# hpcaitech/Open-Sora

Measured on AMD Instinct MI355X. Metric: latent_frames_per_sec (30-step rectified-flow sampling; denoise-step ms in ms_per_step), higher is better.
Workload: dtype bf16; 1 GPU; MMDiT-XL (hidden 1152, 16x72, 9+19 blocks) denoise step, latent 16x64x64 (16x512x512 px), L=16896 tokens, CFG batch 3, 30-step Euler sampling; cfg_batch=3, parallelism=single GPU

## Files before the change

### include/osk.h

```cpp
#ifndef OSK_H
#define OSK_H
#include <stdint.h>
#ifdef __cplusplus
extern "C" {
#endif

#define OSK_ABI_VERSION 2
int osk_abi_version(void);
const char* osk_arch(void);

int osk_ln_modulate_bf16(const void* x, int64_t x_batch_stride, int64_t x_row_stride,
                         void* out, int64_t out_batch_stride, int64_t out_row_stride,
                         const float* shift, const float* scale, int64_t mod_batch_stride,
                         int B, int L, int D, float eps, void* stream);

int osk_gemm_bf16(const void* A, int64_t a_batch_stride, int64_t a_row_stride, int a_rows_per_batch,
                  const void* W, int64_t w_row_stride, const float* bias,
                  void* C, int64_t c_batch_stride, int64_t c_row_stride, int c_rows_per_batch,
                  const void* res, const float* gate, int64_t gate_batch_stride,
                  int M, int N, int K, int gelu_from, int out_f32, void* stream);

int osk_gemm_tile_choice(int M, int N, int K);
int osk_gemm_tile_override(int tile_kind);
int osk_gemm_tile_choice_strided(int M, int N, int K, int64_t a_batch_stride, int64_t a_row_stride, int a_rows_per_batch,
                                 int64_t w_row_stride);

typedef struct OskGemmOperands {
  const void* A; int64_t a_batch_stride, a_row_stride; int a_rows_per_batch;
  const void* W; int64_t w_row_stride; const float* bias;
  void* C; int64_t c_batch_stride, c_row_stride; int c_rows_per_batch;
  const void* res; const float* gate; int64_t gate_batch_stride;
  int M;
} OskGemmOperands;
int osk_gemm_bf16_pair(const OskGemmOperands* first, const OskGemmOperands* second, int N, int K, int gelu_from, void* stream);

typedef struct OskGemmTask {
  OskGemmOperands op;
  int N, gelu_from;
  int skip_from, skip_len;
  int vt_head_dim;
} OskGemmTask;
int osk_gemm_group_bf16(const OskGemmTask* tasks, int n_tasks, int K, void* stream);

int osk_gemm_geglu_bf16(const void* A, int64_t a_batch_stride, int64_t a_row_stride, int a_rows_per_batch,
                        const void* W_packed, int64_t w_row_stride, const float* bias_packed, void* C,
                        int64_t c_batch_stride, int64_t c_row_stride, int c_rows_per_batch, int M, int N_out, int K,
                        void* workspace, int64_t workspace_bytes, void* stream);

int osk_ln_modulate_fp8(const void* x, int64_t x_batch_stride, int64_t x_row_stride, void* out8, float* scales,
                        const float* shift, const float* scale, int64_t mod_batch_stride,
                        int B, int L, int D, float eps, void* stream);
int osk_quantize_rows_fp8(const void* x, int64_t x_batch_stride, int64_t x_row_stride, int rows_per_batch,
                          void* out8, float* scales, int M, int K, void* stream);
int osk_gemm_fp8(const void* A8, int64_t a_batch_stride, int64_t a_row_stride, int a_rows_per_batch,
                 const float* a_scale, const void* W8, int64_t w_row_stride, const float* w_scale,
                 const float* bias, void* C, int64_t c_batch_stride, int64_t c_row_stride, int c_rows_per_batch,
                 const void* res, const float* gate, int64_t gate_batch_stride,
                 int M, int N, int K, int gelu_from, int out_f32, void* stream);

int osk_gemv_tasks_bf16(const float* x, int64_t x_batch_stride, int Bv, int K,
                        const uint64_t* w_ptrs, const uint64_t* b_ptrs, const int32_t* out_cols,
                        const int32_t* n_rows, int n_tasks,
                        float* out, int64_t out_batch_stride, int act_in, int accumulate, void* stream);

int osk_timestep_embedding(const float* t, int B, int dim, float max_period, float time_factor,
                           float* out, void* stream);

int osk_rope_table(const float* ids, int64_t n_rows, int n_axes, const int32_t* axes_dim_host,
                   double theta, int f32_angles, float* cos_out, float* sin_out, void* stream);

int osk_qknorm_rope_bf16(void* q, void* k, int64_t batch_stride, int64_t row_stride,
                         const void* q_scale0, const void* k_scale0,
                         const void* q_scale1, const void* k_scale1, int l_split,
                         const float* cos_t, const float* sin_t, int64_t cs_batch_stride,
                         int B, int L, int H, int hd, int rope_mode, float eps, float q_mult, void* stream);

int osk_v_transpose_bf16(const void* v, int64_t batch_stride, int64_t row_stride,
                         void* vt, int B, int L, int H, int hd, void* stream);

int osk_kv_join_bf16(const void* k_seg, const void* v_seg,
                     int64_t seg_stride, int64_t batch_stride, int64_t row_stride,
                     void* k_out, int64_t ko_batch_stride, int64_t ko_row_stride,
                     void* vt_out,
                     int B, int H, int hd, int n_seg, int seg_len, int L, void* stream);

#define OSK_KV_JOIN_K_BF16 0
#define OSK_KV_JOIN_K_E4M3 1
int osk_kv_quant_rows_fp8(const void* x, int64_t batch_stride, int64_t row_stride, const float* scales,
                          void* out, int64_t o_batch_stride, int64_t o_row_stride,
                          int B, int L, int H, int hd, void* stream);
int osk_kv_join_fp8(const void* k_seg, int64_t k_seg_stride, int64_t k_batch_stride, int64_t k_row_stride, int k_kind,
                    const void* v_seg, int64_t v_seg_stride, int64_t v_batch_stride, int64_t v_row_stride,
                    void* k_out, int64_t ko_batch_stride, int64_t ko_row_stride,
                    void* vt8_out,
                    int B, int H, int hd, int n_seg, int seg_len, int L, void* stream);

int osk_attention_fwd_bf16(const void* q, int64_t q_batch_stride, int64_t q_row_stride,
                           const void* k, int64_t k_seg_stride, int64_t k_batch_stride, int64_t k_row_stride,
                           const void* vt, int64_t vt_seg_stride,
                           void* out, int64_t o_batch_stride, int64_t o_row_stride,
                           float* lse, int B, int H, int Lq, int n_seg, int seg_len, int hd,
                           float scale, int q_prescaled, int kv_batches, void* stream);

int64_t osk_attention_workspace_bytes(void);
int osk_attention_tail_split_factor(int B, int H, int Lq, int n_seg, int seg_len, int hd, int64_t workspace_bytes);
int osk_attention_launch_shape(int B, int H, int Lq, int n_seg, int seg_len, int hd, float score_bound,
                               int64_t workspace_bytes, int* rows_per_unit);
int osk_attention_rows_override(int rows_per_unit);
int osk_attention_fwd_ws_bf16(const void* q, int64_t q_batch_stride, int64_t q_row_stride,
                           const void* k, int64_t k_seg_stride, int64_t k_batch_stride, int64_t k_row_stride,
                           const void* vt, int64_t vt_seg_stride,
                           void* out, int64_t o_batch_stride, int64_t o_row_stride,
                           float* lse, int B, int H, int Lq, int n_seg, int seg_len, int hd,
                           float scale, int q_prescaled, int kv_batches, void* workspace, int64_t workspace_bytes, void* stream);

int osk_attention_fwd_bounded_bf16(const void* q, int64_t q_batch_stride, int64_t q_row_stride,
                           const void* k, int64_t k_seg_stride, int64_t k_batch_stride, int64_t k_row_stride,
                           const void* vt, int64_t vt_seg_stride,
                           void* out, int64_t o_batch_stride, int64_t o_row_stride,
                           float* lse, int B, int H, int Lq, int n_seg, int seg_len, int hd,
                           float scale, int q_prescaled, int kv_batches, float score_bound,
                           void* workspace, int64_t workspace_bytes, void* stream);

int osk_rownorm2_max_bf16(const void* x, int64_t batch_stride, int64_t row_stride, int B, int L, int H, int hd,
                          float* out, int accumulate, void* stream);
int osk_attention_fwd_auto_bf16(const void* q, int64_t q_batch_stride, int64_t q_row_stride,
                           const void* k, int64_t k_seg_stride, int64_t k_batch_stride, int64_t k_row_stride,
                           const void* vt, int64_t vt_seg_stride,
                           void* out, int64_t o_batch_stride, int64_t o_row_stride,
                           float* lse, int B, int H, int Lq, int n_seg, int seg_len, int hd,
                           float scale, int q_prescaled, int kv_batches, const float* q_norm2_max, const float* k_norm2_max,
                           void* workspace, int64_t workspace_bytes, void* stream);

int osk_attention_merge_bf16(const void* parts, int64_t part_stride, int64_t p_batch_stride, int64_t p_row_stride,
                             const float* lse, void* out, int64_t o_batch_stride, int64_t o_row_stride, float* lse_out,
                             int S, int B, int H, int L, int hd, void* stream);

int osk_v_scale_fp8(const void* v, int64_t v_batch_stride, int64_t v_row_stride, float* scales, int B, int L, int H,
                    int hd, void* stream);
int osk_kv_scale_fp8(const void* k, int64_t k_batch_stride, int64_t k_row_stride,
                     const void* v, int64_t v_batch_stride, int64_t v_row_stride, float* scales,
                     int B, int L, int H, int hd, void* stream);
int osk_v_transpose_fp8(const void* v, int64_t v_batch_stride, int64_t v_row_stride, const float* scales, void* vt8,
                        int B, int L, int H, int hd, void* stream);
int osk_attention_fwd_pv8_bf16(const void* q, int64_t q_batch_stride, int64_t q_row_stride,
                               const void* k, int64_t k_seg_stride, int64_t k_batch_stride, int64_t k_row_stride,
                               const void* vt8, int64_t vt8_seg_stride, const float* v_scale,
                               void* out, int64_t o_batch_stride, int64_t o_row_stride,
                               float* lse, int B, int H, int Lq, int n_seg, int seg_len, int hd,
                               float scale, int q_prescaled, int kv_batches, void* workspace, int64_t workspace_bytes,
                               void* stream);

int osk_k_pack_fp8(const void* k, int64_t k_batch_stride, int64_t k_row_stride, const float* scales, void* k8,
                   int B, int L, int H, int hd, void* stream);
int osk_attention_fwd_qk8_bf16(const void* q, int64_t q_batch_stride, int64_t q_row_stride,
                               const void* k8, int64_t k8_seg_stride, int64_t k8_batch_stride, int64_t k8_row_stride,
                               const float* k_scale, const void* vt8, int64_t vt8_seg_stride, const float* v_scale,
                               void* out, int64_t o_batch_stride, int64_t o_row_stride,
                               float* lse, int B, int H, int Lq, int n_seg, int seg_len, int hd,
                               float scale, int q_prescaled, int kv_batches, void* workspace, int64_t workspace_bytes,
                               void* stream);

#define OSK_ATTN_BF16 0
#define OSK_ATTN_PV8 1
#define OSK_ATTN_QK8 2
int64_t osk_attention_ragged_workspace_bytes(int B, int H, int Lq, int hd);
int osk_attention_fwd_ragged_bf16(const void* q, int64_t q_batch_stride, int64_t q_row_stride,
                                  const void* k, int64_t k_seg_stride, int64_t k_batch_stride, int64_t k_row_stride,
                                  const float* k_scale, const void* vt, int64_t vt_seg_stride, const float* v_scale,
                                  void* out, int64_t o_batch_stride, int64_t o_row_stride, float* lse,
                                  int B, int H, int Lq, int n_seg, int seg_len, int last_seg_len, int hd,
                                  float scale, int q_prescaled, int kv_batches, float score_bound, int mode,
                                  void* workspace, int64_t workspace_bytes, void* stream);
int osk_attention_merge_into_bf16(void* out, int64_t o_batch_stride, int64_t o_row_stride, float* lse, const float* o_b,
                                  const float* lse_b, int B, int H, int Lq, int hd, void* stream);
int osk_attention_merge_into2_bf16(void* out, int64_t o_batch_stride, int64_t o_row_stride, float* lse, const float* o_b,
                                   const float* lse_b, const float* o_c, const float* lse_c, int B, int H, int Lq, int hd,
                                   void* stream);

int64_t osk_attention_window_workspace_bytes(int B, int H, int Lq, int hd);
int osk_attention_fwd_window_bf16(const void* q, int64_t q_batch_stride, int64_t q_row_stride,
                                  const void* k, int64_t k_batch_stride, int64_t k_row_stride, const void* vt,
                                  void* out, int64_t o_batch_stride, int64_t o_row_stride, float* lse,
                                  int B, int H, int Lq, int Lk, int n_prefix, int hd, float scale, int q_prescaled,
                                  int kv_batches, float score_bound, const int32_t* windows, int n_windows,
                                  void* workspace, int64_t workspace_bytes, void* stream);
int osk_attention_fwd_window_fp8_bf16(const void* q, int64_t q_batch_stride, int64_t q_row_stride,
                                      const void* k, int64_t k_batch_stride, int64_t k_row_stride, const float* k_scale,
                                      const void* vt, const float* v_scale, void* out, int64_t o_batch_stride,
                                      int64_t o_row_stride, float* lse, int B, int H, int Lq, int Lk, int n_prefix, int hd,
                                      float scale, int q_prescaled, int kv_batches, int mode, const int32_t* windows,
                                      int n_windows, void* workspace, int64_t workspace_bytes, void* stream);
int64_t osk_attention_window_anchor_workspace_bytes(int B, int H, int Lq, int hd);
int osk_attention_fwd_window_anchor_bf16(const void* q, int64_t q_batch_stride, int64_t q_row_stride,
                                         const void* k, int64_t k_batch_stride, int64_t k_row_stride, const float* k_scale,
                                         const void* vt, const float* v_scale, void* out, int64_t o_batch_stride,
                                         int64_t o_row_stride, float* lse, int B, int H, int Lq, int Lk, int n_prefix,
                                         int n_suffix, int hd, float scale, int q_prescaled, int kv_batches, float score_bound,
                                         int mode, const int32_t* windows, int n_windows, void* workspace,
                                         int64_t workspace_bytes, void* stream);

int osk_attention_short_bf16(const void* q, int64_t q_batch_stride, int64_t q_row_stride, const void* k, int64_t k_batch_stride,
                             int64_t k_row_stride, const void* v, int64_t v_batch_stride, int64_t v_row_stride, void* out,
                             int64_t o_batch_stride, int64_t o_row_stride, const float* alibi_slopes, int B, int H, int Lq, int Lk,
                             int hd, float scale, void* stream);

int osk_attention_relbias_bf16(const void* q, int64_t q_batch_stride, int64_t q_row_stride, const void* k, int64_t k_batch_stride,
                               int64_t k_row_stride, const void* v, int64_t v_batch_stride, int64_t v_row_stride, void* out,
                               int64_t o_batch_stride, int64_t o_row_stride, const float* bias, int64_t bias_row_stride, int B,
                               int H, int L, int hd, float scale, void* stream);

const char* osk_attention_kernel_name(int hd, int seg_len);
const char* osk_attention_body_name(int hd, int n_seg, int seg_len, float score_bound);

int osk_cfg_euler_bf16(const void* pred, int64_t n, const void* x, void* x_out,
                       float g_txt, float g_img, const float* g_img_vec, float dt, void* stream);

int osk_cfg_euler_nb_bf16(const void* pred, int nb, int64_t n, const void* x, void* x_out,
                          float g_txt, float g_img, const float* g_img_vec, float dt, void* stream);

int osk_copy_rows_bf16(const void* src, int64_t src_chunk_stride, int64_t src_batch_stride, int64_t src_row_stride, void* dst,
                       int64_t dst_chunk_stride, int64_t dst_batch_stride, int64_t dst_row_stride, int n_chunks, int B, int L, int C,
                       void* stream);

int64_t osk_step_delta_workspace_bytes(int B, int L, int C);
int osk_step_delta_bf16(const void* cur, int64_t cur_batch_stride, int64_t cur_row_stride, void* prev, float* sums, int B, int L, int C,
                        void* workspace, int64_t workspace_bytes, void* stream);

int osk_step_sums_combine_f32(const float* pairs, int P, float* sums, void* stream);

int osk_residual_sub_bf16(const void* a, int64_t a_batch_stride, int64_t a_row_stride, const void* b, int64_t b_batch_stride,
                          int64_t b_row_stride, void* out, int64_t out_batch_stride, int64_t out_row_stride, int B, int L, int C,
                          void* stream);
int osk_residual_add_bf16(const void* a, int64_t a_batch_stride, int64_t a_row_stride, const void* b, int64_t b_batch_stride,
                          int64_t b_row_stride, void* out, int64_t out_batch_stride, int64_t out_row_stride, int B, int L, int C,
                          void* stream);

int osk_attn_cache_copy_bf16(const void* src, int64_t src_batch_stride, int64_t src_row_stride, void* dst, int64_t dst_batch_stride,
                             int64_t dst_row_stride, const int32_t* row_map, int cache_rows, int to_cache, int B, int L, int C,
                             void* stream);


int osk_causal_conv3d_ndhwc_bf16(const void* x, int B, int T, int H, int W, int Cin,
                                 const void* w, int64_t w_row_stride, const float* bias, int Cout, int ksize,
                                 int stride_t, int stride_h, int stride_w, int up_t, int up_hw,
                                 const void* res, void* out, int To, int Ho, int Wo, void* stream);

int osk_causal_conv3d_gn_ndhwc_bf16(const void* x, int B, int T, int H, int W, int Cin,
                                    const void* w, int64_t w_row_stride, const float* bias, int Cout, int ksize,
                                    int stride_t, int stride_h, int stride_w, int up_t, int up_hw,
                                    const void* res, void* out, int To, int Ho, int Wo,
                                    double* gn_sums, int gn_groups, void* stream);


int osk_conv2d_nhwc_bf16(const void* x, int B, int H, int W, int Cin, const void* w, int64_t w_row_stride,
                         const float* bias, int Cout, int ksize, int stride, int pad, int up, const void* res,
                         void* out, int Ho, int Wo, double* gn_sums, int gn_groups, void* stream);

int osk_groupnorm_stats_ndhwc_bf16(const void* x, int B, int64_t S, int C, int G, double* sums, void* stream);

int osk_groupnorm_apply_ndhwc_bf16(const void* x, const double* sums, const float* gamma, const float* beta,
                                   void* out, int B, int64_t S, int C, int G, float eps, int silu, void* stream);

int osk_groupnorm_table_f32(const double* sums, const float* gamma, const float* beta, float* table, int B, int64_t S,
                            int C, int G, float eps, void* stream);
int osk_causal_conv3d_gnin_ndhwc_bf16(const void* x, const float* gn_in_table, int B, int T, int H, int W, int Cin,
                                      const void* w, int64_t w_row_stride, const float* bias, int Cout, int ksize,
                                      int stride_t, int stride_h, int stride_w, const void* res, void* out, int To, int Ho,
                                      int Wo, double* gn_sums, int gn_groups, void* stream);

int osk_masked_softmax_f32_bf16(const float* scores, int64_t ld_scores, void* probs, int64_t ld_probs,
                                int Sq, int Sk, int keys_per_frame, float scale, void* stream);

int osk_attention_hd512_fwd_bf16(const void* q, int64_t q_batch_stride, int64_t q_row_stride, const void* k,
                                 int64_t k_batch_stride, int64_t k_row_stride, const void* vt, int64_t vt_batch_stride,
                                 int64_t vt_row_stride, const float* bias_v, void* out, int64_t out_batch_stride,
                                 int64_t out_row_stride, int B, int S, int keys_per_frame, float scale, void* stream);
int osk_attention_hd512_fwd_ws_bf16(const void* q, int64_t q_batch_stride, int64_t q_row_stride, const void* k,
                                    int64_t k_batch_stride, int64_t k_row_stride, const void* vt, int64_t vt_batch_stride,
                                    int64_t vt_row_stride, const float* bias_v, void* out, int64_t out_batch_stride,
                                    int64_t out_row_stride, int B, int S, int keys_per_frame, float scale, void* workspace,
                                    int64_t workspace_bytes, void* stream);
int64_t osk_attention_hd512_workspace_bytes(int B, int S);

int osk_blend_bf16(const void* a, void* b, int64_t outer, int Da, int Db, int extent, int64_t inner, void* stream);


int osk_conv3d_zp_ndhwc_bf16(const void* x, int B, int T, int H, int W, int Cin, const void* w, int64_t w_row_stride,
                             const float* bias, int Cout, int ksize, int up_t, int up_hw, int act, const void* res,
                             void* out, void* stream);

int osk_conv3d_zp_strided_ndhwc_bf16(const void* x, int B, int T, int H, int W, int Cin, const void* w, int64_t w_row_stride,
                                     const float* bias, int Cout, int stride_t, int stride_hw, const void* res, void* out,
                                     void* stream);

int osk_unshuffle_avg_ndhwc_bf16(const void* x, int B, int T, int H, int W, int Cin, void* out, int Cout, int ft, int fhw,
                                 void* stream);

int osk_dup_shuffle_ndhwc_bf16(const void* x, int B, int T, int H, int W, int Cin, void* out, int Cout, int ft, int fhw,
                               void* stream);

int osk_dwconv3d_ndhwc_bf16(const void* x, int B, int T, int H, int W, int C, const void* w, const float* bias, int ksize,
                            int glu, void* out, void* stream);

int osk_gconv32_bf16(const void* x, int64_t M, int C, const void* w, void* out, void* stream);

int osk_relu_linear_attn_bf16(const void* qkv, int B, int N, int G, void* out, int64_t out_row_stride, float* workspace,
                              int64_t workspace_bytes, int nsplit, float eps, void* stream);

int osk_rmsnorm_affine_bf16(const void* x, int64_t M, int C, const float* weight, const float* bias, float eps,
                            const void* res, int relu, void* out, void* stream);


int osk_layernorm_affine_bf16(const void* x, int64_t x_row_stride, void* out, int64_t out_row_stride, const float* weight,
                              const float* bias, int64_t M, int C, float eps, void* stream);

int osk_attention_causal_bf16(const void* q, int64_t q_batch_stride, int64_t q_row_stride, const void* k, int64_t k_batch_stride,
                              int64_t k_row_stride, const void* v, int64_t v_batch_stride, int64_t v_row_stride, void* out,
                              int64_t o_batch_stride, int64_t o_row_stride, int B, int H, int L, int hd, float scale, void* stream);

int osk_gemm_quickgelu_bf16(const void* A, int64_t a_batch_stride, int64_t a_row_stride, int a_rows_per_batch, const void* W,
                            int64_t w_row_stride, const float* bias, void* C, int64_t c_batch_stride, int64_t c_row_stride,
                            int c_rows_per_batch, int M, int N, int K, void* stream);

typedef struct OskLoraAdapter {
  const void* a; int64_t a_row_stride;
  const void* b; int64_t b_row_stride;
  int r; float scale;
} OskLoraAdapter;
int osk_lora_merge_bf16(const void* w, int64_t w_row_stride, void* out, int64_t out_row_stride, int N, int K,
                        const OskLoraAdapter* adapters, int n_adapters, void* stream);

#ifdef __cplusplus
}
#endif
#endif
```

### open_sora_amd/_C.py

```python
from __future__ import annotations

import ctypes as C
import os

import torch

from .build import LIB_PATH

_i64, _i32, _f32, _f64, _vp = C.c_int64, C.c_int32, C.c_float, C.c_double, C.c_void_p

SIGNATURES = {
    "osk_abi_version": [],
    "osk_arch": [],
    "osk_gemm_geglu_bf16": [_vp, _i64, _i64, _i32, _vp, _i64, _vp, _vp, _i64, _i64, _i32, _i32, _i32, _i32, _vp, _i64, _vp],
    "osk_attention_short_bf16": [_vp, _i64, _i64, _vp, _i64, _i64, _vp, _i64, _i64, _vp, _i64, _i64, _vp, _i32, _i32, _i32, _i32, _i32,
                                 _f32, _vp],
    "osk_attention_relbias_bf16": [_vp, _i64, _i64, _vp, _i64, _i64, _vp, _i64, _i64, _vp, _i64, _i64, _vp, _i64, _i32, _i32, _i32, _i32,
                                   _f32, _vp],
    "osk_attention_kernel_name": [_i32, _i32],
    "osk_attention_body_name": [_i32, _i32, _i32, _f32],
    "osk_ln_modulate_bf16": [_vp, _i64, _i64, _vp, _i64, _i64, _vp, _vp, _i64, _i32, _i32, _i32, _f32, _vp],
    "osk_gemm_bf16": [_vp, _i64, _i64, _i32, _vp, _i64, _vp, _vp, _i64, _i64, _i32, _vp, _vp, _i64,
                      _i32, _i32, _i32, _i32, _i32, _vp],
    "osk_gemm_bf16_pair": [_vp, _vp, _i32, _i32, _i32, _vp],
    "osk_gemm_group_bf16": [_vp, _i32, _i32, _vp],
    "osk_gemm_tile_choice": [_i32, _i32, _i32],
    "osk_gemm_tile_choice_strided": [_i32, _i32, _i32, _i64, _i64, _i32, _i64],
    "osk_gemm_tile_override": [_i32],
    "osk_ln_modulate_fp8": [_vp, _i64, _i64, _vp, _vp, _vp, _vp, _i64, _i32, _i32, _i32, _f32, _vp],
    "osk_quantize_rows_fp8": [_vp, _i64, _i64, _i32, _vp, _vp, _i32, _i32, _vp],
    "osk_gemm_fp8": [_vp, _i64, _i64, _i32, _vp, _vp, _i64, _vp, _vp, _vp, _i64, _i64, _i32, _vp, _vp, _i64,
                     _i32, _i32, _i32, _i32, _i32, _vp],
    "osk_gemv_tasks_bf16": [_vp, _i64, _i32, _i32, _vp, _vp, _vp, _vp, _i32, _vp, _i64, _i32, _i32, _vp],
    "osk_timestep_embedding": [_vp, _i32, _i32, _f32, _f32, _vp, _vp],
    "osk_rope_table": [_vp, _i64, _i32, C.POINTER(_i32), _f64, _i32, _vp, _vp, _vp],
    "osk_qknorm_rope_bf16": [_vp, _vp, _i64, _i64, _vp, _vp, _vp, _vp, _i32, _vp, _vp, _i64,
                             _i32, _i32, _i32, _i32, _i32, _f32, _f32, _vp],
    "osk_v_transpose_bf16": [_vp, _i64, _i64, _vp, _i32, _i32, _i32, _i32, _vp],
    "osk_kv_join_bf16": [_vp, _vp, _i64, _i64, _i64, _vp, _i64, _i64, _vp, _i32, _i32, _i32, _i32, _i32, _i32, _vp],
    "osk_kv_quant_rows_fp8": [_vp, _i64, _i64, _vp, _vp, _i64, _i64, _i32, _i32, _i32, _i32, _vp],
    "osk_kv_join_fp8": [_vp, _i64, _i64, _i64, _i32, _vp, _i64, _i64, _i64, _vp, _i64, _i64, _vp, _i32, _i32, _i32, _i32, _i32, _i32, _vp],
    "osk_attention_fwd_bf16": [_vp, _i64, _i64, _vp, _i64, _i64, _i64, _vp, _i64, _vp, _i64, _i64, _vp,
                               _i32, _i32, _i32, _i32, _i32, _i32, _f32, _i32, _i32, _vp],
    "osk_attention_fwd_ws_bf16": [_vp, _i64, _i64, _vp, _i64, _i64, _i64, _vp, _i64, _vp, _i64, _i64, _vp,
                                  _i32, _i32, _i32, _i32, _i32, _i32, _f32, _i32, _i32, _vp, _i64, _vp],
    "osk_attention_fwd_bounded_bf16": [_vp, _i64, _i64, _vp, _i64, _i64, _i64, _vp, _i64, _vp, _i64, _i64, _vp,
                                       _i32, _i32, _i32, _i32, _i32, _i32, _f32, _i32, _i32, _f32, _vp, _i64, _vp],
    "osk_attention_fwd_auto_bf16": [_vp, _i64, _i64, _vp, _i64, _i64, _i64, _vp, _i64, _vp, _i64, _i64, _vp,
                                    _i32, _i32, _i32, _i32, _i32, _i32, _f32, _i32, _i32, _vp, _vp, _vp, _i64, _vp],
    "osk_attention_merge_bf16": [_vp, _i64, _i64, _i64, _vp, _vp, _i64, _i64, _vp, _i32, _i32, _i32, _i32, _i32, _vp],
    "osk_attention_ragged_workspace_bytes": [_i32, _i32, _i32, _i32],
    "osk_attention_fwd_ragged_bf16": [_vp, _i64, _i64, _vp, _i64, _i64, _i64, _vp, _vp, _i64, _vp, _vp, _i64, _i64, _vp,
                                      _i32, _i32, _i32, _i32, _i32, _i32, _i32, _f32, _i32, _i32, _f32, _i32, _vp, _i64, _vp],
    "osk_attention_merge_into_bf16": [_vp, _i64, _i64, _vp, _vp, _vp, _i32, _i32, _i32, _i32, _vp],
    "osk_attention_window_workspace_bytes": [_i32, _i32, _i32, _i32],
    "osk_attention_fwd_window_bf16": [_vp, _i64, _i64, _vp, _i64, _i64, _vp, _vp, _i64, _i64, _vp, _i32, _i32, _i32, _i32, _i32, _i32,
                                      _f32, _i32, _i32, _f32, _vp, _i32, _vp, _i64, _vp],
    "osk_attention_fwd_window_fp8_bf16": [_vp, _i64, _i64, _vp, _i64, _i64, _vp, _vp, _vp, _vp, _i64, _i64, _vp, _i32, _i32, _i32, _i32,
                                          _i32, _i32, _f32, _i32, _i32, _i32, _vp, _i32, _vp, _i64, _vp],
    "osk_attention_merge_into2_bf16": [_vp, _i64, _i64, _vp, _vp, _vp, _vp, _vp, _i32, _i32, _i32, _i32, _vp],
    "osk_attention_window_anchor_workspace_bytes": [_i32, _i32, _i32, _i32],
    "osk_attention_fwd_window_anchor_bf16": [_vp, _i64, _i64, _vp, _i64, _i64, _vp, _vp, _vp, _vp, _i64, _i64, _vp, _i32, _i32, _i32, _i32,
                                             _i32, _i32, _i32, _f32, _i32, _i32, _f32, _i32, _vp, _i32, _vp, _i64, _vp],
    "osk_rownorm2_max_bf16": [_vp, _i64, _i64, _i32, _i32, _i32, _i32, _vp, _i32, _vp],
    "osk_attention_workspace_bytes": [],
    "osk_v_scale_fp8": [_vp, _i64, _i64, _vp, _i32, _i32, _i32, _i32, _vp],
    "osk_kv_scale_fp8": [_vp, _i64, _i64, _vp, _i64, _i64, _vp, _i32, _i32, _i32, _i32, _vp],
    "osk_v_transpose_fp8": [_vp, _i64, _i64, _vp, _vp, _i32, _i32, _i32, _i32, _vp],
    "osk_attention_fwd_pv8_bf16": [_vp, _i64, _i64, _vp, _i64, _i64, _i64, _vp, _i64, _vp, _vp, _i64, _i64, _vp,
                                   _i32, _i32, _i32, _i32, _i32, _i32, _f32, _i32, _i32, _vp, _i64, _vp],
    "osk_k_pack_fp8": [_vp, _i64, _i64, _vp, _vp, _i32, _i32, _i32, _i32, _vp],
    "osk_attention_fwd_qk8_bf16": [_vp, _i64, _i64, _vp, _i64, _i64, _i64, _vp, _vp, _i64, _vp, _vp, _i64, _i64, _vp,
                                   _i32, _i32, _i32, _i32, _i32, _i32, _f32, _i32, _i32, _vp, _i64, _vp],
    "osk_attention_tail_split_factor": [_i32, _i32, _i32, _i32, _i32, _i32, _i64],
    "osk_attention_launch_shape": [_i32, _i32, _i32, _i32, _i32, _i32, _f32, _i64, C.POINTER(_i32)],
    "osk_attention_rows_override": [_i32],
    "osk_cfg_euler_bf16": [_vp, _i64, _vp, _vp, _f32, _f32, _vp, _f32, _vp],
    "osk_cfg_euler_nb_bf16": [_vp, _i32, _i64, _vp, _vp, _f32, _f32, _vp, _f32, _vp],
    "osk_copy_rows_bf16": [_vp, _i64, _i64, _i64, _vp, _i64, _i64, _i64, _i32, _i32, _i32, _i32, _vp],
    "osk_step_delta_workspace_bytes": [_i32, _i32, _i32],
    "osk_step_delta_bf16": [_vp, _i64, _i64, _vp, _vp, _i32, _i32, _i32, _vp, _i64, _vp],
    "osk_step_sums_combine_f32": [_vp, _i32, _vp, _vp],
    "osk_residual_sub_bf16": [_vp, _i64, _i64, _vp, _i64, _i64, _vp, _i64, _i64, _i32, _i32, _i32, _vp],
    "osk_residual_add_bf16": [_vp, _i64, _i64, _vp, _i64, _i64, _vp, _i64, _i64, _i32, _i32, _i32, _vp],
    "osk_attn_cache_copy_bf16": [_vp, _i64, _i64, _vp, _i64, _i64, _vp, _i32, _i32, _i32, _i32, _i32, _vp],
    "osk_causal_conv3d_ndhwc_bf16": [_vp, _i32, _i32, _i32, _i32, _i32, _vp, _i64, _vp, _i32, _i32, _i32, _i32, _i32,
                                     _i32, _i32, _vp, _vp, _i32, _i32, _i32, _vp],
    "osk_causal_conv3d_gn_ndhwc_bf16": [_vp, _i32, _i32, _i32, _i32, _i32, _vp, _i64, _vp, _i32, _i32, _i32, _i32, _i32,
                                        _i32, _i32, _vp, _vp, _i32, _i32, _i32, _vp, _i32, _vp],
    "osk_causal_conv3d_gnin_ndhwc_bf16": [_vp, _vp, _i32, _i32, _i32, _i32, _i32, _vp, _i64, _vp, _i32, _i32, _i32, _i32,
                                          _i32, _vp, _vp, _i32, _i32, _i32, _vp, _i32, _vp],
    "osk_conv2d_nhwc_bf16": [_vp, _i32, _i32, _i32, _i32, _vp, _i64, _vp, _i32, _i32, _i32, _i32, _i32, _vp, _vp, _i32, _i32,
                             _vp, _i32, _vp],
    "osk_groupnorm_table_f32": [_vp, _vp, _vp, _vp, _i32, _i64, _i32, _i32, _f32, _vp],
    "osk_groupnorm_stats_ndhwc_bf16": [_vp, _i32, _i64, _i32, _i32, _vp, _vp],
    "osk_groupnorm_apply_ndhwc_bf16": [_vp, _vp, _vp, _vp, _vp, _i32, _i64, _i32, _i32, _f32, _i32, _vp],
    "osk_masked_softmax_f32_bf16": [_vp, _i64, _vp, _i64, _i32, _i32, _i32, _f32, _vp],
    "osk_blend_bf16": [_vp, _vp, _i64, _i32, _i32, _i32, _i64, _vp],
    "osk_attention_hd512_fwd_ws_bf16": [_vp, _i64, _i64, _vp, _i64, _i64, _vp, _i64, _i64, _vp, _vp, _i64, _i64, _i32, _i32,
                                        _i32, _f32, _vp, _i64, _vp],
    "osk_attention_hd512_workspace_bytes": [_i32, _i32],
    "osk_attention_hd512_fwd_bf16": [_vp, _i64, _i64, _vp, _i64, _i64, _vp, _i64, _i64, _vp, _vp, _i64, _i64, _i32, _i32,
                                     _i32, _f32, _vp],
    "osk_conv3d_zp_ndhwc_bf16": [_vp, _i32, _i32, _i32, _i32, _i32, _vp, _i64, _vp, _i32, _i32, _i32, _i32, _i32, _vp, _vp, _vp],
    "osk_conv3d_zp_strided_ndhwc_bf16": [_vp, _i32, _i32, _i32, _i32, _i32, _vp, _i64, _vp, _i32, _i32, _i32, _vp, _vp, _vp],
    "osk_dup_shuffle_ndhwc_bf16": [_vp, _i32, _i32, _i32, _i32, _i32, _vp, _i32, _i32, _i32, _vp],
    "osk_unshuffle_avg_ndhwc_bf16": [_vp, _i32, _i32, _i32, _i32, _i32, _vp, _i32, _i32, _i32, _vp],
    "osk_dwconv3d_ndhwc_bf16": [_vp, _i32, _i32, _i32, _i32, _i32, _vp, _vp, _i32, _i32, _vp, _vp],
    "osk_gconv32_bf16": [_vp, _i64, _i32, _vp, _vp, _vp],
    "osk_relu_linear_attn_bf16": [_vp, _i32, _i32, _i32, _vp, _i64, _vp, _i64, _i32, _f32, _vp],
    "osk_rmsnorm_affine_bf16": [_vp, _i64, _i32, _vp, _vp, _f32, _vp, _i32, _vp, _vp],
    "osk_layernorm_affine_bf16": [_vp, _i64, _vp, _i64, _vp, _vp, _i64, _i32, _f32, _vp],
    "osk_attention_causal_bf16": [_vp, _i64, _i64, _vp, _i64, _i64, _vp, _i64, _i64, _vp, _i64, _i64, _i32, _i32, _i32, _i32, _f32, _vp],
    "osk_gemm_quickgelu_bf16": [_vp, _i64, _i64, _i32, _vp, _i64, _vp, _vp, _i64, _i64, _i32, _i32, _i32, _i32, _vp],
    "osk_lora_merge_bf16": [_vp, _i64, _vp, _i64, _i32, _i32, _vp, _i32, _vp],
}


def _load() -> C.CDLL:
    if not os.path.isfile(LIB_PATH):
        raise ImportError(
            f"{LIB_PATH} is missing: build it with `python -m open_sora_amd.build` (hipcc, gfx950). "
            "open_sora_amd has no CPU or eager fallback."
        )
    lib = C.CDLL(LIB_PATH)
    for name, argtypes in SIGNATURES.items():
        fn = getattr(lib, name)
        fn.argtypes = argtypes
        fn.restype = (C.c_char_p if name in ("osk_arch", "osk_attention_kernel_name", "osk_attention_body_name") else
                      _i64 if name in ("osk_attention_workspace_bytes", "osk_attention_hd512_workspace_bytes",
                                       "osk_attention_ragged_workspace_bytes", "osk_attention_window_workspace_bytes",
                                       "osk_attention_window_anchor_workspace_bytes",
                                       "osk_step_delta_workspace_bytes") else _i32)
    if lib.osk_abi_version() != 2:
        raise ImportError("libosk_hip.so ABI version mismatch")
    return lib


class _TracingLib:

    def __init__(self, inner):
        self._inner = inner
        self._ids: dict = {}

    def _norm(self, kind, v):
        if kind is _vp:
            if v is None:
                return "NULL"
            v = int(v)
            k = self._ids.setdefault(v, len(self._ids))
            return f"p{k}@{v & 0xFF:02x}"
        if isinstance(v, C.Array):
            return tuple(int(x) for x in v)
        return round(float(v), 9) if kind in (_f32, _f64) else int(v)

    def __getattr__(self, name):
        fn = getattr(self._inner, name)
        sig = SIGNATURES.get(name)
        if sig is None:
            return fn

        def traced(*args):
            TRACE_LOG.append((name,) + tuple(self._norm(k, a) for k, a in zip(sig, args)))
            return fn(*args)

        return traced


TRACE_LOG: list = []
lib = _load()
if os.environ.get("OSK_TRACE"):
    lib = _TracingLib(lib)


OSK_EUNSUPPORTED = -2


def _check(status: int, what: str) -> None:
    if status != 0:
        kind = "invalid argument / unsupported shape" if status < 0 else "HIP error"
        raise RuntimeError(f"{what} failed: status {status} ({kind})")


def _stream() -> int:
    return torch.cuda.current_stream().cuda_stream


def _p(t) -> int | None:
    return None if t is None else t.data_ptr()


def ln_modulate(x: torch.Tensor, shift: torch.Tensor, scale: torch.Tensor, out: torch.Tensor,
                mod_batch_stride: int, eps: float = 1e-6) -> torch.Tensor:
    B, L, D = x.shape
    assert x.dtype == torch.bfloat16 and out.dtype == torch.bfloat16 and shift.dtype == torch.float32, (x.dtype, out.dtype)
    _check(lib.osk_ln_modulate_bf16(x.data_ptr(), x.stride(0), x.stride(1), out.data_ptr(), out.stride(0),
                                    out.stride(1), shift.data_ptr(), scale.data_ptr(), mod_batch_stride,
                                    B, L, D, eps, _stream()), "osk_ln_modulate_bf16")
    return out


PROFILE_GEMM = None
PROFILE_ATTENTION = None


class _prof:

    def __init__(self, sink, *extra):
        self.sink, self.extra = sink, extra

    def __enter__(self):
        if self.sink is not None:
            self.e0, self.e1 = torch.cuda.Event(enable_timing=True), torch.cuda.Event(enable_timing=True)
            self.e0.record()

    def __exit__(self, *exc):
        if self.sink is not None:
            self.e1.record()
            self.sink.append((self.e0, self.e1, *self.extra))
        return False


def _gemm_prof(flops: float) -> _prof:
    return _prof(PROFILE_GEMM, flops)


def _attn_prof() -> _prof:
    return _prof(PROFILE_ATTENTION)


def gemm(a: torch.Tensor, w: torch.Tensor, bias, out: torch.Tensor, *, res=None, gate=None,
         gate_batch_stride: int = 0, gelu_from: int | None = None) -> torch.Tensor:
    B, L, K = a.shape
    N = w.shape[0]
    assert out.shape[0] == B and out.shape[1] == L and out.shape[2] == N
    assert a.dtype == torch.bfloat16 and w.dtype == torch.bfloat16 and out.dtype in (torch.bfloat16, torch.float32), \
        (a.dtype, w.dtype, out.dtype)
    if res is not None:
        assert res.stride() == out.stride() and res.dtype == torch.bfloat16
    with _gemm_prof(2.0 * B * L * N * K):
        _check(lib.osk_gemm_bf16(a.data_ptr(), a.stride(0), a.stride(1), L, w.data_ptr(), w.stride(0), _p(bias),
                                 out.data_ptr(), out.stride(0), out.stride(1), L, _p(res), _p(gate),
                                 gate_batch_stride, B * L, N, K, N if gelu_from is None else gelu_from,
                                 1 if out.dtype == torch.float32 else 0, _stream()), "osk_gemm_bf16")
    return out


def gemm_tile_kind(a: torch.Tensor, w: torch.Tensor) -> int:
    B, L, K = a.shape
    kind = lib.osk_gemm_tile_choice_strided(B * L, w.shape[0], K, a.stride(0), a.stride(1), L, w.stride(0))
    if kind < 0:
        _check(kind, "osk_gemm_tile_choice_strided")
    return kind


def geglu_pack(w_value: torch.Tensor, w_gate: torch.Tensor, b_value=None, b_gate=None):
    n, k = w_value.shape
    assert w_gate.shape == (n, k) and n % 16 == 0
    w = torch.stack((w_value.reshape(n // 16, 16, k), w_gate.reshape(n // 16, 16, k)), 1).reshape(2 * n, k).contiguous()
    b = None
    if b_value is not None:
        b = torch.stack((b_value.float().reshape(n // 16, 16), b_gate.float().reshape(n // 16, 16)), 1).reshape(2 * n).contiguous()
    return w, b


def gemm_geglu(a: torch.Tensor, w_packed: torch.Tensor, bias_packed, out: torch.Tensor, workspace: torch.Tensor | None = None):
    B, L, K = a.shape
    n_out = w_packed.shape[0] // 2
    assert out.shape == (B, L, n_out) and a.dtype == out.dtype == w_packed.dtype == torch.bfloat16
    _check(lib.osk_gemm_geglu_bf16(a.data_ptr(), a.stride(0), a.stride(1), L, w_packed.data_ptr(), w_packed.stride(0), _p(bias_packed),
                                   out.data_ptr(), out.stride(0), out.stride(1), L, B * L, n_out, K, _p(workspace),
                                   0 if workspace is None else workspace.numel() * workspace.element_size(), _stream()),
           "osk_gemm_geglu_bf16")
    return out


class OskGemmOperands(C.Structure):
    _fields_ = [("A", _vp), ("a_batch_stride", _i64), ("a_row_stride", _i64), ("a_rows_per_batch", _i32),
                ("W", _vp), ("w_row_stride", _i64), ("bias", _vp),
                ("C", _vp), ("c_batch_stride", _i64), ("c_row_stride", _i64), ("c_rows_per_batch", _i32),
                ("res", _vp), ("gate", _vp), ("gate_batch_stride", _i64), ("M", _i32)]


def _gemm_operands(a, w, bias, out, res, gate, gate_batch_stride, *, wide_out: bool = False) -> OskGemmOperands:
    B, L, K = a.shape
    assert out.shape[0] == B and out.shape[1] == L and (out.shape[2] >= 1 if wide_out else out.shape[2] == w.shape[0]) and w.shape[1] == K
    assert a.dtype == torch.bfloat16 and w.dtype == torch.bfloat16 and out.dtype == torch.bfloat16
    if res is not None:
        assert res.stride() == out.stride() and res.dtype == torch.bfloat16
    return OskGemmOperands(a.data_ptr(), a.stride(0), a.stride(1), L, w.data_ptr(), w.stride(0), _p(bias), out.data_ptr(),
                           out.stride(0), out.stride(1), L, _p(res), _p(gate), gate_batch_stride, B * L)


def gemm_pair(first: dict, second: dict, *, gelu_from: int | None = None) -> None:
    ops = [_gemm_operands(d["a"], d["w"], d["bias"], d["out"], d.get("res"), d.get("gate"), d.get("gate_batch_stride", 0))
           for d in (first, second)]
    N, K = first["w"].shape
    assert tuple(second["w"].shape) == (N, K)
    with _gemm_prof(2.0 * (ops[0].M + ops[1].M) * N * K):
        _check(lib.osk_gemm_bf16_pair(C.addressof(ops[0]), C.addressof(ops[1]), N, K, N if gelu_from is None else gelu_from,
                                      _stream()), "osk_gemm_bf16_pair")


class OskGemmTask(C.Structure):
    _fields_ = [("op", OskGemmOperands), ("N", _i32), ("gelu_from", _i32), ("skip_from", _i32), ("skip_len", _i32), ("vt_head_dim", _i32)]


def gemm_group(tasks: list) -> bool:
    arr = (OskGemmTask * len(tasks))()
    K = None
    flops = 0.0
    for t, d in zip(arr, tasks):
        if "vt" in d:
            x, w, vt = d["x"], d["w"], d["vt"]
            B, L, k_ = x.shape
            assert x.dtype == w.dtype == vt.dtype == torch.bfloat16 and vt.is_contiguous() and vt.dim() == 4 and d["vt_pos"] % 64 == 0
            assert vt.shape[0] == B and vt.shape[1] * vt.shape[2] == w.shape[0] and d["vt_pos"] + (L + 63) // 64 * 64 <= vt.shape[3]
            t.op = OskGemmOperands(x.data_ptr(), x.stride(0), x.stride(1), L, w.data_ptr(), w.stride(0), _p(d.get("bias")),
                                   vt.data_ptr() + 2 * d["vt_pos"], vt.stride(0), vt.stride(2), L, None, None, 0, B * L)
            t.N, t.gelu_from, t.skip_from, t.skip_len, t.vt_head_dim = w.shape[0], w.shape[0], 0, 0, d["hd"]
            flops += 2.0 * B * L * w.shape[0] * k_
        else:
            a, w, out = d["a"], d["w"], d["out"]
            k_ = a.shape[2]
            t.op = _gemm_operands(a, w, d.get("bias"), out, d.get("res"), d.get("gate"), d.get("gate_batch_stride", 0), wide_out=True)
            sf, sl = d.get("skip", (0, 0))
            t.N, t.gelu_from, t.skip_from, t.skip_len, t.vt_head_dim = w.shape[0], d.get("gelu_from", w.shape[0]) if d.get("gelu_from") is not None else w.shape[0], sf, sl, 0
            flops += 2.0 * a.shape[0] * a.shape[1] * (w.shape[0] - sl) * k_
        assert K in (None, k_), "the tasks of a group share K"
        K = k_
    with _gemm_prof(flops):
        rc = lib.osk_gemm_group_bf16(C.addressof(arr), len(tasks), K, _stream())
    if rc == OSK_EUNSUPPORTED:
        return False
    _check(rc, "osk_gemm_group_bf16")
    return True


def ln_modulate_fp8(x: torch.Tensor, shift: torch.Tensor, scale: torch.Tensor, mod_batch_stride: int, eps: float = 1e-6):
    B, L, D = x.shape
    out8 = torch.empty(B * L, D, dtype=torch.uint8, device=x.device)
    scales = torch.empty(B * L, dtype=torch.float32, device=x.device)
    _check(lib.osk_ln_modulate_fp8(x.data_ptr(), x.stride(0), x.stride(1), out8.data_ptr(), scales.data_ptr(),
                                   shift.data_ptr(), scale.data_ptr(), mod_batch_stride, B, L, D, eps, _stream()),
           "osk_ln_modulate_fp8")
    return out8, scales


def quantize_rows_fp8(x: torch.Tensor, out8: torch.Tensor | None = None, scales: torch.Tensor | None = None):
    if x.dim() == 2:
        x = x.unsqueeze(0)
    B, L, K = x.shape
    M = B * L
    if out8 is None:
        out8 = torch.empty(M, K, dtype=torch.uint8, device=x.device)
    if scales is None:
        scales = torch.empty(M, dtype=torch.float32, device=x.device)
    assert out8.is_contiguous() and out8.numel() == M * K and scales.numel() >= M
    _check(lib.osk_quantize_rows_fp8(x.data_ptr(), x.stride(0), x.stride(1), L, out8.data_ptr(), scales.data_ptr(),
                                     M, K, _stream()), "osk_quantize_rows_fp8")
    return out8, scales


def gemm_fp8_supported(M: int, N: int, K: int) -> bool:
    return M >= 256 and N >= 128 and K % 128 == 0 and 256 * K <= 0xFFFFFFFF


def gemm_fp8(a8: torch.Tensor, a_scale: torch.Tensor, w8: torch.Tensor, w_scale: torch.Tensor, bias,
             out: torch.Tensor, *, res=None, gate=None, gate_batch_stride: int = 0,
             gelu_from: int | None = None) -> torch.Tensor:
    M, K = a8.shape
    N = w8.shape[0]
    B, L = out.shape[0], out.shape[1]
    assert B * L == M and out.shape[2] == N and w8.shape[1] == K
    if res is not None:
        assert res.stride() == out.stride()
    with _gemm_prof(2.0 * M * N * K):
        _check(lib.osk_gemm_fp8(a8.data_ptr(), 0, a8.stride(0), M, a_scale.data_ptr(), w8.data_ptr(), w8.stride(0),
                                w_scale.data_ptr(), _p(bias), out.data_ptr(), out.stride(0), out.stride(1), L, _p(res),
                                _p(gate), gate_batch_stride, M, N, K, N if gelu_from is None else gelu_from,
                                1 if out.dtype == torch.float32 else 0, _stream()), "osk_gemm_fp8")
    return out


def gemv_tasks(x: torch.Tensor, tasks, out: torch.Tensor, act_in: int = 0, accumulate: bool = False):
    Bv, K = x.shape
    _check(lib.osk_gemv_tasks_bf16(x.data_ptr(), x.stride(0), Bv, K, tasks.w_ptrs.data_ptr(),
                                   tasks.b_ptrs.data_ptr(), tasks.out_cols.data_ptr(),
                                   tasks.n_rows.data_ptr(), tasks.n_tasks, out.data_ptr(), out.stride(0),
                                   act_in, 1 if accumulate else 0, _stream()), "osk_gemv_tasks_bf16")
    return out


class GemvTasks:

    ROWS = 64

    def __init__(self, layers, device):
        wp, bp, oc, nr = [], [], [], []
        self._keep = []
        for w, b, col in layers:
            assert w.dtype == torch.bfloat16 and w.is_contiguous()
            self._keep.append((w, b))
            N, K = w.shape
            for r0 in range(0, N, self.ROWS):
                n = min(self.ROWS, N - r0)
                wp.append(w.data_ptr() + r0 * K * 2)
                bp.append(0 if b is None else b.data_ptr() + r0 * 2)
                oc.append(col + r0)
                nr.append(n)
        self.n_tasks = len(wp)
        to_i64 = lambda v: v - (1 << 64) if v >= (1 << 63) else v
        self.w_ptrs = torch.tensor([to_i64(v) for v in wp], dtype=torch.int64, device=device)
        self.b_ptrs = torch.tensor([to_i64(v) for v in bp], dtype=torch.int64, device=device)
        self.out_cols = torch.tensor(oc, dtype=torch.int32, device=device)
        self.n_rows = torch.tensor(nr, dtype=torch.int32, device=device)


def timestep_embedding(t: torch.Tensor, out: torch.Tensor, max_period: float = 10000.0,
                       time_factor: float = 1000.0) -> torch.Tensor:
    B, dim = out.shape
    _check(lib.osk_timestep_embedding(t.data_ptr(), B, dim, max_period, time_factor, out.data_ptr(), _stream()),
           "osk_timestep_embedding")
    return out


def rope_table(ids: torch.Tensor, axes_dim, theta: float, f32_angles: bool, cos: torch.Tensor, sin: torch.Tensor):
    n_rows, n_axes = ids.shape
    arr = (_i32 * n_axes)(*[int(a) for a in axes_dim])
    _check(lib.osk_rope_table(ids.data_ptr(), n_rows, n_axes, arr, float(theta), 1 if f32_angles else 0,
                              cos.data_ptr(), sin.data_ptr(), _stream()), "osk_rope_table")


def qknorm_rope(q: torch.Tensor, k: torch.Tensor, qs0, ks0, qs1, ks1, l_split: int, cos, sin,
                cs_batch_stride: int, H: int, hd: int, rope_mode: int, eps: float = 1e-6, q_mult: float = 1.0):
    t = q if q is not None else k
    B, L, _ = t.shape
    assert q is None or k is None or q.stride() == k.stride()
    _check(lib.osk_qknorm_rope_bf16(_p(q), _p(k), t.stride(0), t.stride(1), qs0.data_ptr(),
                                    ks0.data_ptr(), qs1.data_ptr(), ks1.data_ptr(), l_split, cos.data_ptr(),
                                    sin.data_ptr(), cs_batch_stride, B, L, H, hd, rope_mode, eps, q_mult, _stream()),
           "osk_qknorm_rope_bf16")


def v_transpose(v: torch.Tensor, vt: torch.Tensor, H: int, hd: int):
    B, L, _ = v.shape
    _check(lib.osk_v_transpose_bf16(v.data_ptr(), v.stride(0), v.stride(1), vt.data_ptr(), B, L, H, hd, _stream()),
           "osk_v_transpose_bf16")


def kv_join(k_seg: torch.Tensor, v_seg: torch.Tensor, k_out: torch.Tensor, vt_out: torch.Tensor, H: int, hd: int, L: int):
    n_seg, B, seg_len, D = k_seg.shape
    assert k_seg.dtype == v_seg.dtype == k_out.dtype == vt_out.dtype == torch.bfloat16 and D == H * hd, (k_seg.dtype, v_seg.dtype, D, H, hd)
    assert v_seg.shape == k_seg.shape and v_seg.stride() == k_seg.stride() and k_seg.stride(3) == 1, (v_seg.shape, v_seg.stride(), k_seg.stride())
    assert tuple(k_out.shape) == (B, L, D) and k_out.stride(2) == 1, (k_out.shape, k_out.stride())
    assert tuple(vt_out.shape) == (B, H, hd, (L + 63) // 64 * 64) and vt_out.is_contiguous(), (vt_out.shape, vt_out.stride())
    _check(lib.osk_kv_join_bf16(k_seg.data_ptr(), v_seg.data_ptr(), k_seg.stride(0), k_seg.stride(1), k_seg.stride(2), k_out.data_ptr(),
                                k_out.stride(0), k_out.stride(1), vt_out.data_ptr(), B, H, hd, n_seg, seg_len, L, _stream()),
           "osk_kv_join_bf16")


_ATTN_WS: dict = {}


def attention_workspace(device) -> torch.Tensor:
    dev = torch.device(device)
    key = (str(dev), torch.cuda.current_stream(dev).cuda_stream if dev.type == "cuda" else 0)
    ws = _ATTN_WS.get(key)
    if ws is None:
        ws = _ATTN_WS[key] = torch.empty(lib.osk_attention_workspace_bytes(), dtype=torch.uint8, device=dev)
    return ws


def _attn_call(name: str, q, k, vt, out, H, hd, scale, lse, n_seg, seg_len, k_seg_stride, vt_seg_stride, q_prescaled, kv_batches,
               workspace, own=(), after_vt=()):
    B, Lq, _ = q.shape
    with _attn_prof():
        _check(getattr(lib, name)(q.data_ptr(), q.stride(0), q.stride(1), k.data_ptr(), k_seg_stride, k.stride(0), k.stride(1),
                                  vt.data_ptr(), vt_seg_stride, *after_vt, out.data_ptr(), out.stride(0), out.stride(1), _p(lse),
                                  B, H, Lq, n_seg, k.shape[1] if seg_len is None else seg_len, hd, scale, int(q_prescaled),
                                  kv_batches, *own, _p(workspace), 0 if workspace is None else workspace.numel(), _stream()), name)
    return out


def attention_fwd(q: torch.Tensor, k: torch.Tensor, vt: torch.Tensor, out: torch.Tensor, H: int, hd: int,
                  scale: float, *, lse=None, n_seg: int = 1, seg_len: int | None = None,
                  k_seg_stride: int = 0, vt_seg_stride: int = 0, q_prescaled: bool = False, kv_batches: int = 0,
                  workspace: torch.Tensor | None = None, score_bound: float = 0.0):
    if CHECK_SCORE_BOUND and score_bound > 0 and not torch.cuda.is_current_stream_capturing():
        _assert_score_bound(q, k, H, hd, scale, n_seg, k.shape[1] if seg_len is None else seg_len, k_seg_stride, q_prescaled, kv_batches,
                            score_bound)
    return _attn_call("osk_attention_fwd_bounded_bf16", q, k, vt, out, H, hd, scale, lse, n_seg, seg_len, k_seg_stride, vt_seg_stride,
                      q_prescaled, kv_batches, workspace, own=(float(score_bound),))


def rownorm2_max(x: torch.Tensor, out: torch.Tensor, H: int, hd: int, accumulate: bool = False) -> torch.Tensor:
    B, L, _ = x.shape
    assert x.dtype == torch.bfloat16 and out.dtype == torch.float32 and out.is_contiguous() and out.numel() == B * H
    _check(lib.osk_rownorm2_max_bf16(x.data_ptr(), x.stride(0), x.stride(1), B, L, H, hd, out.data_ptr(), 1 if accumulate else 0, _stream()),
           "osk_rownorm2_max_bf16")
    return out


def attention_fwd_auto(q: torch.Tensor, k: torch.Tensor, vt: torch.Tensor, out: torch.Tensor, H: int, hd: int, scale: float,
                       qn2: torch.Tensor, kn2: torch.Tensor, *, lse=None, n_seg: int = 1, seg_len: int | None = None,
                       k_seg_stride: int = 0, vt_seg_stride: int = 0, q_prescaled: bool = True, kv_batches: int = 0,
                       workspace: torch.Tensor | None = None):
    B = q.shape[0]
    assert qn2.dtype == kn2.dtype == torch.float32 and qn2.numel() == B * H and kn2.numel() == (kv_batches or B) * H
    return _attn_call("osk_attention_fwd_auto_bf16", q, k, vt, out, H, hd, scale, lse, n_seg, seg_len, k_seg_stride, vt_seg_stride,
                      q_prescaled, kv_batches, workspace, own=(qn2.data_ptr(), kn2.data_ptr()))


def attention_merge(parts: torch.Tensor, lse: torch.Tensor, out: torch.Tensor, H: int, hd: int,
                    lse_out: torch.Tensor | None = None) -> torch.Tensor:
    assert parts.dim() == 4 and lse.dim() == 4 and out.dim() == 3, (parts.shape, lse.shape, out.shape)
    S, B, L, D = parts.shape
    assert 1 <= S <= 8 and D == H * hd and hd % 8 == 0, (parts.shape, H, hd)
    assert parts.dtype == torch.bfloat16 and out.dtype == torch.bfloat16 and tuple(out.shape) == (B, L, D), (parts.dtype, out.dtype, out.shape)
    assert lse.dtype == torch.float32 and lse.is_contiguous() and tuple(lse.shape) == (S, B, H, L), (lse.dtype, lse.shape, lse.stride())
    for t in (parts, out):
        assert t.stride(-1) == 1 and all(st % 8 == 0 for st in t.stride()[:-1]) and t.data_ptr() % 16 == 0, (t.stride(), t.data_ptr() % 16)
    if lse_out is not None:
        assert lse_out.dtype == torch.float32 and lse_out.is_contiguous() and tuple(lse_out.shape) == (B, H, L), (lse_out.dtype, lse_out.shape)
    _check(lib.osk_attention_merge_bf16(parts.data_ptr(), parts.stride(0), parts.stride(1), parts.stride(2), lse.data_ptr(),
                                        out.data_ptr(), out.stride(0), out.stride(1), _p(lse_out), S, B, H, L, hd, _stream()),
           "osk_attention_merge_bf16")
    return out


def _grown_workspace(kind: str, need: int, device) -> torch.Tensor:
    dev = torch.device(device)
    key = (kind, str(dev), torch.cuda.current_stream(dev).cuda_stream if dev.type == "cuda" else 0)
    ws = _ATTN_WS.get(key)
    if ws is None or ws.numel() < need:
        ws = _ATTN_WS[key] = torch.empty(need, dtype=torch.uint8, device=dev)
    return ws


def attention_ragged_workspace(B: int, H: int, Lq: int, hd: int, device) -> torch.Tensor:
    return _grown_workspace("ragged", lib.osk_attention_ragged_workspace_bytes(B, H, Lq, hd), device)


def _attn_operands(mode: int, q, k, k_scale, vt, v_scale, out, lse, H: int, hd: int, kv_batches: int, Lk: int, k_seg_stride: int = 0,
                   vt_seg_stride: int = 0, vt_keys: int | None = None):
    assert mode != 2 or hd == 128, f"the fp8 QK^T kernel exists for head_dim 128 only, not {hd}"
    assert q.dim() == 3 and q.shape[2] == H * hd, (q.shape, H, hd)
    assert q.dtype == torch.bfloat16 and out.dtype == torch.bfloat16 and q.stride(2) == 1 and out.stride(2) == 1, (q.dtype, out.dtype, q.stride(), out.stride())
    assert q.stride(0) % 8 == 0 and q.stride(1) % 8 == 0 and q.data_ptr() % 16 == 0, (q.stride(), q.data_ptr() % 16)
    B, Lq, _ = q.shape
    Bkv = kv_batches or B
    for s_ in ((), (v_scale,), (k_scale, v_scale))[mode]:
        assert s_ is not None and s_.dtype == torch.float32 and s_.is_contiguous() and s_.numel() == Bkv * H, "scales: f32 [Bkv, H]"
    if mode == 2:
        assert k.dtype == torch.uint8 and k.dim() == 4 and k.stride(3) == 1 and k.stride(2) == 128, (k.dtype, k.shape, k.stride())
        assert tuple(k.shape) == k8_shape(Bkv, H, Lk, hd) and k.stride(1) == k.shape[2] * 128, (k.shape, k.stride(), Lk)
        assert k.data_ptr() % 16 == 0 and k.stride(0) % 16 == 0 and k_seg_stride % 16 == 0, (k.stride(), k_seg_stride)
    else:
        assert k.dtype == torch.bfloat16 and k.dim() == 3 and k.stride(2) == 1 and k.shape[2] == H * hd, (k.dtype, k.shape, k.stride())
        assert k.stride(0) % 8 == 0 and k.stride(1) % 8 == 0 and k_seg_stride % 8 == 0 and k.data_ptr() % 16 == 0, (k.stride(), k_seg_stride)
    assert vt.dtype == (torch.bfloat16 if mode == 0 else torch.uint8) and vt.data_ptr() % 16 == 0, (vt.dtype, vt.data_ptr() % 16)
    assert vt_seg_stride % (8 if mode == 0 else 16) == 0, vt_seg_stride
    if vt_keys is not None:
        assert vt.shape[-2] == (hd if mode == 0 else vt8_rows(hd)) and vt.shape[-1] == vt_keys, (vt.shape, hd, vt_keys)
    if lse is not None:
        assert lse.dtype == torch.float32 and lse.is_contiguous() and tuple(lse.shape) == (B, H, Lq), (lse.dtype, lse.shape)
    return k.stride(0), 128 if mode == 2 else k.stride(1)


def attention_fwd_ragged(q: torch.Tensor, k: torch.Tensor, vt: torch.Tensor, out: torch.Tensor, H: int, hd: int, scale: float, *,
                         n_seg: int, seg_len: int, last_seg_len: int, k_seg_stride: int, vt_seg_stride: int, workspace: torch.Tensor,
                         lse=None, q_prescaled: bool = False, kv_batches: int = 0, score_bound: float = 0.0,
                         k_scale: torch.Tensor | None = None, v_scale: torch.Tensor | None = None):
    assert out.dim() == 3 and q.shape == out.shape, (q.shape, out.shape)
    assert n_seg >= 2 and 1 <= last_seg_len <= seg_len, (n_seg, seg_len, last_seg_len)
    assert out.stride(0) % 8 == 0 and out.stride(1) % 8 == 0 and out.data_ptr() % 16 == 0, (out.stride(), out.data_ptr() % 16)
    assert k_scale is None or v_scale is not None, "qk8 operands come with both scale vectors"
    mode = 0 if v_scale is None else (1 if k_scale is None else 2)
    kbs, krs = _attn_operands(mode, q, k, k_scale, vt, v_scale, out, lse, H, hd, kv_batches, seg_len, k_seg_stride, vt_seg_stride)
    B, Lq, _ = q.shape
    Bkv = kv_batches or B
    assert workspace is not None and workspace.dtype == torch.uint8 and workspace.data_ptr() % 16 == 0
    if CHECK_SCORE_BOUND and mode == 0 and score_bound > 0 and not torch.cuda.is_current_stream_capturing():
        _assert_score_bound(q, k, H, hd, scale, n_seg - 1, seg_len, k_seg_stride, q_prescaled, kv_batches, score_bound)
        k_last = torch.as_strided(k, (Bkv, last_seg_len, H * hd), k.stride(), k.storage_offset() + (n_seg - 1) * k_seg_stride)
        _assert_score_bound(q, k_last, H, hd, scale, 1, last_seg_len, 0, q_prescaled, kv_batches, score_bound)
    with _attn_prof():
        _check(lib.osk_attention_fwd_ragged_bf16(q.data_ptr(), q.stride(0), q.stride(1), k.data_ptr(), k_seg_stride, kbs, krs, _p(k_scale),
                                                 vt.data_ptr(), vt_seg_stride, _p(v_scale), out.data_ptr(), out.stride(0), out.stride(1),
                                                 _p(lse), B, H, Lq, n_seg, seg_len, last_seg_len, hd, scale, int(q_prescaled), kv_batches,
                                                 float(score_bound), mode, workspace.data_ptr(), workspace.numel(), _stream()),
               "osk_attention_fwd_ragged_bf16")
    return out


def attention_window_workspace_bytes(B: int, H: int, Lq: int, hd: int) -> int:
    return int(lib.osk_attention_window_workspace_bytes(B, H, Lq, hd))


def attention_window_workspace(B: int, H: int, Lq: int, hd: int, device) -> torch.Tensor:
    return _grown_workspace("window", lib.osk_attention_window_workspace_bytes(B, H, Lq, hd), device)


def check_window_table(windows: torch.Tensor, Lq: int, Lk: int, n_prefix: int, n_suffix: int = 0) -> None:
    if not (isinstance(windows, torch.Tensor) and windows.device.type == "cpu" and windows.dtype == torch.int32):
        raise ValueError("windows: a host (CPU) int32 tensor is expected")
    if n_prefix < 0 or n_prefix % 64 or n_prefix >= Lk:
        raise ValueError(f"n_prefix = {n_prefix}: a multiple of 64 in [0, Lk = {Lk}) is expected")
    if n_suffix < 0 or (n_suffix > 0 and ((Lk - n_suffix) % 64 or Lk - n_suffix <= n_prefix)):
        raise ValueError(f"n_suffix = {n_suffix}: 0, or Lk - n_suffix a multiple of 64 greater than n_prefix = {n_prefix} is expected (Lk = {Lk})")
    nqb, tiles = (Lq + 255) // 256, (Lk - n_suffix - n_prefix + 63) // 64
    if windows.dim() != 2 or tuple(windows.shape) != (nqb, 2):
        raise ValueError(f"windows: shape {tuple(windows.shape)}, expected ({nqb}, 2) = one row per 256 query rows")
    first, n = windows[:, 0], windows[:, 1]
    if bool((first < 0).any()):
        raise ValueError("windows: a negative first tile")
    if bool((n < 1).any()):
        raise ValueError("windows: an empty range (tile count < 1)")
    if bool((first.long() + n.long() > tiles).any()):
        raise ValueError(f"windows: a range ends past the body's {tiles} tiles")


_WINDOW_DEV: dict = {}


def _window_on_device(windows: torch.Tensor, device) -> torch.Tensor:
    c = windows.contiguous()
    key = (str(torch.device(device)), tuple(c.shape), c.numpy().tobytes())
    dev = _WINDOW_DEV.get(key)
    if dev is None:
# ... 771 lines not shown
```

### open_sora_amd/csrc/gemm256x.hip

```cpp
#include "acc_quads.h"
#include "gemm_epilogue16.h"
#include "tile256.h"
#include "gemm256x_regs.inc"

namespace osk_gemm {
namespace {

struct GeoX {
  static constexpr int NB = OSKX_NB;
  template <int T>
  OSK_DEV void read(const osk_v4f* aq, float* v4) {
#pragma unroll
    for (int i = 0; i < 4; ++i) asm volatile("v_accvgpr_read_b32 %0, %1" : "=v"(v4[i]) : "a"(aq[T][i]));
  }
};

template <int NP>
struct GemmPack {
  GemmParams p[NP];
};

#ifdef OSK_GEMM_TILE_TIMING
__device__ unsigned long long osk_gemm_tile_ticks[4];
#define OSK_TT(i, t0) if (threadIdx.x == 0) atomicAdd(&osk_gemm_tile_ticks[i], __builtin_amdgcn_s_memtime() - (t0))
#else
#define OSK_TT(i, t0)
#endif


template <bool OUT_F32>
struct LinearWalk {
  template <int NP>
  OSK_DEV int col_tiles(const GemmPack<NP>& pk, int) { return (pk.p[0].N - pk.p[0].skip_len + 255) / 256; }
  template <int NP>
  OSK_DEV int phys_n0(const GemmPack<NP>& pk, int n0) { return n0 + (n0 >= pk.p[0].skip_from ? pk.p[0].skip_len : 0); }
  OSK_DEV int64_t a_row(const GemmParams& p, int m) { return osk_tile256::a_row_offset(p, m); }
  OSK_DEV int64_t w_row(const GemmParams& p, int n, bool) { return osk_tile256::w_row_offset(p, n); }
  OSK_DEV bool affine(const GemmParams& p, int m0, int n0) {
    return m0 + 256 <= p.M && n0 + 256 <= p.N && m0 / p.arpb == (m0 + 255) / p.arpb;
  }
  OSK_DEV int64_t a_origin(const GemmParams& p, int m0) { return osk_tile256::tile_window(m0, p.M, p.arpb, 0x7fffffff, p.abs_, p.ars).lo; }
  OSK_DEV int64_t w_origin(const GemmParams& p, int n0) { return osk_tile256::tile_window(n0, p.N, 0x7fffffff, 0x7fffffff, 0, p.wrs).lo; }
  OSK_DEV bool folded(const GemmParams& p, int n0w) { return p.bias != nullptr && n0w + OSKX_NB * 16 <= p.N; }
  OSK_DEV void epilogue(const osk_v4f* aq, const GemmParams& p, int m0w, int n0w, int l15, int q4, bool folded) {
    constexpr int WT = OSKX_NB * 16;
    const int b_first = m0w / p.crpb, b_last = (m0w + WT - 1) / p.crpb;
    const bool interior = m0w + WT <= p.M && n0w + WT <= p.N && b_first == b_last;
    epi16::epilogue_all<GeoX, OUT_F32>(aq, p, m0w, n0w, l15, q4, interior, folded);
  }
};

struct VtWalk {
  template <int NP>
  OSK_DEV int col_tiles(const GemmPack<NP>& pk, int i) { return (pk.p[i].N + 255) / 256; }
  template <int NP>
  OSK_DEV int phys_n0(const GemmPack<NP>&, int n0) { return n0; }
  OSK_DEV int64_t a_row(const GemmParams& p, int m) {
    m = m < p.M ? m : p.M - 1;
    return (int64_t)m * p.ars;
  }
  OSK_DEV int64_t w_row(const GemmParams& p, int n, bool permute) {
    n = n < p.N ? n : p.N - 1;
    const int wb = n / p.wrpb;
    int pos = n - wb * p.wrpb;
    if (permute) pos = vt_perm64(pos, p.vt);
    pos = pos < p.wvalid ? pos : p.wvalid - 1;
    return wb * p.wbs + (int64_t)pos * p.wrs;
  }
  OSK_DEV bool affine(const GemmParams& p, int m0, int n0) {
    const int wb = n0 / p.wrpb, pos0 = n0 - wb * p.wrpb;
    return m0 + 256 <= p.M && n0 + 256 <= p.N && pos0 + 256 <= p.wrpb && pos0 + 256 <= p.wvalid;
  }
  OSK_DEV int64_t a_origin(const GemmParams& p, int m0) { return osk_tile256::tile_window(m0, p.M, 0x7fffffff, 0x7fffffff, 0, p.ars).lo; }
  OSK_DEV int64_t w_origin(const GemmParams& p, int n0) { return osk_tile256::tile_window(n0, p.N, p.wrpb, p.wvalid, p.wbs, p.wrs).lo; }
  OSK_DEV bool folded(const GemmParams&, int) { return false; }
  OSK_DEV void epilogue(const osk_v4f* aq, const GemmParams& p, int m0w, int n0w, int l15, int q4, bool) {
    epi16::vt_all<GeoX>(aq, p, m0w, n0w, l15, q4);
  }
};

#define OSKW_OPERANDS                                                                                               \
  ::"v"(faA0), "v"(faW0), "v"(aoff[0]), "v"(aoff[1]), "v"(aoff[2]), "v"(aoff[3]), "v"(aoff[4]), "v"(aoff[5]),          \
      "v"(aoff[6]), "v"(aoff[7]), "v"(woff[0]), "v"(woff[1]), "v"(woff[2]), "v"(woff[3]), "v"(woff[4]), "v"(woff[5]),  \
      "v"(woff[6]), "v"(woff[7]), "v"(boff), "s"(abase), "s"(wbase), "s"(bbase), "s"(nk), "s"(adst), "s"(wdst),        \
      "s"(flags), "s"(abasen), "s"(wbasen), "v"(aoffp), "v"(woffp)

template <class Walk, int NP>
OSK_DEV void tile_walk(const GemmPack<NP>& pk) {
  constexpr int WT = OSKX_NB * 16;
  extern __shared__ __attribute__((aligned(16))) unsigned char smem[];
  const int tid = threadIdx.x;
  const int lane = tid & 63;
  const int wave = __builtin_amdgcn_readfirstlane(tid >> 6);
  const int wm = wave >> 1, wn = wave & 1;
  const int q4 = lane >> 4, l15 = lane & 15;

  const int nbn0 = Walk::col_tiles(pk, 0), nbn1 = Walk::col_tiles(pk, NP - 1);
  const int nt0 = ((pk.p[0].M + 255) / 256) * nbn0;
  const int ntiles = NP == 1 ? nt0 : nt0 + ((pk.p[NP - 1].M + 255) / 256) * nbn1;
  const int grp = pk.p[0].group > 0 ? pk.p[0].group : 1;
  auto tile_of = [&](int it, int& sel, int& m0, int& n0) {
    int tile = xcd_remap(it, ntiles);
    sel = (NP > 1 && tile >= nt0) ? 1 : 0;
    tile -= sel ? nt0 : 0;
    const osk_tile256::TileBlock t = osk_tile256::grouped_tile(tile, (pk.p[sel].M + 255) / 256, sel ? nbn1 : nbn0, grp);
    m0 = t.bm * 256;
    n0 = Walk::phys_n0(pk, t.bn * 256);
  };
  const unsigned lds_base = (unsigned)(uintptr_t)(__attribute__((address_space(3))) unsigned char*)smem;
  const unsigned sz0 = (unsigned)((q4 ^ ((l15 >> 1) & 7)) << 4);
  const unsigned faA0 = lds_base + (wm * WT + l15) * 128 + sz0;
  const unsigned faW0 = lds_base + OSKX_W_BASE + (wn * WT + l15) * 128 + sz0;
  const unsigned nk = rfl((unsigned)(pk.p[0].K / 64));
  const unsigned adst = rfl(lds_base + wave * 1024), wdst = rfl(lds_base + OSKX_W_BASE + wave * 1024);

  unsigned prefetched = 0;
  for (int it = blockIdx.x; it < ntiles; it += (int)gridDim.x) {
    const int itn = it + (int)gridDim.x;
#ifdef OSK_GEMM_TILE_TIMING
    const unsigned long long tt0 = __builtin_amdgcn_s_memtime();
#endif
    int sel, m0, n0, seln = 0, m0n = 0, n0n = 0;
    tile_of(it, sel, m0, n0);
    const GemmParams& p = pk.p[NP == 1 ? 0 : sel];
    bool has_next = itn < ntiles;
    const int64_t alo = Walk::a_origin(p, m0), wlo = Walk::w_origin(p, n0);
    int64_t alon = alo, wlon = wlo;
    if (has_next) {
      tile_of(itn, seln, m0n, n0n);
      has_next = seln == sel && Walk::affine(p, m0, n0) && Walk::affine(p, m0n, n0n);
      alon = Walk::a_origin(p, m0n);
      wlon = Walk::w_origin(p, n0n);
    }
    const uint64_t abase = rfl64((uint64_t)(uintptr_t)p.A + (uint64_t)(alo * 2)), wbase = rfl64((uint64_t)(uintptr_t)p.W + (uint64_t)(wlo * 2));
    const uint64_t abasen = rfl64((uint64_t)(uintptr_t)p.A + (uint64_t)(alon * 2)), wbasen = rfl64((uint64_t)(uintptr_t)p.W + (uint64_t)(wlon * 2));
    const uint64_t bbase = rfl64((uint64_t)(uintptr_t)p.bias);
    unsigned aoff[8], woff[8];
#pragma unroll
    for (int i = 0; i < 8; ++i) {
      const int r = osk_tile256::dma_row<4>(wave, lane, i);
      const int c = osk_tile256::dma_chunk(lane, r);
      aoff[i] = (unsigned)((Walk::a_row(p, m0 + r) - alo) * 2 + c * 16);
      woff[i] = (unsigned)((Walk::w_row(p, n0 + r, true) - wlo) * 2 + c * 16);
    }
    const int m0w = m0 + wm * WT, n0w = n0 + wn * WT;
    const bool folded = Walk::folded(p, n0w);
    const unsigned boff = (unsigned)((n0w + q4 * 4) * 4);
    const unsigned flags = rfl(prefetched | (has_next ? 2u : 0u) | (folded ? 4u : 0u));
    const unsigned aoffp = (unsigned)((Walk::a_row(p, m0 + wave * 64 + lane) - alo) * 2);
    const unsigned woffp = (unsigned)((Walk::w_row(p, n0 + wave * 64 + lane, false) - wlo) * 2);
    OSK_TT(0, tt0);
#ifdef OSK_GEMM_TILE_TIMING
    const unsigned long long tt1 = __builtin_amdgcn_s_memtime();
#endif
    asm volatile(
#include "gemm256x_body.inc"
        OSKW_OPERANDS : OSKX_CLOBBERS);
    static_assert(OSKX_ACC_QUADS == 64, "the generated loop's accumulator map: quad T = tile T, a0 .. a255");
    osk_v4f aq[64];
    asm volatile("" : OSK_AQ_OUT_0_64(aq));
    OSK_TT(1, tt1);
#ifdef OSK_GEMM_TILE_TIMING
    const unsigned long long tt2 = __builtin_amdgcn_s_memtime();
#endif
    Walk::epilogue(aq, p, m0w, n0w, l15, q4, folded);
    OSK_TT(2, tt2);
#ifdef OSK_GEMM_TILE_TIMING
    if (threadIdx.x == 0) atomicAdd(&osk_gemm_tile_ticks[3], 1ull);
#endif
    prefetched = has_next ? 1u : 0u;
  }
}

#undef OSKW_OPERANDS

template <bool OUT_F32, int NP>
__global__ void __launch_bounds__(256, 1) gemm256x_kernel(const GemmPack<NP> pk) {
  tile_walk<LinearWalk<OUT_F32>>(pk);
}

template <int NP>
__global__ void __launch_bounds__(256, 1) gemm256x_vt_kernel(const GemmPack<NP> pk) {
  static_assert(NP <= 2, "a run-time index into a wider pack makes hipcc copy the pack to scratch");
  tile_walk<VtWalk>(pk);
}

int tiles_of(const GemmParams& p) { return ((p.M + 255) / 256) * ((p.N - p.skip_len + 255) / 256); }

template <bool OUT_F32>
int launch_one(const GemmParams& p, hipStream_t st) {
  auto kernel = gemm256x_kernel<OUT_F32, 1>;
  OSK_ENSURE_MAX_SMEM(kernel, OSKX_SMEM);
  GemmPack<1> pk;
  pk.p[0] = p;
  hipLaunchKernelGGL(kernel, dim3(osk_tile256::persistent_grid(tiles_of(p))), dim3(256), OSKX_SMEM, st, pk);
  return (int)hipGetLastError();
}

}

#ifdef OSK_GEMM_TILE_TIMING
extern "C" int osk_gemm_tile_timing_read(unsigned long long* out4) {
  unsigned long long zero[4] = {0, 0, 0, 0};
  if (hipMemcpyFromSymbol(out4, HIP_SYMBOL(osk_gemm_tile_ticks), sizeof(zero)) != hipSuccess) return -1;
  return hipMemcpyToSymbol(HIP_SYMBOL(osk_gemm_tile_ticks), zero, sizeof(zero)) == hipSuccess ? 0 : -1;
}
#endif

int launch_gemm256x(const GemmParams& p, int out_f32, hipStream_t st) {
  return out_f32 ? launch_one<true>(p, st) : launch_one<false>(p, st);
}

int launch_gemm256x_pair(const GemmParams& p0, const GemmParams& p1, hipStream_t st) {
  auto kernel = gemm256x_kernel<false, 2>;
  OSK_ENSURE_MAX_SMEM(kernel, OSKX_SMEM);
  GemmPack<2> pk;
  pk.p[0] = p0;
  pk.p[1] = p1;
  hipLaunchKernelGGL(kernel, dim3(osk_tile256::persistent_grid(tiles_of(p0) + tiles_of(p1))), dim3(256), OSKX_SMEM, st, pk);
  return (int)hipGetLastError();
}

int launch_gemm256x_vt(const GemmParams* ps, int n, hipStream_t st) {
  if (n < 1 || n > 2) return OSK_EINVAL;
  auto kernel = gemm256x_vt_kernel<2>;
  OSK_ENSURE_MAX_SMEM(kernel, OSKX_SMEM);
  GemmPack<2> pk;
  int ntiles = 0;
  for (int i = 0; i < 2; ++i) {
    pk.p[i] = ps[i < n ? i : 0];
    if (i >= n) pk.p[i].M = 0;
    ntiles += tiles_of(pk.p[i]);
  }
  hipLaunchKernelGGL(kernel, dim3(osk_tile256::persistent_grid(ntiles)), dim3(256), OSKX_SMEM, st, pk);
  return (int)hipGetLastError();
}

}
```

### open_sora_amd/csrc/gemm_bf16.hip

```cpp
#include <atomic>
#include "gemm_params.h"
#include "tile128.h"
#include "../../include/osk.h"

namespace {

using namespace osk_tile128;
using osk_gemm::GemmParams;

struct GemmASrc {
  const unsigned short* ga[4];
  __device__ __forceinline__ const unsigned short* operator()(const Lane&, int i, int kt) const { return ga[i] + kt * BK; }
};

constexpr int ACT_GELU_FROM = 0, ACT_QUICK_GELU = 1;

template <bool OUT_F32, int ACT = ACT_GELU_FROM>
__global__ void __launch_bounds__(256, 2) gemm_bf16_kernel(const GemmParams p) {
  extern __shared__ __attribute__((aligned(16))) unsigned char smem[];
  const Lane g = make_lane(p.M, p.N, p.W, p.wrs);
  const int m0 = g.bm * BM;

  GemmASrc a_src;
#pragma unroll
  for (int i = 0; i < 4; ++i) {
    int m = m0 + g.row[i];
    m = m < p.M ? m : p.M - 1;
    const int b = m / p.arpb, l = m - b * p.arpb;
    a_src.ga[i] = p.A + b * p.abs_ + (int64_t)l * p.ars + g.cch[i] * 8;
  }

  f32x16_t acc[2][2];
  mainloop(g, smem, p.K / BK, a_src, acc);

#pragma unroll
  for (int tm = 0; tm < 2; ++tm) {
    const int m = m0 + acc_row(g, tm);
    if (m >= p.M) continue;
    const int b = m / p.crpb, l = m - b * p.crpb;
    const int64_t roff = b * p.cbs + (int64_t)l * p.crs;
    const float* grow = p.gate ? p.gate + b * p.gbs : nullptr;
#pragma unroll
    for (int tn = 0; tn < 2; ++tn) {
#pragma unroll
      for (int qd = 0; qd < 4; ++qd) {
        const int n = acc_col(g, tn, qd);
        if (n >= p.N) continue;
        float v[4];
#pragma unroll
        for (int j = 0; j < 4; ++j) v[j] = acc[tn][tm][qd * 4 + j];
        if (n + 3 < p.N) {
          if (p.bias) {
            const float4 bv = *reinterpret_cast<const float4*>(p.bias + n);
            v[0] += bv.x; v[1] += bv.y; v[2] += bv.z; v[3] += bv.w;
          }
#pragma unroll
          for (int j = 0; j < 4; ++j) {
            if constexpr (ACT == ACT_QUICK_GELU) v[j] = quick_gelu(v[j]);
            else if (n + j >= p.gelu_from) v[j] = gelu_tanh(v[j]);
          }
          if (grow) {
            const float4 gv = *reinterpret_cast<const float4*>(grow + n);
            const uint2 rv = *reinterpret_cast<const uint2*>(p.res + roff + n);
            v[0] = bf16_lo(rv.x) + gv.x * v[0];
            v[1] = bf16_hi(rv.x) + gv.y * v[1];
            v[2] = bf16_lo(rv.y) + gv.z * v[2];
            v[3] = bf16_hi(rv.y) + gv.w * v[3];
          }
          if constexpr (OUT_F32) {
            *reinterpret_cast<float4*>(reinterpret_cast<float*>(p.C) + roff + n) = make_float4(v[0], v[1], v[2], v[3]);
          } else {
            uint2 o;
            o.x = pack_bf16x2(v[0], v[1]);
            o.y = pack_bf16x2(v[2], v[3]);
            *reinterpret_cast<uint2*>(reinterpret_cast<unsigned short*>(p.C) + roff + n) = o;
          }
        } else {
          for (int j = 0; j < 4 && n + j < p.N; ++j) {
            float t = v[j] + (p.bias ? p.bias[n + j] : 0.f);
            if constexpr (ACT == ACT_QUICK_GELU) t = quick_gelu(t);
            else if (n + j >= p.gelu_from) t = gelu_tanh(t);
            if (grow) t = bf16_bits_to_f32(p.res[roff + n + j]) + grow[n + j] * t;
            if constexpr (OUT_F32) reinterpret_cast<float*>(p.C)[roff + n + j] = t;
            else reinterpret_cast<unsigned short*>(p.C)[roff + n + j] = f32_to_bf16_bits(t);
          }
        }
      }
    }
  }
}

}

static int fill_params(GemmParams& p, const void* A, int64_t a_batch_stride, int64_t a_row_stride, int a_rows_per_batch,
                       const void* W, int64_t w_row_stride, const float* bias, void* C, int64_t c_batch_stride,
                       int64_t c_row_stride, int c_rows_per_batch, const void* res, const float* gate,
                       int64_t gate_batch_stride, int M, int N, int K, int gelu_from, int out_f32) {
  if (!A || !W || !C || M <= 0 || N <= 0 || K <= 0) return OSK_EINVAL;
  if (K % BK) return OSK_EINVAL;
  if (a_rows_per_batch <= 0 || c_rows_per_batch <= 0) return OSK_EINVAL;
  if ((a_batch_stride & 7) || (a_row_stride & 7) || (w_row_stride & 7)) return OSK_EINVAL;
  if ((c_batch_stride & 3) || (c_row_stride & 3)) return OSK_EINVAL;
  if (((uintptr_t)A & 15) || ((uintptr_t)W & 15) || ((uintptr_t)C & 7) || ((uintptr_t)bias & 15)) return OSK_EINVAL;
  if (gate && (!res || ((uintptr_t)gate & 15) || (gate_batch_stride & 3) || ((uintptr_t)res & 7))) return OSK_EINVAL;
  if (out_f32 && ((uintptr_t)C & 15)) return OSK_EINVAL;
  p.A = (const unsigned short*)A; p.abs_ = a_batch_stride; p.ars = a_row_stride; p.arpb = a_rows_per_batch;
  p.W = (const unsigned short*)W; p.wrs = w_row_stride; p.bias = bias;
  p.C = C; p.cbs = c_batch_stride; p.crs = c_row_stride; p.crpb = c_rows_per_batch;
  p.res = (const unsigned short*)res; p.gate = gate; p.gbs = gate_batch_stride;
  p.M = M; p.N = N; p.K = K; p.gelu_from = gelu_from;
  p.group = (N + 255) / 256 <= 6 ? 4 : 8;
  return OSK_OK;
}

static std::atomic<int> g_tile_override{-1};
static int tile_choice(int M, int N, int K, double* cost = nullptr) {
  auto rounds = [](int64_t tiles, int64_t slots) { return (double)((tiles + slots - 1) / slots); };
  const int forced = g_tile_override.load(std::memory_order_relaxed);
  if (forced >= 0 && !cost) return forced;
  const int64_t m256 = (M + 255) / 256, m128 = (M + 127) / 128;
  const double r128 = K >= 2304 ? 0.60 : 0.74;
  const double c256 = rounds(m256 * ((N + 255) / 256), 256) * 4.0 / 1.00;
  const double c128 = rounds(m256 * ((N + 127) / 128), 256) * 2.0 / r128;
  const double cold = rounds(m128 * ((N + 127) / 128), 512) * 1.0 / (0.5 * 0.55);
  const bool wide = N >= 256 && c256 <= c128;
  const double best = wide ? c256 : c128;
  if (cost) *cost = cold < best ? cold : best;
  if (cold < best) return 0;
  return wide ? 2 : 1;
}

static bool large_tiles_ok(const GemmParams& p) { return osk_gemm::gemm256_supported(p); }

static int dispatch_kind(const GemmParams& p) { return large_tiles_ok(p) ? tile_choice(p.M, p.N, p.K) : 0; }

namespace {
__global__ void __launch_bounds__(256) geglu_rows_kernel(const unsigned short* __restrict__ t, unsigned short* __restrict__ c,
                                                         int64_t cbs, int64_t crs, int crpb, int M, int n_out) {
  const int per_row = n_out / 4;
  const int64_t total = (int64_t)M * per_row;
  for (int64_t i = (int64_t)blockIdx.x * 256 + threadIdx.x; i < total; i += (int64_t)gridDim.x * 256) {
    const int m = (int)(i / per_row), c4 = (int)(i - (int64_t)m * per_row) * 4;
    const int j2 = c4 >> 4, r = c4 & 15;
    const unsigned short* row = t + (int64_t)m * 2 * n_out + j2 * 32 + r;
    const uint2 v = *reinterpret_cast<const uint2*>(row), g = *reinterpret_cast<const uint2*>(row + 16);
    uint2 o;
    o.x = pack_bf16x2(bf16_lo(v.x) * gelu_tanh(bf16_lo(g.x)), bf16_hi(v.x) * gelu_tanh(bf16_hi(g.x)));
    o.y = pack_bf16x2(bf16_lo(v.y) * gelu_tanh(bf16_lo(g.y)), bf16_hi(v.y) * gelu_tanh(bf16_hi(g.y)));
    const int b = m / crpb, l = m - b * crpb;
    *reinterpret_cast<uint2*>(c + b * cbs + (int64_t)l * crs + c4) = o;
  }
}
}

extern "C" int osk_gemm_geglu_bf16(const void* A, int64_t a_batch_stride, int64_t a_row_stride, int a_rows_per_batch,
                                   const void* W_packed, int64_t w_row_stride, const float* bias_packed, void* C,
                                   int64_t c_batch_stride, int64_t c_row_stride, int c_rows_per_batch, int M, int N_out, int K,
                                   void* workspace, int64_t workspace_bytes, void* stream) {
  if (N_out <= 0 || (N_out & 15)) return OSK_EINVAL;
  GemmParams p;
  const int N = 2 * N_out;
  const int rc = fill_params(p, A, a_batch_stride, a_row_stride, a_rows_per_batch, W_packed, w_row_stride, bias_packed, C,
                             c_batch_stride, c_row_stride, c_rows_per_batch, nullptr, nullptr, 0, M, N, K, N, 0);
  if (rc != OSK_OK) return rc;
  hipStream_t st = (hipStream_t)stream;
  p.geglu = 1;
  if (large_tiles_ok(p) && tile_choice(M, N, K) == 2) return osk_gemm::launch_gemm256x(p, 0, st);
  if (!workspace || ((uintptr_t)workspace & 15) || workspace_bytes < (int64_t)M * N * 2) return OSK_EUNSUPPORTED;
  const int rc2 = osk_gemm_bf16(A, a_batch_stride, a_row_stride, a_rows_per_batch, W_packed, w_row_stride, bias_packed, workspace,
                                (int64_t)M * N, N, M, nullptr, nullptr, 0, M, N, K, N, 0, stream);
  if (rc2 != OSK_OK) return rc2;
  const int64_t total = (int64_t)M * (N_out / 4);
  const int blocks = (int)((total + 255) / 256 < 4096 ? (total + 255) / 256 : 4096);
  hipLaunchKernelGGL(geglu_rows_kernel, dim3(blocks), dim3(256), 0, st, (const unsigned short*)workspace, (unsigned short*)C,
                     c_batch_stride, c_row_stride, c_rows_per_batch, M, N_out);
  return (int)hipGetLastError();
}

extern "C" int osk_gemm_tile_choice(int M, int N, int K) { return tile_choice(M, N, K); }
extern "C" int osk_gemm_tile_choice_strided(int M, int N, int K, int64_t a_batch_stride, int64_t a_row_stride, int a_rows_per_batch,
                                            int64_t w_row_stride) {
  if (M <= 0 || N <= 0 || K <= 0 || (K % BK) || a_rows_per_batch <= 0) return OSK_EINVAL;
  if ((a_batch_stride & 7) || (a_row_stride & 7) || (w_row_stride & 7)) return OSK_EINVAL;
  GemmParams p{};
  p.abs_ = a_batch_stride; p.ars = a_row_stride; p.arpb = a_rows_per_batch; p.wrs = w_row_stride;
  p.M = M; p.N = N; p.K = K;
  return dispatch_kind(p);
}
extern "C" int osk_gemm_tile_override(int tile_kind) {
  if (tile_kind < -1 || tile_kind > 2) return OSK_EINVAL;
  g_tile_override.store(tile_kind, std::memory_order_relaxed);
  return OSK_OK;
}

extern "C" int osk_gemm_bf16_pair(const OskGemmOperands* a, const OskGemmOperands* b, int N, int K, int gelu_from, void* stream) {
  if (!a || !b) return OSK_EINVAL;
  GemmParams p[2];
  const OskGemmOperands* o[2] = {a, b};
  for (int i = 0; i < 2; ++i) {
    const int rc = fill_params(p[i], o[i]->A, o[i]->a_batch_stride, o[i]->a_row_stride, o[i]->a_rows_per_batch, o[i]->W,
                               o[i]->w_row_stride, o[i]->bias, o[i]->C, o[i]->c_batch_stride, o[i]->c_row_stride,
                               o[i]->c_rows_per_batch, o[i]->res, o[i]->gate, o[i]->gate_batch_stride, o[i]->M, N, K, gelu_from, 0);
    if (rc != OSK_OK) return rc;
  }
  const int big = p[0].M >= p[1].M ? 0 : 1;
  double c_big = 0.0, c_small = 0.0;
  if (large_tiles_ok(p[0]) && large_tiles_ok(p[1]) && tile_choice(p[big].M, N, K, &c_big) == 2) {
    tile_choice(p[big ^ 1].M, N, K, &c_small);
    const int64_t nbn = (N + 255) / 256, tiles = ((p[0].M + 255) / 256 + (p[1].M + 255) / 256) * nbn;
    const double c_pair = (double)((tiles + 255) / 256) * 4.0;
    if (c_pair < c_big + c_small) return osk_gemm::launch_gemm256x_pair(p[big], p[big ^ 1], (hipStream_t)stream);
  }
  (void)big;
  for (int i = 0; i < 2; ++i) {
    const int rc = osk_gemm_bf16(o[i]->A, o[i]->a_batch_stride, o[i]->a_row_stride, o[i]->a_rows_per_batch, o[i]->W, o[i]->w_row_stride,
                                 o[i]->bias, o[i]->C, o[i]->c_batch_stride, o[i]->c_row_stride, o[i]->c_rows_per_batch, o[i]->res,
                                 o[i]->gate, o[i]->gate_batch_stride, o[i]->M, N, K, gelu_from, 0, stream);
    if (rc != OSK_OK) return rc;
  }
  return OSK_OK;
}

extern "C" int osk_gemm_bf16(const void* A, int64_t a_batch_stride, int64_t a_row_stride,
                             int a_rows_per_batch, const void* W, int64_t w_row_stride,
                             const float* bias, void* C, int64_t c_batch_stride, int64_t c_row_stride,
                             int c_rows_per_batch, const void* res, const float* gate,
                             int64_t gate_batch_stride, int M, int N, int K, int gelu_from,
                             int out_f32, void* stream) {
  GemmParams p;
  const int rc = fill_params(p, A, a_batch_stride, a_row_stride, a_rows_per_batch, W, w_row_stride, bias, C, c_batch_stride,
                             c_row_stride, c_rows_per_batch, res, gate, gate_batch_stride, M, N, K, gelu_from, out_f32);
  if (rc != OSK_OK) return rc;
  hipStream_t st = (hipStream_t)stream;
  const int kind = dispatch_kind(p);
  if (kind == 2) return osk_gemm::launch_gemm256x(p, out_f32, st);
  if (kind == 1) return osk_gemm::launch_gemm256p(p, out_f32, st);
  const int nblk = ((M + BM - 1) / BM) * ((N + BN - 1) / BN);
  dim3 grid(nblk), block(256);
  if (out_f32) hipLaunchKernelGGL((gemm_bf16_kernel<true>), grid, block, SMEM_BYTES, st, p);
  else hipLaunchKernelGGL((gemm_bf16_kernel<false>), grid, block, SMEM_BYTES, st, p);
  return (int)hipGetLastError();
}

extern "C" int osk_gemm_quickgelu_bf16(const void* A, int64_t a_batch_stride, int64_t a_row_stride, int a_rows_per_batch, const void* W,
                                       int64_t w_row_stride, const float* bias, void* C, int64_t c_batch_stride, int64_t c_row_stride,
                                       int c_rows_per_batch, int M, int N, int K, void* stream) {
  GemmParams p;
  const int rc = fill_params(p, A, a_batch_stride, a_row_stride, a_rows_per_batch, W, w_row_stride, bias, C, c_batch_stride,
                             c_row_stride, c_rows_per_batch, nullptr, nullptr, 0, M, N, K, N, 0);
  if (rc != OSK_OK) return rc;
  const int64_t nblk = (int64_t)((M + BM - 1) / BM) * ((N + BN - 1) / BN);
  if (nblk > 0x7FFFFFFF) return OSK_EUNSUPPORTED;
  hipLaunchKernelGGL((gemm_bf16_kernel<false, ACT_QUICK_GELU>), dim3((unsigned)nblk), dim3(256), SMEM_BYTES, (hipStream_t)stream, p);
  return (int)hipGetLastError();
}

extern "C" int osk_gemm_group_bf16(const OskGemmTask* tasks, int n_tasks, int K, void* stream) {
  if (!tasks || n_tasks < 1 || n_tasks > 4 || K <= 0 || (K % BK)) return OSK_EINVAL;
  GemmParams plain[4], vts[4];
  int n_plain = 0, n_vt = 0;
  for (int i = 0; i < n_tasks; ++i) {
    const OskGemmTask& t = tasks[i];
    const OskGemmOperands& o = t.op;
    if (t.vt_head_dim == 0) {
      GemmParams& p = plain[n_plain++];
      const int rc = fill_params(p, o.A, o.a_batch_stride, o.a_row_stride, o.a_rows_per_batch, o.W, o.w_row_stride, o.bias, o.C,
                                 o.c_batch_stride, o.c_row_stride, o.c_rows_per_batch, o.res, o.gate, o.gate_batch_stride, o.M, t.N, K,
                                 t.gelu_from, 0);
      if (rc != OSK_OK) return rc;
      if (t.skip_len < 0 || t.skip_from < 0) return OSK_EINVAL;
      if (t.skip_len > 0) {
        if (o.gate || (t.skip_from % 256) || (t.skip_len % 8) || t.skip_from + t.skip_len > t.N) return OSK_EINVAL;
        p.skip_from = t.skip_from;
        p.skip_len = t.skip_len;
      }
      if (!large_tiles_ok(p) || t.N - t.skip_len < 128) return OSK_EUNSUPPORTED;
      continue;
    }
    GemmParams& p = vts[n_vt++];
    const int hd = t.vt_head_dim, L = o.a_rows_per_batch;
    if (hd != 64 && hd != 72 && hd != 128) return OSK_EUNSUPPORTED;
    if (!o.A || !o.W || !o.C || o.res || o.gate || L <= 0 || o.M <= 0 || (o.M % L) || t.N <= 0 || (t.N % hd)) return OSK_EINVAL;
    if ((o.a_batch_stride & 7) || (o.a_row_stride & 7) || (o.w_row_stride & 7) || ((uintptr_t)o.A & 15) || ((uintptr_t)o.W & 15) ||
        ((uintptr_t)o.C & 1) || ((uintptr_t)o.bias & 3))
      return OSK_EINVAL;
    const int B = o.M / L, Lp = (L + 63) / 64 * 64;
    if ((int64_t)B * Lp > 0x7fffff00) return OSK_EUNSUPPORTED;
    p = GemmParams{};
    p.A = (const unsigned short*)o.W; p.abs_ = 0; p.ars = o.w_row_stride; p.arpb = 0x7fffffff;
    p.W = (const unsigned short*)o.A; p.wrs = o.a_row_stride; p.wbs = o.a_batch_stride; p.wrpb = Lp; p.wvalid = L;
    p.bias = nullptr; p.rowbias = o.bias;
    p.C = o.C; p.cbs = 0; p.crs = o.c_row_stride; p.crpb = t.N; p.ccbs = o.c_batch_stride;
    p.res = nullptr; p.gate = nullptr; p.gbs = 0;
    p.M = t.N; p.N = B * Lp; p.K = K; p.gelu_from = p.N;
    p.group = 8;
    p.vt = hd == 128 ? 2 : 1;
    if (!osk_gemm::gemm256_supported(p)) return OSK_EUNSUPPORTED;
  }
  if (n_vt > 2 || n_plain > 2) return OSK_EUNSUPPORTED;
  hipStream_t st = (hipStream_t)stream;
  if (n_plain == 2 && plain[0].N == plain[1].N && plain[0].gelu_from == plain[1].gelu_from && !plain[0].skip_len && !plain[1].skip_len) {
    const int big = plain[0].M >= plain[1].M ? 0 : 1;
    plain[big ^ 1].group = plain[big].group;
    const int rc = osk_gemm::launch_gemm256x_pair(plain[big], plain[big ^ 1], st);
    if (rc != OSK_OK) return rc;
  } else {
    for (int i = 0; i < n_plain; ++i) {
      const int rc = osk_gemm::launch_gemm256x(plain[i], 0, st);
      if (rc != OSK_OK) return rc;
    }
  }
  if (n_vt) {
    if (n_vt == 2 && vts[1].M * (int64_t)vts[1].N > vts[0].M * (int64_t)vts[0].N) { const GemmParams t_ = vts[0]; vts[0] = vts[1]; vts[1] = t_; }
    return osk_gemm::launch_gemm256x_vt(vts, n_vt, st);
  }
  return OSK_OK;
}
```

### open_sora_amd/csrc/gemm_epilogue16.h

```cpp
#pragma once
#include "gemm_epilogue.h"

namespace osk_gemm {
namespace epi16 {

using epi::GELU_ALL;
using epi::GELU_MIXED;
using epi::GELU_NONE;

template <class Geo, int T, bool GATE, int GELU>
OSK_DEV void tile_values_rv(const osk_v4f* aq, const GemmParams& p, int n, const float4& gq, const uint2& rv, float* acc) {
  Geo::template read<T>(aq, acc);
  if constexpr (GELU == GELU_ALL) {
#pragma unroll
    for (int i = 0; i < 4; ++i) acc[i] = gelu_tanh(acc[i]);
  } else if constexpr (GELU == GELU_MIXED) {
#pragma unroll
    for (int i = 0; i < 4; ++i) {
      const float g = gelu_tanh(acc[i]);
      acc[i] = n + i >= p.gelu_from ? g : acc[i];
    }
  }
  if constexpr (GATE) {
    acc[0] = bf16_lo(rv.x) + gq.x * acc[0];
// ... 25 lines not shown
    *reinterpret_cast<uint4*>(reinterpret_cast<unsigned short*>(p.C) + storeoff[I / 2] + n0w + J * 16) = make_uint4(sx[0], sy[0], sx[1], sy[1]);
  }
}


template <class Geo, bool GATE, int GELU, int J, int I>
OSK_DEV uint4 chunk_interior(const osk_v4f* aq, const GemmParams& p, const int64_t* rowoff, int n0w, int q4, const float4& gq) {
  constexpr int NB = Geo::NB;
  const int n = n0w + J * 16 + q4 * 4;
  float a0[4], a1[4];
  tile_values<Geo, J * NB + I, GATE, GELU>(aq, p, rowoff[I], n, gq, a0);
  tile_values<Geo, J * NB + I + 1, GATE, GELU>(aq, p, rowoff[I + 1], n, gq, a1);
  auto sx = __builtin_amdgcn_permlane16_swap(pack_bf16x2(a0[0], a0[1]), pack_bf16x2(a1[0], a1[1]), false, false);
  auto sy = __builtin_amdgcn_permlane16_swap(pack_bf16x2(a0[2], a0[3]), pack_bf16x2(a1[2], a1[3]), false, false);
  return make_uint4(sx[0], sy[0], sx[1], sy[1]);
}

template <class Geo, int GELU, int J, int I>
OSK_DEV uint4 chunk_interior_res(const osk_v4f* aq, const GemmParams& p, int n0w, int q4, const float4& gq, const uint4& rc) {
  constexpr int NB = Geo::NB;
  const int n = n0w + J * 16 + q4 * 4;
  auto ux = __builtin_amdgcn_permlane16_swap(rc.x, rc.z, false, false);
  auto uy = __builtin_amdgcn_permlane16_swap(rc.y, rc.w, false, false);
  float a0[4], a1[4];
  tile_values_rv<Geo, J * NB + I, true, GELU>(aq, p, n, gq, make_uint2(ux[0], uy[0]), a0);
  tile_values_rv<Geo, J * NB + I + 1, true, GELU>(aq, p, n, gq, make_uint2(ux[1], uy[1]), a1);
  auto sx = __builtin_amdgcn_permlane16_swap(pack_bf16x2(a0[0], a0[1]), pack_bf16x2(a1[0], a1[1]), false, false);
  auto sy = __builtin_amdgcn_permlane16_swap(pack_bf16x2(a0[2], a0[3]), pack_bf16x2(a1[2], a1[3]), false, false);
  return make_uint4(sx[0], sy[0], sx[1], sy[1]);
}

template <class Geo, bool GATE, int GELU, bool RESW, int I, int... Js>
OSK_DEV void row_pair_wide(const osk_v4f* aq, const GemmParams& p, const int64_t* rowoff, int64_t own, int n0w, int q4, int lane, const float4* gq,
                           std::integer_sequence<int, Js...>) {
  constexpr int NB = Geo::NB;
  static_assert(NB % 4 == 0, "column blocks are transposed in groups of four");
  uint4 d[NB];
  const int j = lane & 3;
  const bool odd = lane & 1, hi = lane & 2;
  const int64_t base_off = own + n0w + 16 * j - (int64_t)j * p.crs;
  if constexpr (GATE && RESW) {
    uint4 rw[NB];
    const unsigned short* rbase = p.res + base_off;
#pragma unroll
    for (int b = 0; b < NB / 4; ++b)
#pragma unroll
      for (int r = 0; r < 4; ++r) rw[4 * b + r] = *reinterpret_cast<const uint4*>(rbase + (int64_t)r * p.crs + 64 * b);
#pragma unroll
    for (int b = 0; b < NB / 4; ++b) {
      quad_transpose(rw[4 * b].x, rw[4 * b + 1].x, rw[4 * b + 2].x, rw[4 * b + 3].x, odd, hi);
      quad_transpose(rw[4 * b].y, rw[4 * b + 1].y, rw[4 * b + 2].y, rw[4 * b + 3].y, odd, hi);
      quad_transpose(rw[4 * b].z, rw[4 * b + 1].z, rw[4 * b + 2].z, rw[4 * b + 3].z, odd, hi);
      quad_transpose(rw[4 * b].w, rw[4 * b + 1].w, rw[4 * b + 2].w, rw[4 * b + 3].w, odd, hi);
    }
    ((d[Js] = chunk_interior_res<Geo, GELU, Js, I>(aq, p, n0w, q4, gq[Js], rw[Js])), ...);
  } else {
    ((d[Js] = chunk_interior<Geo, GATE, GELU, Js, I>(aq, p, rowoff, n0w, q4, gq[Js])), ...);
  }
#pragma unroll
  for (int b = 0; b < NB / 4; ++b) {
    quad_transpose(d[4 * b].x, d[4 * b + 1].x, d[4 * b + 2].x, d[4 * b + 3].x, odd, hi);
    quad_transpose(d[4 * b].y, d[4 * b + 1].y, d[4 * b + 2].y, d[4 * b + 3].y, odd, hi);
    quad_transpose(d[4 * b].z, d[4 * b + 1].z, d[4 * b + 2].z, d[4 * b + 3].z, odd, hi);
    quad_transpose(d[4 * b].w, d[4 * b + 1].w, d[4 * b + 2].w, d[4 * b + 3].w, odd, hi);
  }
  unsigned short* base = reinterpret_cast<unsigned short*>(p.C) + base_off;
#pragma unroll
  for (int b = 0; b < NB / 4; ++b)
#pragma unroll
    for (int r = 0; r < 4; ++r)
      *reinterpret_cast<uint4*>(base + (int64_t)r * p.crs + 64 * b) = d[4 * b + r];
}

template <class Geo, bool GATE, int GELU, int... Is>
OSK_DEV void tile_interior_wide(const osk_v4f* aq, const GemmParams& p, const int64_t* rowoff, const int64_t* storeoff, int n0w, int q4, int lane,
                                const float4* gq, std::integer_sequence<int, Is...>) {
  if constexpr (GATE) {
#ifndef OSK_GEMM_NARROW_RES
    if ((((uintptr_t)p.res) & 15) == 0) {
      (row_pair_wide<Geo, GATE, GELU, true, 2 * Is>(aq, p, rowoff, storeoff[Is], n0w, q4, lane, gq, std::make_integer_sequence<int, Geo::NB>{}), ...);
      return;
    }
#endif
  }
  (row_pair_wide<Geo, GATE, GELU, false, 2 * Is>(aq, p, rowoff, storeoff[Is], n0w, q4, lane, gq, std::make_integer_sequence<int, Geo::NB>{}), ...);
}

template <class Geo, bool OUT_F32, int T>
OSK_DEV void tile_edge(const osk_v4f* aq, const GemmParams& p, int m0w, int n0w, int l15, int q4, bool folded) {
  constexpr int NB = Geo::NB;
  constexpr int J = T / NB, I = T % NB;
  float acc[4];
  Geo::template read<T>(aq, acc);
  const int m = m0w + I * 16 + l15;
  if (m >= p.M) return;
  const int b = m / p.crpb, l = m - b * p.crpb;
  const int64_t roff = b * p.cbs + (int64_t)l * p.crs;
  const float* grow = p.gate ? p.gate + b * p.gbs : nullptr;
  const int n = n0w + J * 16 + q4 * 4;
  for (int j = 0; j < 4 && n + j < p.N; ++j) {
    float t = acc[j];
    if (!folded && p.bias) t += p.bias[n + j];
    if (n + j >= p.gelu_from) t = gelu_tanh(t);
    if (grow) t = bf16_bits_to_f32(p.res[roff + n + j]) + grow[n + j] * t;
    if constexpr (OUT_F32) reinterpret_cast<float*>(p.C)[roff + n + j] = t;
    else reinterpret_cast<unsigned short*>(p.C)[roff + n + j] = f32_to_bf16_bits(t);
  }
}

template <class Geo, bool OUT_F32, bool GATE, int GELU, int I, int... Js>
OSK_DEV void row_pair(const osk_v4f* aq, const GemmParams& p, const int64_t* rowoff, const int64_t* storeoff, int n0w, int q4, const float4* gq,
                      std::integer_sequence<int, Js...>) {
  (pair_interior<Geo, OUT_F32, GATE, GELU, Js, I>(aq, p, rowoff, storeoff, n0w, q4, gq[Js]), ...);
}

template <class Geo, bool OUT_F32, bool GATE, int GELU, int... Is>
OSK_DEV void tile_interior(const osk_v4f* aq, const GemmParams& p, const int64_t* rowoff, const int64_t* storeoff, int n0w, int q4, const float4* gq,
                           std::integer_sequence<int, Is...>) {
  (row_pair<Geo, OUT_F32, GATE, GELU, 2 * Is>(aq, p, rowoff, storeoff, n0w, q4, gq, std::make_integer_sequence<int, Geo::NB>{}), ...);
}

template <class Geo, bool OUT_F32, bool GATE>
OSK_DEV void cols_interior(const osk_v4f* aq, const GemmParams& p, const int64_t* rowoff, const int64_t* storeoff, int m0w, int n0w, int q4) {
  constexpr int NB = Geo::NB;
  constexpr auto seq = std::make_integer_sequence<int, NB / 2>{};
  float4 gq[NB];
#pragma unroll
  for (int j = 0; j < NB; ++j) {
    gq[j] = make_float4(0.f, 0.f, 0.f, 0.f);
    if constexpr (GATE) gq[j] = *reinterpret_cast<const float4*>(p.gate + (m0w / p.crpb) * p.gbs + n0w + j * 16 + q4 * 4);
  }
  if constexpr (!OUT_F32) {
#ifndef OSK_GEMM_NARROW_STORES
    const int lane = q4 * 16 + (int)(threadIdx.x & 15);
    if (n0w + NB * 16 <= p.gelu_from) tile_interior_wide<Geo, GATE, GELU_NONE>(aq, p, rowoff, storeoff, n0w, q4, lane, gq, seq);
    else if (n0w >= p.gelu_from) tile_interior_wide<Geo, GATE, GELU_ALL>(aq, p, rowoff, storeoff, n0w, q4, lane, gq, seq);
    else tile_interior_wide<Geo, GATE, GELU_MIXED>(aq, p, rowoff, storeoff, n0w, q4, lane, gq, seq);
    return;
#endif
  }
  if (n0w + NB * 16 <= p.gelu_from) tile_interior<Geo, OUT_F32, GATE, GELU_NONE>(aq, p, rowoff, storeoff, n0w, q4, gq, seq);
  else if (n0w >= p.gelu_from) tile_interior<Geo, OUT_F32, GATE, GELU_ALL>(aq, p, rowoff, storeoff, n0w, q4, gq, seq);
  else tile_interior<Geo, OUT_F32, GATE, GELU_MIXED>(aq, p, rowoff, storeoff, n0w, q4, gq, seq);
}

template <class Geo, bool OUT_F32, int... Ts>
OSK_DEV void tiles_edge(const osk_v4f* aq, const GemmParams& p, int m0w, int n0w, int l15, int q4, bool folded, std::integer_sequence<int, Ts...>) {
  (tile_edge<Geo, OUT_F32, Ts>(aq, p, m0w, n0w, l15, q4, folded), ...);
}

template <class Geo, int J2, int I>
OSK_DEV void geglu_pair_interior(const osk_v4f* aq, const GemmParams& p, const int64_t* storeoff, int n0o) {
  constexpr int NB = Geo::NB;
  float v0[4], g0[4], v1[4], g1[4];
  Geo::template read<(2 * J2) * NB + I>(aq, v0);
  Geo::template read<(2 * J2 + 1) * NB + I>(aq, g0);
  Geo::template read<(2 * J2) * NB + I + 1>(aq, v1);
  Geo::template read<(2 * J2 + 1) * NB + I + 1>(aq, g1);
#pragma unroll
  for (int i = 0; i < 4; ++i) {
    v0[i] *= gelu_tanh(g0[i]);
    v1[i] *= gelu_tanh(g1[i]);
  }
  auto sx = __builtin_amdgcn_permlane16_swap(pack_bf16x2(v0[0], v0[1]), pack_bf16x2(v1[0], v1[1]), false, false);
  auto sy = __builtin_amdgcn_permlane16_swap(pack_bf16x2(v0[2], v0[3]), pack_bf16x2(v1[2], v1[3]), false, false);
  *reinterpret_cast<uint4*>(reinterpret_cast<unsigned short*>(p.C) + storeoff[I / 2] + n0o + J2 * 16) = make_uint4(sx[0], sy[0], sx[1], sy[1]);
}

template <class Geo, int I, int... J2s>
OSK_DEV void geglu_row_pair(const osk_v4f* aq, const GemmParams& p, const int64_t* storeoff, int n0o, std::integer_sequence<int, J2s...>) {
  (geglu_pair_interior<Geo, J2s, I>(aq, p, storeoff, n0o), ...);
}

template <class Geo, int... Is>
OSK_DEV void geglu_interior(const osk_v4f* aq, const GemmParams& p, const int64_t* storeoff, int n0o, std::integer_sequence<int, Is...>) {
  (geglu_row_pair<Geo, 2 * Is>(aq, p, storeoff, n0o, std::make_integer_sequence<int, Geo::NB / 2>{}), ...);
}

template <class Geo, int T2>
OSK_DEV void geglu_tile_edge(const osk_v4f* aq, const GemmParams& p, int m0w, int n0w, int l15, int q4, bool folded) {
  constexpr int NB = Geo::NB;
  constexpr int J2 = T2 / NB, I = T2 % NB;
  float v[4], g[4];
  Geo::template read<(2 * J2) * NB + I>(aq, v);
  Geo::template read<(2 * J2 + 1) * NB + I>(aq, g);
  const int m = m0w + I * 16 + l15;
  if (m >= p.M) return;
  const int b = m / p.crpb, l = m - b * p.crpb;
  const int64_t roff = b * p.cbs + (int64_t)l * p.crs;
  const int nv = n0w + (2 * J2) * 16 + q4 * 4;
  const int no = n0w / 2 + J2 * 16 + q4 * 4;
  for (int j = 0; j < 4 && no + j < p.N / 2; ++j) {
    float tv = v[j], tg = g[j];
    if (!folded && p.bias) { tv += p.bias[nv + j]; tg += p.bias[nv + 16 + j]; }
    reinterpret_cast<unsigned short*>(p.C)[roff + no + j] = f32_to_bf16_bits(tv * gelu_tanh(tg));
  }
}

template <class Geo, int... Ts>
OSK_DEV void geglu_tiles_edge(const osk_v4f* aq, const GemmParams& p, int m0w, int n0w, int l15, int q4, bool folded, std::integer_sequence<int, Ts...>) {
  (geglu_tile_edge<Geo, Ts>(aq, p, m0w, n0w, l15, q4, folded), ...);
}

template <class Geo>
OSK_DEV void geglu_all(const osk_v4f* aq, const GemmParams& p, int m0w, int n0w, int l15, int q4, bool interior, bool folded) {
  constexpr int NB = Geo::NB;
  if (m0w >= p.M || n0w >= p.N) return;
  const bool wide = ((((uintptr_t)p.C) & 15) == 0) && ((p.crs & 7) == 0) && ((p.cbs & 7) == 0);
  if (!interior || !wide || (p.bias && !folded)) {
    geglu_tiles_edge<Geo>(aq, p, m0w, n0w, l15, q4, folded, std::make_integer_sequence<int, (NB / 2) * NB>{});
    return;
  }
  int64_t storeoff[NB / 2];
  const int b = m0w / p.crpb, l0 = m0w - b * p.crpb + l15;
#pragma unroll
  for (int i = 0; i < NB / 2; ++i) storeoff[i] = b * p.cbs + (int64_t)(l0 + 16 * (2 * i + (q4 & 1))) * p.crs + (q4 >> 1) * 8;
  geglu_interior<Geo>(aq, p, storeoff, n0w / 2, std::make_integer_sequence<int, NB / 2>{});
}

template <class Geo, int J, int I>
OSK_DEV uint4 vt_chunk(const osk_v4f* aq, float rb0, float rb1) {
  constexpr int NB = Geo::NB;
  float a0[4], a1[4];
  Geo::template read<J * NB + I>(aq, a0);
  Geo::template read<J * NB + I + 1>(aq, a1);
#pragma unroll
  for (int i = 0; i < 4; ++i) { a0[i] += rb0; a1[i] += rb1; }
  auto sx = __builtin_amdgcn_permlane16_swap(pack_bf16x2(a0[0], a0[1]), pack_bf16x2(a1[0], a1[1]), false, false);
  auto sy = __builtin_amdgcn_permlane16_swap(pack_bf16x2(a0[2], a0[3]), pack_bf16x2(a1[2], a1[3]), false, false);
  return make_uint4(sx[0], sy[0], sx[1], sy[1]);
}

template <class Geo, int I, int... Js>
OSK_DEV void vt_row_pair(const osk_v4f* aq, const GemmParams& p, int64_t own, const float* rb, int lane, std::integer_sequence<int, Js...>) {
  constexpr int NB = Geo::NB;
  uint4 d[NB];
  const int j = lane & 3;
  const bool odd = lane & 1, hi = lane & 2;
  ((d[Js] = vt_chunk<Geo, Js, I>(aq, rb[I], rb[I + 1])), ...);
#pragma unroll
  for (int b = 0; b < NB / 4; ++b) {
    quad_transpose(d[4 * b].x, d[4 * b + 1].x, d[4 * b + 2].x, d[4 * b + 3].x, odd, hi);
    quad_transpose(d[4 * b].y, d[4 * b + 1].y, d[4 * b + 2].y, d[4 * b + 3].y, odd, hi);
    quad_transpose(d[4 * b].z, d[4 * b + 1].z, d[4 * b + 2].z, d[4 * b + 3].z, odd, hi);
    quad_transpose(d[4 * b].w, d[4 * b + 1].w, d[4 * b + 2].w, d[4 * b + 3].w, odd, hi);
  }
  unsigned short* base = reinterpret_cast<unsigned short*>(p.C) + own + 16 * j - (int64_t)j * p.crs;
#pragma unroll
  for (int b = 0; b < NB / 4; ++b)
#pragma unroll
    for (int r = 0; r < 4; ++r)
      *reinterpret_cast<uint4*>(base + (int64_t)r * p.crs + 64 * b) = d[4 * b + r];
}

template <class Geo, int... Is>
OSK_DEV void vt_interior(const osk_v4f* aq, const GemmParams& p, const int64_t* storeoff, const float* rb, int lane, std::integer_sequence<int, Is...>) {
  (vt_row_pair<Geo, 2 * Is>(aq, p, storeoff[Is], rb, lane, std::make_integer_sequence<int, Geo::NB>{}), ...);
}

template <class Geo, int T>
OSK_DEV void vt_tile_edge(const osk_v4f* aq, const GemmParams& p, int m0w, int n0w, int l15, int q4) {
  constexpr int NB = Geo::NB;
  constexpr int J = T / NB, I = T % NB;
  float acc[4];
  Geo::template read<T>(aq, acc);
  const int m = m0w + I * 16 + l15;
  if (m >= p.M) return;
  const float rb = p.rowbias ? p.rowbias[m] : 0.f;
  const int n = n0w + J * 16 + q4 * 4;
  for (int j = 0; j < 4 && n + j < p.N; ++j) {
    const int b = (n + j) / p.wrpb, pos = (n + j) - b * p.wrpb;
    const float t = vt_perm64(pos, p.vt) < p.wvalid ? acc[j] + rb : 0.f;
    reinterpret_cast<unsigned short*>(p.C)[b * p.ccbs + (int64_t)m * p.crs + pos] = f32_to_bf16_bits(t);
  }
}

template <class Geo, int... Ts>
OSK_DEV void vt_tiles_edge(const osk_v4f* aq, const GemmParams& p, int m0w, int n0w, int l15, int q4, std::integer_sequence<int, Ts...>) {
  (vt_tile_edge<Geo, Ts>(aq, p, m0w, n0w, l15, q4), ...);
}

template <class Geo>
OSK_DEV void vt_all(const osk_v4f* aq, const GemmParams& p, int m0w, int n0w, int l15, int q4) {
  constexpr int NB = Geo::NB, WT = NB * 16;
  if (m0w >= p.M || n0w >= p.N) return;
  const int bcol = n0w / p.wrpb, pos0 = n0w - bcol * p.wrpb;
  const bool interior = m0w + WT <= p.M && n0w + WT <= p.N && pos0 + WT <= p.wrpb && pos0 + WT <= p.wvalid &&
                        ((((uintptr_t)p.C) & 15) == 0) && ((p.crs & 7) == 0) && ((p.ccbs & 7) == 0);
  if (!interior) {
    vt_tiles_edge<Geo>(aq, p, m0w, n0w, l15, q4, std::make_integer_sequence<int, NB * NB>{});
    return;
  }
  float rb[NB];
#pragma unroll
  for (int i = 0; i < NB; ++i) rb[i] = p.rowbias ? p.rowbias[m0w + 16 * i + l15] : 0.f;
  int64_t storeoff[NB / 2];
  const int64_t col0 = bcol * p.ccbs + pos0 + (q4 >> 1) * 8;
#pragma unroll
  for (int i = 0; i < NB / 2; ++i) storeoff[i] = (int64_t)(m0w + l15 + 16 * (2 * i + (q4 & 1))) * p.crs + col0;
  const int lane = q4 * 16 + l15;
  vt_interior<Geo>(aq, p, storeoff, rb, lane, std::make_integer_sequence<int, NB / 2>{});
}

template <class Geo, bool OUT_F32>
OSK_DEV void epilogue_all(const osk_v4f* aq, const GemmParams& p, int m0w, int n0w, int l15, int q4, bool interior, bool folded) {
  constexpr int NB = Geo::NB;
  if constexpr (!OUT_F32) {
    if (p.geglu) {
      geglu_all<Geo>(aq, p, m0w, n0w, l15, q4, interior, folded);
      return;
    }
  }
  if (m0w >= p.M || n0w >= p.N) return;
  const bool wide = OUT_F32 || (((((uintptr_t)p.C) & 15) == 0) && ((p.crs & 7) == 0) && ((p.cbs & 7) == 0));
  if (!interior || !wide || (p.bias && !folded)) {
    tiles_edge<Geo, OUT_F32>(aq, p, m0w, n0w, l15, q4, folded, std::make_integer_sequence<int, NB * NB>{});
    return;
  }
  int64_t rowoff[NB], storeoff[NB / 2];
  const int b = m0w / p.crpb, l0 = m0w - b * p.crpb + l15;
#pragma unroll
  for (int i = 0; i < NB; ++i) rowoff[i] = b * p.cbs + (int64_t)(l0 + 16 * i) * p.crs;
#pragma unroll
  for (int i = 0; i < NB / 2; ++i) storeoff[i] = ((q4 & 1) ? rowoff[2 * i + 1] : rowoff[2 * i]) + (q4 >> 1) * 8;
  if (p.gate) cols_interior<Geo, OUT_F32, true>(aq, p, rowoff, storeoff, m0w, n0w, q4);
  else cols_interior<Geo, OUT_F32, false>(aq, p, rowoff, storeoff, m0w, n0w, q4);
}

}
}
```

### open_sora_amd/csrc/gemm_params.h

```cpp
#pragma once
#include "osk_common.h"
#include <utility>

namespace osk_gemm {

struct GemmParams {
  const unsigned short* A;
  int64_t abs_, ars;
  int arpb;
  const unsigned short* W;
  int64_t wrs;
  const float* bias;
  void* C;
  int64_t cbs, crs;
  int crpb;
  const unsigned short* res;
  const float* gate;
  int64_t gbs;
  int M, N, K, gelu_from;
  int group;
  int geglu = 0;
  const float* sa = nullptr;
  const float* sw = nullptr;
  int skip_from = 0x7fffffff, skip_len = 0;
  int vt = 0;
  int wrpb = 0x7fffffff, wvalid = 0x7fffffff;
  int64_t wbs = 0, ccbs = 0;
  const float* rowbias = nullptr;
};

static __host__ __device__ __forceinline__ int vt_perm64(int pos, int kind) {
  const int g = pos & ~63, p = pos & 63;
  if (kind == 1) {
    const int pc = p >> 3, j = p & 7, r = pc & 3;
    return g + 32 * (pc >> 2) + ((r & 1) << 4) + ((r >> 1) << 2) + ((j >> 2) << 3) + (j & 3);
  }
  const int p16 = p & 15, grp = p & ~15;
  return g + grp + ((p16 < 4 || p16 >= 12) ? p16 : (p16 < 8 ? p16 + 4 : p16 - 4));
}

bool gemm256_supported(const GemmParams& p);
int launch_gemm256p(const GemmParams& p, int out_f32, hipStream_t st);
int launch_gemm256x(const GemmParams& p, int out_f32, hipStream_t st);
int launch_gemm256x_pair(const GemmParams& p0, const GemmParams& p1, hipStream_t st);
int launch_gemm256x_vt(const GemmParams* ps, int n, hipStream_t st);
bool gemm256_fp8_supported(const GemmParams& p);
int launch_gemm256_fp8(const GemmParams& p, int bn, int out_f32, hipStream_t st);

}
```

### open_sora_amd/mmdit.py

```python
from __future__ import annotations

import math
import os
from dataclasses import dataclass, field

import weakref

import torch
from torch import Tensor, nn

from . import _C

_OPS = _C


def set_ops_for_testing(ops) -> None:
    global _OPS
    _OPS = ops


def ops():
    return _OPS

BF16 = torch.bfloat16


@dataclass
class MMDiTConfig:

    model_type = "MMDiT"
    from_pretrained: str | None
    cache_dir: str | None
    in_channels: int
    vec_in_dim: int
    context_in_dim: int
    hidden_size: int
    mlp_ratio: float
    num_heads: int
    depth: int
    depth_single_blocks: int
    axes_dim: list
    theta: int
    qkv_bias: bool
    guidance_embed: bool
    cond_embed: bool = False
    fused_qkv: bool = True
    grad_ckpt_settings: tuple | None = None
    use_liger_rope: bool = False
    patch_size: int = 2

    def get(self, attribute_name, default=None):
        return getattr(self, attribute_name, default)

    def __contains__(self, attribute_name):
        return hasattr(self, attribute_name)


class _OskState:

    def __getstate__(self):
        d = self.__dict__.copy()
        for k in [k for k in d if k.startswith("_osk_")]:
            del d[k]
        if "_plan" in d:
            d["_plan"] = None
        return d


_WATCHERS: "weakref.WeakKeyDictionary" = weakref.WeakKeyDictionary()
_WATCHED: "weakref.WeakSet" = weakref.WeakSet()


def _state_loaded(module, _incompatible_keys) -> None:
    for ref in _WATCHERS.get(module, ()):
        b = ref()
        if b is None:
            continue
        if hasattr(b, "invalidate_plan"):
            b.invalidate_plan()
        elif "_osk_plan" in b.__dict__:
            object.__delattr__(b, "_osk_plan")


def _watch_state_loads(owner) -> None:
    if owner in _WATCHED:
        return
    for m in owner.modules():
        if _state_loaded not in m._load_state_dict_post_hooks.values():
            m.register_load_state_dict_post_hook(_state_loaded)
        _WATCHERS.setdefault(m, []).append(weakref.ref(owner))
    _WATCHED.add(owner)


class _Holder(nn.Module):

    def forward(self, *a, **k):
        raise RuntimeError(
            f"{type(self).__name__} holds parameters only; its arithmetic runs in libosk_hip.so via the "
            "block processor / MMDiTModel.forward (no eager fallback)."
        )


class MLPEmbedder(_Holder):
    def __init__(self, in_dim: int, hidden_dim: int):
        super().__init__()
        self.in_layer = nn.Linear(in_dim, hidden_dim, bias=True)
        self.silu = nn.SiLU()
        self.out_layer = nn.Linear(hidden_dim, hidden_dim, bias=True)


class RMSNorm(_Holder):
    def __init__(self, dim: int):
        super().__init__()
        self.scale = nn.Parameter(torch.ones(dim))


class QKNorm(_Holder):
    def __init__(self, dim: int):
        super().__init__()
        self.query_norm = RMSNorm(dim)
        self.key_norm = RMSNorm(dim)


class SelfAttention(_Holder):
    def __init__(self, dim: int, num_heads: int = 8, qkv_bias: bool = False, fused_qkv: bool = True):
        super().__init__()
        self.num_heads = num_heads
        self.fused_qkv = fused_qkv
        if fused_qkv:
            self.qkv = nn.Linear(dim, dim * 3, bias=qkv_bias)
        else:
            self.q_proj = nn.Linear(dim, dim, bias=qkv_bias)
            self.k_proj = nn.Linear(dim, dim, bias=qkv_bias)
            self.v_proj = nn.Linear(dim, dim, bias=qkv_bias)
        self.norm = QKNorm(dim // num_heads)
        self.proj = nn.Linear(dim, dim)


class Modulation(_Holder):
    def __init__(self, dim: int, double: bool):
        super().__init__()
        self.is_double = double
        self.multiplier = 6 if double else 3
        self.lin = nn.Linear(dim, self.multiplier * dim, bias=True)


class _NoParamNorm(_Holder):

    def __init__(self, dim: int, eps: float = 1e-6):
        super().__init__()
        self.normalized_shape = (dim,)
        self.eps = eps


class DoubleStreamBlock(_OskState, nn.Module):
    def __init__(self, hidden_size: int, num_heads: int, mlp_ratio: float, qkv_bias: bool = False,
                 fused_qkv: bool = True):
        super().__init__()
        mlp_hidden = int(hidden_size * mlp_ratio)
        self.num_heads = num_heads
        self.hidden_size = hidden_size
        self.head_dim = hidden_size // num_heads
        for s in ("img", "txt"):
            setattr(self, f"{s}_mod", Modulation(hidden_size, double=True))
            setattr(self, f"{s}_norm1", _NoParamNorm(hidden_size))
            setattr(self, f"{s}_attn", SelfAttention(hidden_size, num_heads, qkv_bias, fused_qkv))
            setattr(self, f"{s}_norm2", _NoParamNorm(hidden_size))
            setattr(self, f"{s}_mlp", nn.Sequential(
                nn.Linear(hidden_size, mlp_hidden, bias=True),
                nn.GELU(approximate="tanh"),
                nn.Linear(mlp_hidden, hidden_size, bias=True),
            ))
        self.set_processor(HipDoubleStreamBlockProcessor())

    def set_processor(self, processor) -> None:
        self.processor = processor

    def get_processor(self):
        return self.processor

    def forward(self, img: Tensor, txt: Tensor, vec: Tensor, pe, **kwargs):
        return self.processor(self, img, txt, vec, pe)


class SingleStreamBlock(_OskState, nn.Module):
    def __init__(self, hidden_size: int, num_heads: int, mlp_ratio: float = 4.0, qk_scale: float | None = None,
                 fused_qkv: bool = True):
        super().__init__()
        self.hidden_dim = hidden_size
        self.hidden_size = hidden_size
        self.num_heads = num_heads
        self.head_dim = hidden_size // num_heads
        self.scale = qk_scale or self.head_dim ** -0.5
        self.fused_qkv = fused_qkv
        self.mlp_hidden_dim = int(hidden_size * mlp_ratio)
        if fused_qkv:
            self.linear1 = nn.Linear(hidden_size, hidden_size * 3 + self.mlp_hidden_dim)
        else:
            self.q_proj = nn.Linear(hidden_size, hidden_size)
            self.k_proj = nn.Linear(hidden_size, hidden_size)
            self.v_mlp = nn.Linear(hidden_size, hidden_size + self.mlp_hidden_dim)
        self.linear2 = nn.Linear(hidden_size + self.mlp_hidden_dim, hidden_size)
        self.norm = QKNorm(self.head_dim)
        self.pre_norm = _NoParamNorm(hidden_size)
        self.mlp_act = nn.GELU(approximate="tanh")
        self.modulation = Modulation(hidden_size, double=False)
        self.set_processor(HipSingleStreamBlockProcessor())

    def set_processor(self, processor) -> None:
        self.processor = processor

    def get_processor(self):
        return self.processor

    def forward(self, x: Tensor, vec: Tensor, pe, **kwargs) -> Tensor:
        return self.processor(self, x, vec, pe)


class LastLayer(_Holder):
    def __init__(self, hidden_size: int, patch_size: int, out_channels: int):
        super().__init__()
        self.norm_final = _NoParamNorm(hidden_size)
        self.linear = nn.Linear(hidden_size, patch_size * patch_size * out_channels, bias=True)
        self.adaLN_modulation = nn.Sequential(nn.SiLU(), nn.Linear(hidden_size, 2 * hidden_size, bias=True))


def _w(t: Tensor) -> Tensor:
    t = t.detach()
    return t if (t.dtype == BF16 and t.is_contiguous()) else t.to(BF16).contiguous()


def _b32(t: Tensor | None) -> Tensor | None:
    return None if t is None else t.detach().float().contiguous()


_LORA: "weakref.WeakKeyDictionary" = weakref.WeakKeyDictionary()


def _lora_key(module) -> tuple:
    return (getattr(module, "_osk_lora_epoch", 0),)


def _lora_merge(w: Tensor, out: Tensor, ads) -> Tensor:
    ads = [(a.to(w.device), b.to(w.device), float(s)) for a, b, s in ads]
    if hasattr(_OPS, "lora_merge"):
        return _OPS.lora_merge(w, out, ads)
    acc = torch.zeros(w.shape, dtype=torch.float32, device=w.device)
    for a, b, s in ads:
        acc += s * (b.float() @ a.float())
    out.copy_((w.float() + acc).to(BF16) if ads else w)
    return out


def _lin_w(lin) -> Tensor:
    w = _w(lin.weight)
    ads = _LORA.get(lin)
    return _lora_merge(w, torch.empty_like(w), ads) if ads else w


def _cat_linear(*lins):
    if len(lins) == 1:
        w = _lin_w(lins[0])
    elif not any(_LORA.get(l) for l in lins):
        w = torch.cat([_w(l.weight) for l in lins], 0).contiguous()
    else:
        ws = [_w(l.weight) for l in lins]
        w = torch.empty(sum(t.shape[0] for t in ws), ws[0].shape[1], dtype=BF16, device=ws[0].device)
        row = 0
        for l, t in zip(lins, ws):
            _lora_merge(t, w[row: row + t.shape[0]], _LORA.get(l) or ())
            row += t.shape[0]
    if lins[0].bias is None:
        return w, None
    b = torch.cat([l.bias.detach().float() for l in lins], 0).contiguous()
    return w, b


def _pad_k(w: Tensor, mult: int = 64) -> Tensor:
    N, K = w.shape
    Kp = (K + mult - 1) // mult * mult
    if Kp == K:
        return w
    out = torch.zeros(N, Kp, dtype=w.dtype, device=w.device)
    out[:, :K] = w
    return out


class Fp8Weight:

    def __init__(self, w: Tensor, w8: Tensor | None = None, sw: Tensor | None = None):
        self.w = w
        if w8 is None:
            w8, sw = _OPS.quantize_rows_fp8(w)
        self.w8, self.sw = w8, sw

    @property
    def shape(self):
        return self.w.shape

    def __getitem__(self, rows):
        assert isinstance(rows, slice) and (rows.start or 0) % 4 == 0
        return Fp8Weight(self.w[rows], self.w8[rows], self.sw[rows])


def _linear(a, w, b, out: Tensor, **epi) -> Tensor:
    if isinstance(a, tuple):
        a8, sa = a
        return _OPS.gemm_fp8(a8, sa, w.w8, w.sw, b, out, **epi)
    if isinstance(w, Fp8Weight):
        B, L, K = a.shape
        if B * L > 0 and _OPS.gemm_fp8_supported(B * L, w.shape[0], K):
            a8, sa = _OPS.quantize_rows_fp8(a)
            return _OPS.gemm_fp8(a8, sa, w.w8, w.sw, b, out, **epi)
        w = w.w
    return _OPS.gemm(a, w, b, out, **epi)


def _linear_pair(first: dict, second: dict, gelu_from: int | None = None) -> None:
    if all(not isinstance(d["a"], tuple) and not isinstance(d["w"], Fp8Weight) for d in (first, second)):
        _OPS.gemm_pair(first, second, gelu_from=gelu_from)
        return
    for d in (first, second):
        epi = {k: d[k] for k in ("res", "gate", "gate_batch_stride") if k in d}
        if gelu_from is not None:
            epi["gelu_from"] = gelu_from
        _linear(d["a"], d["w"], d["bias"], d["out"], **epi)


def _ln_modulate_for(w, x: Tensor, shift: Tensor, scale: Tensor, xm: Tensor, mbs: int):
    B, L, K = x.shape
    if isinstance(w, Fp8Weight) and B * L > 0 and _OPS.gemm_fp8_supported(B * L, 128, K):
        return _OPS.ln_modulate_fp8(x, shift, scale, mbs)
    _OPS.ln_modulate(x, shift, scale, xm, mbs)
    return xm


@dataclass
class _AttnW:
    qkv_w: Tensor
    qkv_b: Tensor | None
    q_scale: Tensor
    k_scale: Tensor
    proj_w: Tensor | None = None
    proj_b: Tensor | None = None


@dataclass
class _DoublePlan:
    img: _AttnW
    txt: _AttnW
    img_mlp: tuple = ()
    txt_mlp: tuple = ()
    mod_layers: list = field(default_factory=list)
    pv8: bool = False
    qk8: bool = False
    key: tuple = ()
    score_bound: float = 0.0


@dataclass
class _SinglePlan:
    w1: Tensor
    b1: Tensor | None
    w2: Tensor
    b2: Tensor | None
    q_scale: Tensor
    k_scale: Tensor
    mod_layers: list = field(default_factory=list)
    pv8: bool = False
    qk8: bool = False
    key: tuple = ()
    score_bound: float = 0.0


def _score_bound(hd: int, q_scales, k_scales) -> float:
    wq = max(float(t.detach().float().abs().max()) for t in q_scales)
    wk = max(float(t.detach().float().abs().max()) for t in k_scales)
    return 1.05 * q_mult(hd) * hd * wq * wk


def _attn_weights(sa, wrap=lambda w: w) -> _AttnW:
    if getattr(sa, "fused_qkv", hasattr(sa, "qkv")):
        w, b = _cat_linear(sa.qkv)
    else:
        w, b = _cat_linear(sa.q_proj, sa.k_proj, sa.v_proj)
    return _AttnW(wrap(w), b, _w(sa.norm.query_norm.scale), _w(sa.norm.key_norm.scale), wrap(_lin_w(sa.proj)),
                  _b32(sa.proj.bias))


def _wrap_for(block):
    return Fp8Weight if getattr(block, "_osk_fp8", False) else (lambda w: w)


def _mod_layer(mod) -> tuple:
    return (_lin_w(mod.lin), None if mod.lin.bias is None else _w(mod.lin.bias))


def _tensor_key(p: Tensor) -> tuple:
    return (p.data_ptr(), 0 if p.is_inference() else p._version)


def _param_key(module):
    return tuple(_tensor_key(p) for p in module.parameters()) + _lora_key(module)


def plan_double(block) -> _DoublePlan:
    p = getattr(block, "_osk_plan", None)
    if p is not None and p.key != _param_key(block):
        p = None
    if p is None:
        wr = _wrap_for(block)
        p = _DoublePlan(
            img=_attn_weights(block.img_attn, wr),
            txt=_attn_weights(block.txt_attn, wr),
            img_mlp=(wr(_lin_w(block.img_mlp[0])), _b32(block.img_mlp[0].bias), wr(_lin_w(block.img_mlp[2])), _b32(block.img_mlp[2].bias)),
            txt_mlp=(wr(_lin_w(block.txt_mlp[0])), _b32(block.txt_mlp[0].bias), wr(_lin_w(block.txt_mlp[2])), _b32(block.txt_mlp[2].bias)),
            mod_layers=[_mod_layer(block.img_mod), _mod_layer(block.txt_mod)],
            pv8=bool(getattr(block, "_osk_fp8", False)), qk8=bool(getattr(block, "_osk_qk8", False)),
        )
        hd = block.head_dim if hasattr(block, "head_dim") else block.hidden_size // block.num_heads
        p.score_bound = _score_bound(hd, (p.img.q_scale, p.txt.q_scale), (p.img.k_scale, p.txt.k_scale))
        p.key = _param_key(block)
        _watch_state_loads(block)
        object.__setattr__(block, "_osk_plan", p)
    return p


def plan_single(block) -> _SinglePlan:
    p = getattr(block, "_osk_plan", None)
    if p is not None and p.key != _param_key(block):
        p = None
    if p is None:
        if getattr(block, "fused_qkv", hasattr(block, "linear1")):
            w1, b1 = _cat_linear(block.linear1)
        else:
            w1, b1 = _cat_linear(block.q_proj, block.k_proj, block.v_mlp)
        wr = _wrap_for(block)
        p = _SinglePlan(wr(w1), b1, wr(_lin_w(block.linear2)), _b32(block.linear2.bias),
                        _w(block.norm.query_norm.scale), _w(block.norm.key_norm.scale),
                        mod_layers=[_mod_layer(block.modulation)], pv8=bool(getattr(block, "_osk_fp8", False)),
                        qk8=bool(getattr(block, "_osk_qk8", False)))
        hd = block.head_dim if hasattr(block, "head_dim") else block.hidden_size // block.num_heads
        p.score_bound = _score_bound(hd, (p.q_scale,), (p.k_scale,))
        p.key = _param_key(block)
        _watch_state_loads(block)
        object.__setattr__(block, "_osk_plan", p)
    return p


class _Workspace:
    def __init__(self, B, L_txt, L_img, D, R, H, hd, device):
        L = L_txt + L_img
        self.B, self.L_txt, self.L_img, self.L = B, L_txt, L_img, L
        self.x = torch.empty(B, L, D, dtype=BF16, device=device)
        self.xm = torch.empty(B, L, D, dtype=BF16, device=device)
        self.y = torch.empty(B * L * (3 * D + R), dtype=BF16, device=device)
        self.h = torch.empty(B, L, R, dtype=BF16, device=device)
        Lp = (L + 63) // 64 * 64
        self.vt = torch.empty(B, H, hd, Lp, dtype=BF16, device=device)
        self.vt_group = hasattr(_OPS, "gemm_group")
        self.attn_window = None
        self.win_ws = None
        self.sp_window = None
        self.attn_anchor = None
        self.win_anchor_ws = None

    def y_double(self, D):
        return self.y[: self.B * self.L * 3 * D].view(self.B, self.L, 3 * D)

    def y_single(self, D, R):
        return self.y.view(self.B, self.L, 3 * D + R)


def _stream_key(device) -> int:
    return torch.cuda.current_stream(device).cuda_stream if torch.device(device).type == "cuda" else 0


def _workspace(owner, B, L_txt, L_img, D, R, H, hd, device) -> _Workspace:
    cache = getattr(owner, "_osk_ws_cache", None)
    if cache is None:
        cache = {}
        object.__setattr__(owner, "_osk_ws_cache", cache)
    key = (B, L_txt, L_img, D, R, H, hd, str(device), _stream_key(device), id(_OPS))
    ws = cache.pop(key, None)
    if ws is None:
        while len(cache) >= 4:
            cache.pop(next(iter(cache)))
        ws = _Workspace(B, L_txt, L_img, D, R, H, hd, device)
    cache[key] = ws
    return ws


@dataclass
class _StepState:
    ws: _Workspace
    rope: object
    mod: Tensor
    plan: dict
    sp: object
    B: int
    L_txt: int
    dtype: torch.dtype
    device: object
    shard: object = None


class _StepCache:

    def __init__(self, key, n, rows, L_img, D, device, shard=None, ranks=1):
        self.key, self.n, self.rows, self.L_img, self.shard = key, n, rows, L_img, shard
        self.prev = torch.zeros(n, L_img, D, dtype=BF16, device=device)
        self.res = torch.empty(rows, L_img, D, dtype=BF16, device=device)
        self.sums = torch.zeros(2, dtype=torch.float32, device=device)
        self.pairs = None if shard is None else torch.zeros(ranks, 2, dtype=torch.float32, device=device)
        self.partials = torch.empty(max(_OPS.step_delta_workspace_bytes(n, L_img, D), 8), dtype=torch.uint8, device=device)
        self.have = [False] * rows


ATTN_CACHE_MODES = ("store", "reuse")


class _AttnCache:

    def __init__(self, key, blocks, rows, L, D, device, shard=None):
        self.key, self.rows, self.L, self.shard = key, rows, L, shard
        self.slots = torch.empty(blocks, rows, L, D, dtype=BF16, device=device)
        self.have = [False] * rows
        self._maps = {}

    def row_map(self, rows: tuple):
        if rows == tuple(range(len(rows))):
            return None
        m = self._maps.get(rows)
        if m is None:
            m = self._maps[rows] = torch.tensor(rows, dtype=torch.int32).to(self.slots.device)
        return m

    def mark(self, rows) -> None:
        for r in rows:
            self.have[r] = True

    def clear(self) -> None:
        self.have = [False] * self.rows


@dataclass
class _AttnStep:
    slot: Tensor
    mode: str
    rows: tuple
    row_map: object

    def view(self):
        r = self.rows
        if len(r) == 1:
            return self.slot[r[0]: r[0] + 1]
        step = r[1] - r[0]
        if step > 0 and all(b - a == step for a, b in zip(r, r[1:])):
            return self.slot[r[0]: r[-1] + 1: step]
        return None


def _attn_store(attn: "_AttnStep", v: Tensor) -> None:
    _OPS.attn_cache_copy(v, attn.slot, attn.row_map, True)


def _attn_load(attn: "_AttnStep", v: Tensor) -> None:
    _OPS.attn_cache_copy(attn.slot, v, attn.row_map, False)


_PE_MEMO: list = [None]


def _pe_to_cos_sin(pe, hd: int):
    if isinstance(pe, _RopeTable):
        return pe.cos, pe.sin, pe.mode
    parts = (pe,) if isinstance(pe, torch.Tensor) else tuple(pe)
    dev = parts[0].device
    memo_ok = not any(t.is_inference() for t in parts) and not (dev.type == "cuda" and torch.cuda.is_current_stream_capturing())
    vers = tuple(t._version for t in parts) if memo_ok else ()
    skey = _stream_key(dev)
    m = _PE_MEMO[0]
    if (memo_ok and m is not None and m[2] == hd and m[3] == str(dev) and m[4] == skey and len(m[0]) == len(parts)
            and all(r() is b for r, b in zip(m[0], parts)) and m[1] == vers):
        return m[5]
    if isinstance(pe, torch.Tensor):
        res = (pe[:, 0, :, :, 0, 0].float().contiguous(), pe[:, 0, :, :, 1, 0].float().contiguous(), 0)
    else:
        cos, sin = pe
        res = (cos[..., : hd // 2].float().contiguous(), sin[..., : hd // 2].float().contiguous(), 1)
    if memo_ok:
        _PE_MEMO[0] = (tuple(weakref.ref(t) for t in parts), vers, hd, str(dev), skey, res)
    return res


@dataclass
class _RopeTable:
    cos: Tensor
    sin: Tensor
    mode: int


class HipEmbedND(nn.Module):

    def __init__(self, dim: int, theta: int, axes_dim, liger: bool):
        super().__init__()
        self.dim, self.theta, self.axes_dim, self.liger = dim, theta, list(axes_dim), liger

    def forward(self, ids: Tensor) -> _RopeTable:
        B, L, n_axes = ids.shape
        idf = ids.float().contiguous().view(B * L, n_axes)
        half = sum(self.axes_dim) // 2
        cos = torch.empty(B, L, half, dtype=torch.float32, device=ids.device)
        sin = torch.empty_like(cos)
        _OPS.rope_table(idf, self.axes_dim, self.theta, self.liger, cos, sin)
        return _RopeTable(cos, sin, 1 if self.liger else 0)


def _mod_views(mod: Tensor, col: int, n: int, D: int):
    return [mod[:, col + i * D: col + (i + 1) * D] for i in range(n)], mod.stride(0)


AUTO_BOUND = True
SCORE_BOUND_LIMIT = 56.0


def q_mult(hd: int) -> float:
    return hd ** -0.5 * 1.4426950408889634


def v_scale_fp8(v: Tensor, H: int, hd: int) -> Tensor:
    return _OPS.v_scale_fp8(v, H, hd)


def _bf16_operands(*xs) -> bool:
    return all(not isinstance(x, (tuple, Fp8Weight)) for x in xs)


def attention_window_bounds(L_txt: int, L_img: int, frame_tokens: int, anchor_head: int = 0, anchor_tail: int = 0) -> tuple[int, int]:
    if L_txt < 0 or L_img <= 0 or frame_tokens <= 0 or anchor_head < 0 or anchor_tail < 0:
        raise ValueError(f"attention_window_bounds: L_txt >= 0, L_img > 0, frame_tokens > 0, anchors >= 0 expected; got "
                         f"{(L_txt, L_img, frame_tokens, anchor_head, anchor_tail)}")
    if L_img % frame_tokens:
        raise ValueError(f"attention_window_bounds: {L_img} image tokens are not whole frames of {frame_tokens}")
    if anchor_head == 0 and anchor_tail == 0:
        return L_txt, 0
    L = L_txt + L_img
    n_prefix = (L_txt + anchor_head * frame_tokens + 63) // 64 * 64
    s0 = (L - anchor_tail * frame_tokens) // 64 * 64 if anchor_tail > 0 else L
    if s0 <= n_prefix:
        raise ValueError(f"attention_window_bounds: anchors ({anchor_head}, {anchor_tail}) of {L_img // frame_tokens} frames leave no "
                         f"windowed keys (prefix [0, {n_prefix}), suffix [{s0}, {L})): that is the full attention, turn the window off")
    return n_prefix, L - s0


def attention_window_table(L_txt: int, L_img: int, frame_tokens: int, window_frames: int, *, row0: int = 0, n_rows: int | None = None,
                           anchor_head: int = 0, anchor_tail: int = 0) -> Tensor:
    if L_txt < 0 or L_img <= 0 or frame_tokens <= 0 or window_frames < 0:
        raise ValueError(f"attention_window_table: L_txt >= 0, L_img > 0, frame_tokens > 0, window_frames >= 0 expected; got {(L_txt, L_img, frame_tokens, window_frames)}")
    if L_img % frame_tokens:
        raise ValueError(f"attention_window_table: {L_img} image tokens are not whole frames of {frame_tokens}")
    N, W, T = frame_tokens, window_frames, L_img // frame_tokens
    L = L_txt + L_img
    n_rows = L - row0 if n_rows is None else n_rows
    if row0 < 0 or n_rows < 1 or row0 + n_rows > L:
        raise ValueError(f"attention_window_table: rows [{row0}, {row0} + {n_rows}) do not lie inside the {L} rows of the joint axis")
    end = row0 + n_rows
    tiles = (L_img + 63) // 64
    rows = []
    for r0 in range(row0, end, 256):
        r1 = min(r0 + 256, end) - 1
        if r0 < L_txt:
            rows.append((0, tiles))
            continue
        f0, f1 = (r0 - L_txt) // N, (r1 - L_txt) // N
        k0, k1 = max(0, f0 - W) * N, min(T, f1 + W + 1) * N
        rows.append((k0 // 64, (k1 + 63) // 64 - k0 // 64))
    if anchor_head == 0 and anchor_tail == 0:
        return torch.tensor(rows, dtype=torch.int32)
    n_prefix, n_suffix = attention_window_bounds(L_txt, L_img, N, anchor_head, anchor_tail)
    body = (L - n_suffix - n_prefix + 63) // 64
    clipped = []
    for t0, n in rows:
        if (t0, n) == (0, tiles):
            clipped.append((0, body))
            continue
        lo = (L_txt + t0 * 64 - n_prefix) // 64
        hi = -((n_prefix - L_txt - (t0 + n) * 64) // 64)
        lo, hi = max(lo, 0), min(hi, body)
        if hi <= lo:
            lo = 0 if hi <= 0 else body - 1
            hi = lo + 1
        clipped.append((lo, hi - lo))
    return torch.tensor(clipped, dtype=torch.int32)


def window_tile_fraction(table: Tensor, L_txt: int, L_img: int, bounds=None) -> float:
    txt_tiles, tiles = (L_txt + 63) // 64, (L_img + 63) // 64
    if bounds is not None:
        fixed = bounds[0] // 64 + (bounds[1] + 63) // 64
        return float((table[:, 1].double() + fixed).sum() / (table.shape[0] * ((L_txt + L_img + 63) // 64)))
    return float((table[:, 1].double() + txt_tiles).sum() / (table.shape[0] * (tiles + txt_tiles)))


def _window_env_default():
    v = os.environ.get("OSK_ATTN_WINDOW_FRAMES", "").strip()
    return int(v) if v else None


def parse_window_anchors(anchors, who: str = "anchors"):
    if anchors is None:
        return None
    if isinstance(anchors, str):
        if not anchors.strip():
            return None
        anchors = anchors.split(",")
    try:
        h, t = (int(a) for a in anchors)
    except (TypeError, ValueError):
        raise ValueError(f"{who}: (head, tail), two non-negative frame counts, expected; got {anchors!r}") from None
    if h < 0 or t < 0:
        raise ValueError(f"{who}: (head, tail), two non-negative frame counts, expected; got {(h, t)}")
    return (h, t) if (h, t) != (0, 0) else None


def _window_anchor_ok() -> bool:
    return hasattr(_OPS, "attention_fwd_window_anchor")


def _window_fp8_ok() -> bool:
    return hasattr(_OPS, "attention_fwd_window_fp8")


def _sp_window_fp8_ok(sp) -> bool:
    return hasattr(_OPS, "kv_join_fp8") and hasattr(_OPS, "kv_quant_rows_fp8") and bool(getattr(sp, "kv_window_fp8", False))


def _window_mode(pv8: bool, qk8: bool, hd: int) -> str:
    if not (pv8 and hd in (72, 128)):
        return "bf16"
    return "qk8" if qk8 and hd == 128 else "pv8"


def _fp8_operands(ws: _Workspace, k: Tensor, v: Tensor, H: int, hd: int, qk8: bool):
    B = v.shape[0]
    vt8 = getattr(ws, "vt8", None)
    if vt8 is None:
        vt8 = ws.vt8 = torch.empty(B, H, _OPS.vt8_rows(hd), ws.vt.shape[-1], dtype=torch.uint8, device=v.device)
    sv = v_scale_fp8(v, H, hd)
    _OPS.v_transpose_fp8(v, sv, vt8, H, hd)
    if not (qk8 and hd == 128):
        return k, None, vt8, sv
    k8 = getattr(ws, "k8", None)
    if k8 is None or tuple(k8.shape) != _OPS.k8_shape(B, H, k.shape[1], hd):
        k8 = ws.k8 = torch.empty(_OPS.k8_shape(B, H, k.shape[1], hd), dtype=torch.uint8, device=k.device)
    sk = v_scale_fp8(k, H, hd)
    _OPS.k_pack_fp8(k, sk, k8, H, hd)
    return k8, sk, vt8, sv


def _joint_attention(ws: _Workspace, q: Tensor, k: Tensor, v: Tensor, H: int, hd: int, pv8: bool = False,
                     score_bound: float = 0.0, vt_ready: bool = False, qk8: bool = False):
    if getattr(ws, "attn_window", None) is not None:
        if pv8 and not _window_fp8_ok():
            raise ValueError("frame-window attention has no fp8 kernels: disable enable_fp8() or set_attention_window(None)")
        if getattr(ws, "attn_anchor", None) is not None:
            if not _window_anchor_ok():
                raise ValueError("frame-window attention: this kernel table has no anchored entry (attention_fwd_window_anchor); "
                                 "set_attention_window(..., anchors=None)")
            if ws.win_anchor_ws is None:
                ws.win_anchor_ws = torch.empty(_OPS.attention_window_anchor_workspace_bytes(q.shape[0], H, q.shape[1], hd),
                                               dtype=torch.uint8, device=q.device)
            kw = dict(n_prefix=ws.attn_anchor[0], n_suffix=ws.attn_anchor[1], windows=ws.attn_window, q_prescaled=True,
                      workspace=ws.win_anchor_ws)
            if pv8 and hd in (72, 128):
                kk, sk, vt8, sv = _fp8_operands(ws, k, v, H, hd, qk8)
                _OPS.attention_fwd_window_anchor(q, kk, vt8, v, H, hd, hd ** -0.5, mode=_window_mode(pv8, qk8, hd), k_scale=sk,
                                                 v_scale=sv, Lk=k.shape[1], **kw)
                return
            if not vt_ready:
                _OPS.v_transpose(v, ws.vt, H, hd)
            _OPS.attention_fwd_window_anchor(q, k, ws.vt, v, H, hd, hd ** -0.5, mode="bf16",
                                             score_bound=score_bound if 0.0 < score_bound <= SCORE_BOUND_LIMIT else 0.0, **kw)
            return
        if ws.win_ws is None:
            ws.win_ws = torch.empty(_OPS.attention_window_workspace_bytes(q.shape[0], H, q.shape[1], hd), dtype=torch.uint8, device=q.device)
        if pv8 and hd in (72, 128):
            kk, sk, vt8, sv = _fp8_operands(ws, k, v, H, hd, qk8)
            _OPS.attention_fwd_window_fp8(q, kk, sk, vt8, sv, v, H, hd, hd ** -0.5, n_prefix=ws.L_txt, windows=ws.attn_window,
                                          mode=_window_mode(pv8, qk8, hd), q_prescaled=True, workspace=ws.win_ws, Lk=k.shape[1])
            return
        if not vt_ready:
            _OPS.v_transpose(v, ws.vt, H, hd)
        _OPS.attention_fwd_window(q, k, ws.vt, v, H, hd, hd ** -0.5, n_prefix=ws.L_txt, windows=ws.attn_window, q_prescaled=True,
                                  score_bound=score_bound if 0.0 < score_bound <= SCORE_BOUND_LIMIT else 0.0, workspace=ws.win_ws)
        return
    wsp = _OPS.attention_workspace(q.device)
    if pv8 and hd in (72, 128):
        kk, sk, vt8, sv = _fp8_operands(ws, k, v, H, hd, qk8)
        if sk is not None:
            _OPS.attention_fwd_qk8(q, kk, sk, vt8, sv, v, H, hd, hd ** -0.5, seg_len=k.shape[1], q_prescaled=True, workspace=wsp)
            return
        _OPS.attention_fwd_pv8(q, k, vt8, sv, v, H, hd, hd ** -0.5, q_prescaled=True, workspace=wsp)
        return
    if not vt_ready:
        _OPS.v_transpose(v, ws.vt, H, hd)
    if AUTO_BOUND and not (0.0 < score_bound <= SCORE_BOUND_LIMIT) and hasattr(_OPS, "attention_fwd_auto"):
        n2 = getattr(ws, "qk_n2", None)
        if n2 is None:
            n2 = ws.qk_n2 = torch.empty(2, q.shape[0], H, dtype=torch.float32, device=q.device)
        _OPS.rownorm2_max(q, n2[0], H, hd)
        _OPS.rownorm2_max(k, n2[1], H, hd)
        _OPS.attention_fwd_auto(q, k, ws.vt, v, H, hd, hd ** -0.5, n2[0], n2[1], q_prescaled=True, workspace=wsp)
        return
    _OPS.attention_fwd(q, k, ws.vt, v, H, hd, hd ** -0.5, q_prescaled=True, workspace=wsp, score_bound=score_bound)


def _sp_qk8(sp, plan) -> dict:
    return {"qk8": True} if plan.qk8 and getattr(sp, "kv_qk8", False) and hasattr(_OPS, "kv_scale_fp8") else {}


def _sp_window(ws) -> dict:
    spec = getattr(ws, "sp_window", None)
    return {} if spec is None else {"window": spec}


def run_double_block(plan: _DoublePlan, ws: _Workspace, mod: Tensor, col_img: int, col_txt: int, rope: _RopeTable,
                     H: int, hd: int, sp=None, x_in=None, x_out=None, attn=None):
    D = H * hd
    Lt, Li = ws.L_txt, ws.L_img
    x_txt, x_img = ws.x[:, :Lt], ws.x[:, Lt:]
    r_img, r_txt = x_img, x_txt
    if x_in is not None:
        assert sp is None and Li and Lt and x_out is not None
        (r_img, r_txt), (x_img, x_txt) = x_in, x_out
    xm_txt, xm_img = ws.xm[:, :Lt], ws.xm[:, Lt:]
    y = ws.y_double(D)
    (i_sh1, i_sc1, i_g1, i_sh2, i_sc2, i_g2), mbs = _mod_views(mod, col_img, 6, D)
    (t_sh1, t_sc1, t_g1, t_sh2, t_sc2, t_g2), _ = _mod_views(mod, col_txt, 6, D)
    csb = rope.cos.stride(0) if rope.cos.shape[0] > 1 else 0
    streams = []
    if Li:
        streams.append((plan.img, r_img, xm_img, y[:, Lt:], i_sh1, i_sc1))
    if Lt:
        streams.append((plan.txt, r_txt, xm_txt, y[:, :Lt], t_sh1, t_sc1))

    q, k, v = y[:, :, :D], y[:, :, D: 2 * D], y[:, :, 2 * D:]
    scales = (plan.txt.q_scale, plan.txt.k_scale, plan.img.q_scale, plan.img.k_scale)
    paired = sp is None and len(streams) == 2
    if attn is not None and attn.mode == "reuse":
        v = attn.view()
        if v is None:
            v = y[:, :, 2 * D:]
            _attn_load(attn, v)
    else:
        _double_block_attention(plan, ws, streams, q, k, v, scales, paired, mbs, rope, csb, Lt, H, hd, sp)
        if attn is not None:
            _attn_store(attn, v)
    _double_block_rest(plan, ws, v, paired, Li, Lt, x_img, x_txt, r_img, r_txt, xm_img, xm_txt, mbs,
                       (i_g1, i_sh2, i_sc2, i_g2), (t_g1, t_sh2, t_sc2, t_g2))


def _double_block_attention(plan, ws, streams, q, k, v, scales, paired, mbs, rope, csb, Lt, H, hd, sp):
    D = H * hd
    acts = [_ln_modulate_for(aw.qkv_w, x_s, sh1, sc1, xm_s, mbs) for aw, x_s, xm_s, y_s, sh1, sc1 in streams]
    vt_ready = False
    if (paired and ws.vt_group and not plan.pv8 and Lt % 64 == 0 and _bf16_operands(*acts, plan.img.qkv_w, plan.txt.qkv_w)):
        tasks = []
        for ((aw, x_s, xm_s, y_s, sh1, sc1), act), pos in zip(zip(streams, acts), (Lt, 0)):
            b = aw.qkv_b
            tasks.append(dict(a=act, w=aw.qkv_w[:2 * D], bias=None if b is None else b[:2 * D], out=y_s))
            tasks.append(dict(x=act, w=aw.qkv_w[2 * D:], bias=None if b is None else b[2 * D:], vt=ws.vt, vt_pos=pos, hd=hd))
        vt_ready = _OPS.gemm_group(tasks)
        if not vt_ready:
            ws.vt_group = False
    if vt_ready:
        pass
    elif paired:
        _linear_pair(*(dict(a=act, w=aw.qkv_w, bias=aw.qkv_b, out=y_s) for (aw, x_s, xm_s, y_s, sh1, sc1), act in zip(streams, acts)))
    elif sp is None:
        for (aw, x_s, xm_s, y_s, sh1, sc1), act in zip(streams, acts):
            _linear(act, aw.qkv_w, aw.qkv_b, y_s)
    if sp is None:
        _OPS.qknorm_rope(q, k, *scales, Lt, rope.cos, rope.sin, csb, H, hd, rope.mode, q_mult=q_mult(hd))
        _joint_attention(ws, q, k, v, H, hd, plan.pv8, plan.score_bound, vt_ready, qk8=plan.qk8)
    else:
        vt_ready = False
        win = _sp_window(ws)
        vt_loc = sp.local_vt(ws.B, ws.L, H, hd, ws.x.device) if (ws.vt_group and not plan.pv8 and Lt % 64 == 0 and hasattr(sp, "local_vt") and not win and
                                                                  _bf16_operands(*acts, *(s_[0].qkv_w for s_ in streams))) else None
        if vt_loc is not None:
            tasks = []
            for ((aw, x_s, xm_s, y_s, sh1, sc1), act) in zip(streams, acts):
                pos = Lt if (aw is plan.img and Lt) else 0
                b = aw.qkv_b
                tasks.append(dict(a=act, w=aw.qkv_w[D: 2 * D], bias=None if b is None else b[D: 2 * D], out=y_s[:, :, D:]))
                tasks.append(dict(x=act, w=aw.qkv_w[2 * D:], bias=None if b is None else b[2 * D:], vt=vt_loc, vt_pos=pos, hd=hd))
            vt_ready = _OPS.gemm_group(tasks)
            if not vt_ready:
                ws.vt_group = False
        if not vt_ready:
            for (aw, x_s, xm_s, y_s, sh1, sc1), act in zip(streams, acts):
                _linear(act, aw.qkv_w[D:], None if aw.qkv_b is None else aw.qkv_b[D:], y_s[:, :, D:])
        _OPS.qknorm_rope(None, k, *scales, Lt, rope.cos, rope.sin, csb, H, hd, rope.mode)
        pending = sp.gather_kv_start(ws, k, v, H, hd, plan.pv8, vt_ready=vt_ready, **_sp_qk8(sp, plan), **win)
        for (aw, x_s, xm_s, y_s, sh1, sc1), act in zip(streams, acts):
            _linear(act, aw.qkv_w[:D], None if aw.qkv_b is None else aw.qkv_b[:D], y_s[:, :, :D])
        _OPS.qknorm_rope(q, None, *scales, Lt, rope.cos, rope.sin, csb, H, hd, rope.mode, q_mult=q_mult(hd))
        sp.attention(ws, pending, q, v, H, hd, plan.score_bound)


def _double_block_rest(plan, ws, v, paired, Li, Lt, x_img, x_txt, r_img, r_txt, xm_img, xm_txt, mbs, mod_img, mod_txt):
    (i_g1, i_sh2, i_sc2, i_g2), (t_g1, t_sh2, t_sc2, t_g2) = mod_img, mod_txt
    if paired:
        _linear_pair(dict(a=v[:, Lt:], w=plan.img.proj_w, bias=plan.img.proj_b, out=x_img, res=r_img, gate=i_g1, gate_batch_stride=mbs),
                     dict(a=v[:, :Lt], w=plan.txt.proj_w, bias=plan.txt.proj_b, out=x_txt, res=r_txt, gate=t_g1, gate_batch_stride=mbs))
        (iw0, ib0, iw2, ib2), (tw0, tb0, tw2, tb2) = plan.img_mlp, plan.txt_mlp
        a_img = _ln_modulate_for(iw0, x_img, i_sh2, i_sc2, xm_img, mbs)
        a_txt = _ln_modulate_for(tw0, x_txt, t_sh2, t_sc2, xm_txt, mbs)
        _linear_pair(dict(a=a_img, w=iw0, bias=ib0, out=ws.h[:, Lt:]), dict(a=a_txt, w=tw0, bias=tb0, out=ws.h[:, :Lt]), gelu_from=0)
        _linear_pair(dict(a=ws.h[:, Lt:], w=iw2, bias=ib2, out=x_img, res=x_img, gate=i_g2, gate_batch_stride=mbs),
                     dict(a=ws.h[:, :Lt], w=tw2, bias=tb2, out=x_txt, res=x_txt, gate=t_g2, gate_batch_stride=mbs))
        return
    if Li:
        _linear(v[:, Lt:], plan.img.proj_w, plan.img.proj_b, x_img, res=x_img, gate=i_g1, gate_batch_stride=mbs)
        w0, b0, w2, b2 = plan.img_mlp
        _linear(_ln_modulate_for(w0, x_img, i_sh2, i_sc2, xm_img, mbs), w0, b0, ws.h[:, Lt:], gelu_from=0)
        _linear(ws.h[:, Lt:], w2, b2, x_img, res=x_img, gate=i_g2, gate_batch_stride=mbs)
    if Lt:
        _linear(v[:, :Lt], plan.txt.proj_w, plan.txt.proj_b, x_txt, res=x_txt, gate=t_g1, gate_batch_stride=mbs)
        w0, b0, w2, b2 = plan.txt_mlp
        _linear(_ln_modulate_for(w0, x_txt, t_sh2, t_sc2, xm_txt, mbs), w0, b0, ws.h[:, :Lt], gelu_from=0)
        _linear(ws.h[:, :Lt], w2, b2, x_txt, res=x_txt, gate=t_g2, gate_batch_stride=mbs)


def run_single_block(plan: _SinglePlan, ws: _Workspace, mod: Tensor, col: int, rope: _RopeTable, H: int, hd: int,
                     R: int, sp=None, x_in=None, x_out=None, attn=None):
    D = H * hd
    x_src = ws.x if x_in is None else x_in
    x_dst = ws.x if x_out is None else x_out
    y = ws.y_single(D, R)
    (shift, scale, gate), mbs = _mod_views(mod, col, 3, D)
    csb = rope.cos.stride(0) if rope.cos.shape[0] > 1 else 0
    act = _ln_modulate_for(plan.w1, x_src, shift, scale, ws.xm, mbs)
    q, k, v = y[:, :, :D], y[:, :, D: 2 * D], y[:, :, 2 * D: 3 * D]
    scales = (plan.q_scale, plan.k_scale, plan.q_scale, plan.k_scale)
    if attn is not None and attn.mode == "reuse":
        b1 = plan.b1
        _linear(act, plan.w1[3 * D:], None if b1 is None else b1[3 * D:], y[:, :, 3 * D:], gelu_from=0)
        _attn_load(attn, v)
    elif sp is None:
        vt_ready = False
        if ws.vt_group and not plan.pv8 and (2 * D) % 256 == 0 and _bf16_operands(act, plan.w1):
            b1 = plan.b1
            vt_ready = _OPS.gemm_group([
                dict(a=act, w=plan.w1, bias=b1, out=y, gelu_from=3 * D, skip=(2 * D, D)),
                dict(x=act, w=plan.w1[2 * D: 3 * D], bias=None if b1 is None else b1[2 * D: 3 * D], vt=ws.vt, vt_pos=0, hd=hd)])
            if not vt_ready:
                ws.vt_group = False
        if not vt_ready:
            _linear(act, plan.w1, plan.b1, y, gelu_from=3 * D)
        _OPS.qknorm_rope(q, k, *scales, 0, rope.cos, rope.sin, csb, H, hd, rope.mode, q_mult=q_mult(hd))
        _joint_attention(ws, q, k, v, H, hd, plan.pv8, plan.score_bound, vt_ready, qk8=plan.qk8)
    else:
        b1 = plan.b1
        vt_ready = False
        win = _sp_window(ws)
        vt_loc = sp.local_vt(ws.B, ws.L, H, hd, ws.x.device) if (ws.vt_group and not plan.pv8 and hasattr(sp, "local_vt") and not win and
                                                                  _bf16_operands(act, plan.w1)) else None
        if vt_loc is not None:
            vt_ready = _OPS.gemm_group([
                dict(a=act, w=plan.w1[D: 2 * D], bias=None if b1 is None else b1[D: 2 * D], out=y[:, :, D:]),
                dict(x=act, w=plan.w1[2 * D: 3 * D], bias=None if b1 is None else b1[2 * D: 3 * D], vt=vt_loc, vt_pos=0, hd=hd)])
            if not vt_ready:
                ws.vt_group = False
        if not vt_ready:
            _linear(act, plan.w1[D: 3 * D], None if b1 is None else b1[D: 3 * D], y[:, :, D: 3 * D])
        _OPS.qknorm_rope(None, k, *scales, 0, rope.cos, rope.sin, csb, H, hd, rope.mode)
        pending = sp.gather_kv_start(ws, k, v, H, hd, plan.pv8, vt_ready=vt_ready, **_sp_qk8(sp, plan), **win)
        mlp_up = lambda: _linear(act, plan.w1[3 * D:], None if b1 is None else b1[3 * D:], y[:, :, 3 * D:], gelu_from=0)
        head_mode = sp.head_parallel(H)
        if not head_mode:
            mlp_up()
        _linear(act, plan.w1[:D], None if b1 is None else b1[:D], q)
        _OPS.qknorm_rope(q, None, *scales, 0, rope.cos, rope.sin, csb, H, hd, rope.mode, q_mult=q_mult(hd))
        if head_mode:
            pending = sp.q_exchange_start(pending, q, H, hd)
            mlp_up()
        sp.attention(ws, pending, q, v, H, hd, plan.score_bound)
    if attn is not None and attn.mode == "store":
        _attn_store(attn, v)
    _linear(y[:, :, 2 * D:], plan.w2, plan.b2, x_dst, res=x_src, gate=gate, gate_batch_stride=mbs)


def _run_modulation(vec32: Tensor, plan, D: int) -> Tensor:
    cached = getattr(plan, "_mod_tasks", None)
    if cached is None or cached[0] != str(vec32.device) or cached[1] is not _OPS:
        cols, col, task_layers = [], 0, []
        for w, b in plan.mod_layers:
            task_layers.append((w, b, col))
            cols.append(col)
            col += w.shape[0]
        cached = (str(vec32.device), _OPS, _OPS.GemvTasks(task_layers, vec32.device), cols, col)
        plan._mod_tasks = cached
    _, _, tasks, cols, ncol = cached
    mod = torch.empty(vec32.shape[0], ncol, dtype=torch.float32, device=vec32.device)
    _OPS.gemv_tasks(vec32, tasks, mod, act_in=1)
    return mod, cols


class _ProcessorPool:
    """owner of the activation workspaces of STAND-ALONE processor calls: one per (geometry, device, stream) shared by every
    block driven that way (57 blocks called one by one used to hold 57 workspaces: ADVICE r2).  Calls on one stream are ordered,
    so blocks sharing a stream can share buffers; another stream gets its own (the key carries the stream)."""


_PROC_POOL = _ProcessorPool()


def _direct_ok(*ts) -> bool:
    return all(t.dtype == BF16 and t.is_contiguous() and t.data_ptr() % 16 == 0 for t in ts)


def _processor_attn_cache_check(attn_cache) -> None:
    if attn_cache is not None:
        raise ValueError("attn_cache: attention broadcast is not available to stand-alone block processor calls (no step identity, no "
                         "cache slot per block); drive an open_sora_amd.mmdit.MMDiTModel through forward_ckpt(attn_cache=...)")


class HipDoubleStreamBlockProcessor:

    def __call__(self, attn: nn.Module, img: Tensor, txt: Tensor, vec: Tensor, pe, attn_cache=None) -> tuple[Tensor, Tensor]:
        _processor_attn_cache_check(attn_cache)
        H, hd = attn.num_heads, attn.head_dim
        D = H * hd
        plan = plan_double(attn)
        B, Li, _ = img.shape
        Lt = txt.shape[1]
        R = plan.img_mlp[0].shape[0]
        ws = _workspace(_PROC_POOL, B, Lt, Li, D, R, H, hd, img.device)
        cos, sin, mode = _pe_to_cos_sin(pe, hd)
        mod, cols = _run_modulation(vec.float().contiguous(), plan, D)
        rope = _RopeTable(cos, sin, mode)
        if Li and Lt and _direct_ok(img, txt):
            o_img, o_txt = torch.empty(B, Li, D, dtype=BF16, device=img.device), torch.empty(B, Lt, D, dtype=BF16, device=img.device)
            run_double_block(plan, ws, mod, cols[0], cols[1], rope, H, hd, x_in=(img, txt), x_out=(o_img, o_txt))
            return o_img, o_txt
        ws.x[:, Lt:].copy_(img)
        ws.x[:, :Lt].copy_(txt)
        run_double_block(plan, ws, mod, cols[0], cols[1], rope, H, hd)
        return ws.x[:, Lt:].clone().to(img.dtype), ws.x[:, :Lt].clone().to(txt.dtype)


class HipSingleStreamBlockProcessor:

    def __call__(self, attn: nn.Module, x: Tensor, vec: Tensor, pe, attn_cache=None) -> Tensor:
        _processor_attn_cache_check(attn_cache)
        H, hd = attn.num_heads, attn.head_dim
        D = H * hd
        plan = plan_single(attn)
        B, L, _ = x.shape
        R = plan.w1.shape[0] - 3 * D
        ws = _workspace(_PROC_POOL, B, 0, L, D, R, H, hd, x.device)
        cos, sin, mode = _pe_to_cos_sin(pe, hd)
        mod, cols = _run_modulation(vec.float().contiguous(), plan, D)
        rope = _RopeTable(cos, sin, mode)
        if _direct_ok(x):
            out = torch.empty(B, L, D, dtype=BF16, device=x.device)
            run_single_block(plan, ws, mod, cols[0], rope, H, hd, R, x_in=x, x_out=out)
            return out
        ws.x.copy_(x)
        run_single_block(plan, ws, mod, cols[0], rope, H, hd, R)
        return ws.x.clone().to(x.dtype)


class MMDiTModel(_OskState, nn.Module):

    config_class = MMDiTConfig

    def __init__(self, config: MMDiTConfig):
        super().__init__()
        self.config = config
        self.in_channels = config.in_channels
        self.out_channels = self.in_channels
        self.patch_size = config.patch_size
        if config.hidden_size % config.num_heads != 0:
            raise ValueError(f"Hidden size {config.hidden_size} must be divisible by num_heads {config.num_heads}")
        pe_dim = config.hidden_size // config.num_heads
        if sum(config.axes_dim) != pe_dim:
            raise ValueError(f"Got {config.axes_dim} but expected positional dim {pe_dim}")
        if config.hidden_size % 64 != 0 or pe_dim not in (64, 72, 128):
            raise ValueError(
                f"gfx950 kernels need hidden_size % 64 == 0 and head_dim in (64, 72, 128); got {config.hidden_size}, {pe_dim}"
            )
        self.hidden_size = config.hidden_size
        self.num_heads = config.num_heads
        self.pe_embedder = HipEmbedND(pe_dim, config.theta, config.axes_dim, liger=config.use_liger_rope)
        D = self.hidden_size
        self.img_in = nn.Linear(self.in_channels, D, bias=True)
        self.time_in = MLPEmbedder(256, D)
        self.vector_in = MLPEmbedder(config.vec_in_dim, D)
        self.guidance_in = MLPEmbedder(256, D) if config.guidance_embed else nn.Identity()
        self.cond_in = nn.Linear(self.in_channels + self.patch_size ** 2, D, bias=True) if config.cond_embed else nn.Identity()
        self.txt_in = nn.Linear(config.context_in_dim, D)
        self.double_blocks = nn.ModuleList([
            DoubleStreamBlock(D, self.num_heads, mlp_ratio=config.mlp_ratio, qkv_bias=config.qkv_bias, fused_qkv=config.fused_qkv)
            for _ in range(config.depth)])
        self.single_blocks = nn.ModuleList([
            SingleStreamBlock(D, self.num_heads, mlp_ratio=config.mlp_ratio, fused_qkv=config.fused_qkv)
            for _ in range(config.depth_single_blocks)])
        self.final_layer = LastLayer(D, 1, self.out_channels)
        if config.cond_embed:
            nn.init.zeros_(self.cond_in.weight)
            nn.init.zeros_(self.cond_in.bias)
        self._plan = None
        self._sp = None
        self._attn_window = None
        self._attn_window_table = None
        self._attn_anchors = None
        self._attn_window_bounds = None
        self.forward = self.forward_ckpt

    def enable_fp8(self, on: bool = True, qk8: bool = False):
        if on and getattr(self, "_attn_window", None) is not None and not _window_fp8_ok():
            raise ValueError("enable_fp8: frame-window attention (set_attention_window) has no fp8 kernels; turn it off first")
        sp = getattr(self, "_sp", None)
        if on and getattr(self, "_attn_window", None) is not None and sp is not None and not _sp_window_fp8_ok(sp):
            raise ValueError("enable_fp8: frame-window attention under sequence parallelism has no fp8 path with this kernel table / sp "
                             "object (kv_join_fp8, kv_quant_rows_fp8, seqpar.SeqPar.kv_window_fp8); set_attention_window(None) first")
        for b in list(self.double_blocks) + list(self.single_blocks):
            object.__setattr__(b, "_osk_fp8", bool(on))
            object.__setattr__(b, "_osk_qk8", bool(on and qk8))
        self.invalidate_plan()
        return self

    def set_attention_window(self, window_frames="env", frame_tokens: int | None = None, anchors="env"):
        if isinstance(window_frames, str) and window_frames == "env":
            window_frames = _window_env_default()
        if isinstance(anchors, str) and anchors == "env":
            anchors = os.environ.get("OSK_ATTN_WINDOW_ANCHORS", "")
        if window_frames is None:
            self._attn_window = None
            self._attn_anchors = None
            return self
        anchors = parse_window_anchors(anchors, "set_attention_window: anchors")
        if anchors is not None and not _window_anchor_ok():
            raise ValueError("set_attention_window: this kernel table has no anchored entry (attention_fwd_window_anchor)")
        if int(window_frames) < 0 or frame_tokens is None or int(frame_tokens) <= 0:
            raise ValueError(f"set_attention_window: window_frames >= 0 and frame_tokens > 0 expected; got {window_frames}, {frame_tokens}")
        if any(getattr(b, "_osk_fp8", False) for b in list(self.double_blocks) + list(self.single_blocks)) and not _window_fp8_ok():
            raise ValueError("set_attention_window: frame-window attention has no fp8 kernels; call enable_fp8(False) first")
        self._sp_window_check(getattr(self, "_sp", None), "set_attention_window")
        self._attn_window = (int(window_frames), int(frame_tokens))
        self._attn_anchors = anchors
        return self

    def _sp_window_check(self, sp, who: str) -> None:
        if sp is None:
            return
        if not getattr(sp, "kv_window", False):
            raise ValueError(f"{who}: frame-window attention does not run under sequence parallelism with this sp object "
                             f"(seqpar.SeqPar.kv_window)")
        if any(getattr(b, "_osk_fp8", False) for b in list(self.double_blocks) + list(self.single_blocks)) and not _sp_window_fp8_ok(sp):
            raise ValueError(f"{who}: frame-window attention under sequence parallelism has no fp8 path with this kernel table / sp object "
                             f"(the e4m3 operands need a join of their own: kv_join_fp8, kv_quant_rows_fp8, seqpar.SeqPar.kv_window_fp8); "
                             f"call enable_fp8(False) or set_attention_window(None)")
        if getattr(sp, "kv_chunks", 1) > 1:
            raise ValueError(f"{who}: frame-window attention under sequence parallelism takes one gather; kv_chunks = {sp.kv_chunks} "
                             f"is refused (seqpar.enable(kv_chunks=1))")

    def _window_table(self, L_txt: int, L_img: int, sp):
        if getattr(self, "_attn_window", None) is None:
            return None
        self._sp_window_check(getattr(self, "_sp", None) if sp is None else sp, "forward")
        if L_txt % 64:
            raise ValueError(f"frame-window attention needs a text length that is a multiple of 64 (the key prefix of "
                             f"osk_attention_fwd_window_bf16); got L_txt = {L_txt}")
        anchors = getattr(self, "_attn_anchors", None)
        key = (L_txt, L_img) + self._attn_window + (anchors or ())
        if self._attn_window_table is None or self._attn_window_table[0] != key:
            a, b = anchors or (0, 0)
            self._attn_window_bounds = None if anchors is None else attention_window_bounds(L_txt, L_img, self._attn_window[1], a, b)
            self._attn_window_table = (key, attention_window_table(L_txt, L_img, self._attn_window[1], self._attn_window[0],
                                                                   anchor_head=a, anchor_tail=b))
        return self._attn_window_table[1]

    def attention_report(self, n_seg: int = 1, seg_len: int = 0, last_seg_len: int = 0) -> dict:
        hd = self.hidden_size // self.num_heads
        plans = [plan_double(b) for b in self.double_blocks] + [plan_single(b) for b in self.single_blocks]
        bounds = [float(p.score_bound) for p in plans]
        bodies = sorted({_OPS.attention_body(hd, n_seg, seg_len, b) for b in bounds}) if hasattr(_OPS, "attention_body") else []
        auto = sum(1 for b in bounds if not (0.0 < b <= SCORE_BOUND_LIMIT)) if AUTO_BOUND and hasattr(_OPS, "attention_fwd_auto") else 0
        sp = getattr(self, "_sp", None)
        chunks = 1
        if sp is not None and hasattr(sp, "kv_chunks_applied"):
            chunks = sp.kv_chunks_applied(self.num_heads, any(p.pv8 for p in plans), seg_len if n_seg > 1 else 0)
        ragged = {}
        if n_seg > 1 and 0 < last_seg_len < seg_len:
            body = lambda n, l: sorted({_OPS.attention_body(hd, n, l, b) for b in bounds}) if hasattr(_OPS, "attention_body") else []
            heads = sp is not None and sp.head_parallel(self.num_heads)
            prep = (1 + int(any(p.qk8 for p in plans))) if heads else 0
            ragged = {"ragged": {"last_seg_len": last_seg_len, "attention_entry_launches": 3, "extra_prep_launches": prep, "bodies_full_segments": body(n_seg - 1, seg_len),
                                 "bodies_last_segment": body(1, last_seg_len), "kv_chunks_requested": getattr(sp, "kv_chunks", 1)}}
            chunks = 1
        window = {"attention_window": None}
        if getattr(self, "_attn_window", None) is not None:
            t = self._attn_window_table
            anchors = getattr(self, "_attn_anchors", None)
            frac = None if t is None else window_tile_fraction(t[1], t[0][0], t[0][1], self._attn_window_bounds if len(t[0]) > 4 else None)
            window = {"attention_window": {"window_frames": self._attn_window[0], "frame_tokens": self._attn_window[1],
                                           "visited_tile_fraction": frac}}
            if anchors is not None:
                window["attention_window"]["anchors"] = anchors
            mode = _window_mode(any(p.pv8 for p in plans), any(p.qk8 for p in plans), hd)
            if mode != "bf16" and _window_fp8_ok():
                window["attention_window"]["mode"] = mode
        return {**ragged, **window, "kv_chunks": chunks, "score_bound_min": min(bounds), "score_bound_max": max(bounds), "bound_limit": SCORE_BOUND_LIMIT, "bodies": bodies,
                "blocks_on_fast_body": sum(1 for b in bounds if 0.0 < b <= SCORE_BOUND_LIMIT), "blocks": len(bounds),
                "blocks_auto_dispatched": auto}

    def invalidate_plan(self):
        self._plan = None
        for b in list(getattr(self, "double_blocks", ())) + list(getattr(self, "single_blocks", ())):
            if hasattr(b, "_osk_plan"):
                object.__delattr__(b, "_osk_plan")

    def _apply(self, fn, *a, **k):
        self.invalidate_plan()
        return super()._apply(fn, *a, **k)

    def load_state_dict(self, *a, **k):
        r = super().load_state_dict(*a, **k)
        self.invalidate_plan()
        return r

    def _plan_key(self):
        return _param_key(self)

    def _build_plan(self, device):
        cfg = self.config
        D = self.hidden_size
        p = {}
        p["double"] = [plan_double(b) for b in self.double_blocks]
        p["single"] = [plan_single(b) for b in self.single_blocks]
        ws_in = [_w(self.img_in.weight)]
        b_in = self.img_in.bias.detach().float()
        if cfg.cond_embed:
            ws_in.append(_w(self.cond_in.weight))
            b_in = b_in + self.cond_in.bias.detach().float()
        p["in_w"] = _pad_k(torch.cat(ws_in, 1).contiguous())
        p["in_b"] = b_in.contiguous()
        p["txt_w"] = _pad_k(_w(self.txt_in.weight))
        p["txt_b"] = _b32(self.txt_in.bias)
        p["final_w"] = _w(self.final_layer.linear.weight)
        p["final_b"] = _b32(self.final_layer.linear.bias)
        layers, col = [], 0
        p["col_double"], p["col_single"] = [], []
        for b in p["double"]:
            c = []
            for w, bias in b.mod_layers:
                layers.append((w, bias, col))
                c.append(col)
                col += w.shape[0]
            p["col_double"].append(c)
        for b in p["single"]:
            w, bias = b.mod_layers[0]
            layers.append((w, bias, col))
            p["col_single"].append(col)
            col += w.shape[0]
        fl = self.final_layer.adaLN_modulation[1]
        layers.append((_w(fl.weight), _w(fl.bias), col))
        p["col_final"] = col
        col += fl.weight.shape[0]
        p["mod_cols"] = col
        p["mod_tasks"] = _OPS.GemvTasks(layers, device)

        def emb(m):
            return (_OPS.GemvTasks([(_w(m.in_layer.weight), _w(m.in_layer.bias), 0)], device),
                    _OPS.GemvTasks([(_w(m.out_layer.weight), _w(m.out_layer.bias), 0)], device))

        p["time_in"] = emb(self.time_in)
        p["vector_in"] = emb(self.vector_in)
        p["guidance_in"] = emb(self.guidance_in) if cfg.guidance_embed else None
        p["key"] = self._plan_key()
        _watch_state_loads(self)
        self._plan = p
        return p

    def prepare_block_inputs(self, img, img_ids, txt, txt_ids, timesteps, y_vec, cond=None, guidance=None,
                             _shard=None):
        cfg = self.config
        if img.ndim != 3 or txt.ndim != 3:
            raise ValueError("Input img and txt tensors must have 3 dimensions.")
        if cfg.cond_embed and cond is None:
            raise ValueError("Didn't get conditional input for conditional model.")
# ... 274 lines not shown
```

Baseline: 4.161 latent frames/s.

## Pre-permute GEMM weight rows so epilogue writes contiguous 16-byte stores

Adds a one-time permutation of weight rows and bias (cached per plan) so that each lane's MFMA accumulator columns land in contiguous 8-element runs of the output. A new store-order epilogue then writes and reads residual values as uint4 vectors instead of narrower scattered stores. It is wired into the double-block proj/MLP pair GEMMs, the single-block w1 group GEMM and the w2 GEMM. The cost is extra weight copies in memory, added fallback paths, and a risk of wrong outputs if the permutation and epilogue mapping disagree.

```diff
diff --git a/include/osk.h b/include/osk.h
--- a/include/osk.h
+++ b/include/osk.h
@@ -19,6 +19,9 @@
                   void* C, int64_t c_batch_stride, int64_t c_row_stride, int c_rows_per_batch,
                   const void* res, const float* gate, int64_t gate_batch_stride,
                   int M, int N, int K, int gelu_from, int out_f32, void* stream);
+
+int osk_gemm_store_order_bf16(const void* W, int64_t w_row_stride, void* W_out, int64_t out_row_stride, const float* bias,
+                              float* bias_out, int N, int K, void* stream);
 
 int osk_gemm_tile_choice(int M, int N, int K);
 int osk_gemm_tile_override(int tile_kind);
@@ -33,6 +36,7 @@
   int M;
 } OskGemmOperands;
 int osk_gemm_bf16_pair(const OskGemmOperands* first, const OskGemmOperands* second, int N, int K, int gelu_from, void* stream);
+int osk_gemm_bf16_pair_store_order(const OskGemmOperands* first, const OskGemmOperands* second, int N, int K, int gelu_from, void* stream);
 
 typedef struct OskGemmTask {
   OskGemmOperands op;
diff --git a/open_sora_amd/_C.py b/open_sora_amd/_C.py
--- a/open_sora_amd/_C.py
+++ b/open_sora_amd/_C.py
@@ -22,7 +22,9 @@
     "osk_ln_modulate_bf16": [_vp, _i64, _i64, _vp, _i64, _i64, _vp, _vp, _i64, _i32, _i32, _i32, _f32, _vp],
     "osk_gemm_bf16": [_vp, _i64, _i64, _i32, _vp, _i64, _vp, _vp, _i64, _i64, _i32, _vp, _vp, _i64,
                       _i32, _i32, _i32, _i32, _i32, _vp],
+    "osk_gemm_store_order_bf16": [_vp, _i64, _vp, _i64, _vp, _vp, _i32, _i32, _vp],
     "osk_gemm_bf16_pair": [_vp, _vp, _i32, _i32, _i32, _vp],
+    "osk_gemm_bf16_pair_store_order": [_vp, _vp, _i32, _i32, _i32, _vp],
     "osk_gemm_group_bf16": [_vp, _i32, _i32, _vp],
     "osk_gemm_tile_choice": [_i32, _i32, _i32],
     "osk_gemm_tile_choice_strided": [_i32, _i32, _i32, _i64, _i64, _i32, _i64],
@@ -230,7 +232,7 @@
 
 
 def gemm(a: torch.Tensor, w: torch.Tensor, bias, out: torch.Tensor, *, res=None, gate=None,
-         gate_batch_stride: int = 0, gelu_from: int | None = None) -> torch.Tensor:
+         gate_batch_stride: int = 0, gelu_from: int | None = None, store_order: bool = False) -> torch.Tensor:
     B, L, K = a.shape
     N = w.shape[0]
     assert out.shape[0] == B and out.shape[1] == L and out.shape[2] == N
@@ -242,8 +244,18 @@
         _check(lib.osk_gemm_bf16(a.data_ptr(), a.stride(0), a.stride(1), L, w.data_ptr(), w.stride(0), _p(bias),
                                  out.data_ptr(), out.stride(0), out.stride(1), L, _p(res), _p(gate),
                                  gate_batch_stride, B * L, N, K, N if gelu_from is None else gelu_from,
-                                 1 if out.dtype == torch.float32 else 0, _stream()), "osk_gemm_bf16")
-    return out
+                                 (1 if out.dtype == torch.float32 else 0) | (2 if store_order else 0), _stream()), "osk_gemm_bf16")
+    return out
+
+
+def gemm_store_order(w: torch.Tensor, bias=None):
+    N, K = w.shape
+    assert w.dtype == torch.bfloat16 and w.stride(1) == 1 and (bias is None or (bias.dtype == torch.float32 and bias.is_contiguous()))
+    wo = torch.empty(N, K, dtype=torch.bfloat16, device=w.device)
+    bo = None if bias is None else torch.empty_like(bias)
+    _check(lib.osk_gemm_store_order_bf16(w.data_ptr(), w.stride(0), wo.data_ptr(), wo.stride(0), _p(bias), _p(bo), N, K, _stream()),
+           "osk_gemm_store_order_bf16")
+    return wo, bo
 
 
 def gemm_tile_kind(a: torch.Tensor, w: torch.Tensor) -> int:
@@ -292,14 +304,18 @@
                            out.stride(0), out.stride(1), L, _p(res), _p(gate), gate_batch_stride, B * L)
 
 
-def gemm_pair(first: dict, second: dict, *, gelu_from: int | None = None) -> None:
+def gemm_pair(first: dict, second: dict, *, gelu_from: int | None = None, store_order: bool = False) -> bool:
     ops = [_gemm_operands(d["a"], d["w"], d["bias"], d["out"], d.get("res"), d.get("gate"), d.get("gate_batch_stride", 0))
            for d in (first, second)]
     N, K = first["w"].shape
     assert tuple(second["w"].shape) == (N, K)
     with _gemm_prof(2.0 * (ops[0].M + ops[1].M) * N * K):
-        _check(lib.osk_gemm_bf16_pair(C.addressof(ops[0]), C.addressof(ops[1]), N, K, N if gelu_from is None else gelu_from,
-                                      _stream()), "osk_gemm_bf16_pair")
+        fn = lib.osk_gemm_bf16_pair_store_order if store_order else lib.osk_gemm_bf16_pair
+        rc = fn(C.addressof(ops[0]), C.addressof(ops[1]), N, K, N if gelu_from is None else gelu_from, _stream())
+    if store_order and rc == OSK_EUNSUPPORTED:
+        return False
+    _check(rc, "osk_gemm_bf16_pair")
+    return True
 
 
 class OskGemmTask(C.Structure):
@@ -325,7 +341,7 @@
             k_ = a.shape[2]
             t.op = _gemm_operands(a, w, d.get("bias"), out, d.get("res"), d.get("gate"), d.get("gate_batch_stride", 0), wide_out=True)
             sf, sl = d.get("skip", (0, 0))
-            t.N, t.gelu_from, t.skip_from, t.skip_len, t.vt_head_dim = w.shape[0], d.get("gelu_from", w.shape[0]) if d.get("gelu_from") is not None else w.shape[0], sf, sl, 0
+            t.N, t.gelu_from, t.skip_from, t.skip_len, t.vt_head_dim = w.shape[0], d.get("gelu_from", w.shape[0]) if d.get("gelu_from") is not None else w.shape[0], sf, sl, (-1 if d.get("store_order") else 0)
             flops += 2.0 * a.shape[0] * a.shape[1] * (w.shape[0] - sl) * k_
         assert K in (None, k_), "the tasks of a group share K"
         K = k_
diff --git a/open_sora_amd/csrc/gemm256x.hip b/open_sora_amd/csrc/gemm256x.hip
--- a/open_sora_amd/csrc/gemm256x.hip
+++ b/open_sora_amd/csrc/gemm256x.hip
@@ -28,7 +28,7 @@
 #endif
 
 
-template <bool OUT_F32>
+template <bool OUT_F32, bool PERM>
 struct LinearWalk {
   template <int NP>
   OSK_DEV int col_tiles(const GemmPack<NP>& pk, int) { return (pk.p[0].N - pk.p[0].skip_len + 255) / 256; }
@@ -46,7 +46,8 @@
     constexpr int WT = OSKX_NB * 16;
     const int b_first = m0w / p.crpb, b_last = (m0w + WT - 1) / p.crpb;
     const bool interior = m0w + WT <= p.M && n0w + WT <= p.N && b_first == b_last;
-    epi16::epilogue_all<GeoX, OUT_F32>(aq, p, m0w, n0w, l15, q4, interior, folded);
+    if constexpr (PERM) epi16::epilogue_all_so<GeoX, OUT_F32>(aq, p, m0w, n0w, l15, q4, interior, folded);
+    else epi16::epilogue_all<GeoX, OUT_F32>(aq, p, m0w, n0w, l15, q4, interior, folded);
   }
 };
 
@@ -174,9 +175,9 @@
 
 #undef OSKW_OPERANDS
 
-template <bool OUT_F32, int NP>
+template <bool OUT_F32, int NP, bool PERM = false>
 __global__ void __launch_bounds__(256, 1) gemm256x_kernel(const GemmPack<NP> pk) {
-  tile_walk<LinearWalk<OUT_F32>>(pk);
+  tile_walk<LinearWalk<OUT_F32, PERM>>(pk);
 }
 
 template <int NP>
@@ -187,9 +188,13 @@
 
 int tiles_of(const GemmParams& p) { return ((p.M + 255) / 256) * ((p.N - p.skip_len + 255) / 256); }
 
-template <bool OUT_F32>
+bool store_order_ok(const GemmParams& p) {
+  return (p.N % 128) == 0 && !p.geglu && !p.vt && (p.skip_len % 128) == 0 && (p.skip_len == 0 || (p.skip_from % 128) == 0);
+}
+
+template <bool OUT_F32, bool PERM>
 int launch_one(const GemmParams& p, hipStream_t st) {
-  auto kernel = gemm256x_kernel<OUT_F32, 1>;
+  auto kernel = gemm256x_kernel<OUT_F32, 1, PERM>;
   OSK_ENSURE_MAX_SMEM(kernel, OSKX_SMEM);
   GemmPack<1> pk;
   pk.p[0] = p;
@@ -208,11 +213,16 @@
 #endif
 
 int launch_gemm256x(const GemmParams& p, int out_f32, hipStream_t st) {
-  return out_f32 ? launch_one<true>(p, st) : launch_one<false>(p, st);
+  if (p.wperm) {
+    if (!store_order_ok(p)) return OSK_EINVAL;
+    return out_f32 ? launch_one<true, true>(p, st) : launch_one<false, true>(p, st);
+  }
+  return out_f32 ? launch_one<true, false>(p, st) : launch_one<false, false>(p, st);
 }
 
 int launch_gemm256x_pair(const GemmParams& p0, const GemmParams& p1, hipStream_t st) {
-  auto kernel = gemm256x_kernel<false, 2>;
+  if (p0.wperm != p1.wperm || (p0.wperm && !(store_order_ok(p0) && store_order_ok(p1)))) return OSK_EINVAL;
+  auto kernel = p0.wperm ? gemm256x_kernel<false, 2, true> : gemm256x_kernel<false, 2, false>;
   OSK_ENSURE_MAX_SMEM(kernel, OSKX_SMEM);
   GemmPack<2> pk;
   pk.p[0] = p0;
diff --git a/open_sora_amd/csrc/gemm_bf16.hip b/open_sora_amd/csrc/gemm_bf16.hip
--- a/open_sora_amd/csrc/gemm_bf16.hip
+++ b/open_sora_amd/csrc/gemm_bf16.hip
@@ -193,7 +193,7 @@
   return OSK_OK;
 }
 
-extern "C" int osk_gemm_bf16_pair(const OskGemmOperands* a, const OskGemmOperands* b, int N, int K, int gelu_from, void* stream) {
+static int gemm_pair(const OskGemmOperands* a, const OskGemmOperands* b, int N, int K, int gelu_from, void* stream, int wperm) {
   if (!a || !b) return OSK_EINVAL;
   GemmParams p[2];
   const OskGemmOperands* o[2] = {a, b};
@@ -202,6 +202,10 @@
                                o[i]->w_row_stride, o[i]->bias, o[i]->C, o[i]->c_batch_stride, o[i]->c_row_stride,
                                o[i]->c_rows_per_batch, o[i]->res, o[i]->gate, o[i]->gate_batch_stride, o[i]->M, N, K, gelu_from, 0);
     if (rc != OSK_OK) return rc;
+    if (wperm) {
+      if ((N % 128) || (p[i].gate && ((uintptr_t)p[i].res & 15))) return OSK_EUNSUPPORTED;
+      p[i].wperm = 1;
+    }
   }
   const int big = p[0].M >= p[1].M ? 0 : 1;
   double c_big = 0.0, c_small = 0.0;
@@ -212,13 +216,21 @@
     if (c_pair < c_big + c_small) return osk_gemm::launch_gemm256x_pair(p[big], p[big ^ 1], (hipStream_t)stream);
   }
   (void)big;
+  if (wperm && (dispatch_kind(p[0]) != 2 || dispatch_kind(p[1]) != 2)) return OSK_EUNSUPPORTED;
   for (int i = 0; i < 2; ++i) {
     const int rc = osk_gemm_bf16(o[i]->A, o[i]->a_batch_stride, o[i]->a_row_stride, o[i]->a_rows_per_batch, o[i]->W, o[i]->w_row_stride,
                                  o[i]->bias, o[i]->C, o[i]->c_batch_stride, o[i]->c_row_stride, o[i]->c_rows_per_batch, o[i]->res,
-                                 o[i]->gate, o[i]->gate_batch_stride, o[i]->M, N, K, gelu_from, 0, stream);
+                                 o[i]->gate, o[i]->gate_batch_stride, o[i]->M, N, K, gelu_from, wperm ? 2 : 0, stream);
     if (rc != OSK_OK) return rc;
   }
   return OSK_OK;
+}
+
+extern "C" int osk_gemm_bf16_pair(const OskGemmOperands* a, const OskGemmOperands* b, int N, int K, int gelu_from, void* stream) {
+  return gemm_pair(a, b, N, K, gelu_from, stream, 0);
+}
+extern "C" int osk_gemm_bf16_pair_store_order(const OskGemmOperands* a, const OskGemmOperands* b, int N, int K, int gelu_from, void* stream) {
+  return gemm_pair(a, b, N, K, gelu_from, stream, 1);
 }
 
 extern "C" int osk_gemm_bf16(const void* A, int64_t a_batch_stride, int64_t a_row_stride,
@@ -228,17 +240,50 @@
                              int64_t gate_batch_stride, int M, int N, int K, int gelu_from,
                              int out_f32, void* stream) {
   GemmParams p;
+  if (out_f32 < 0 || out_f32 > 3) return OSK_EINVAL;
+  const int wperm = out_f32 >> 1;
+  out_f32 &= 1;
   const int rc = fill_params(p, A, a_batch_stride, a_row_stride, a_rows_per_batch, W, w_row_stride, bias, C, c_batch_stride,
                              c_row_stride, c_rows_per_batch, res, gate, gate_batch_stride, M, N, K, gelu_from, out_f32);
   if (rc != OSK_OK) return rc;
   hipStream_t st = (hipStream_t)stream;
   const int kind = dispatch_kind(p);
+  if (wperm) {
+    if (kind != 2 || (N % 128) || (gate && ((uintptr_t)res & 15))) return OSK_EUNSUPPORTED;
+    p.wperm = 1;
+  }
   if (kind == 2) return osk_gemm::launch_gemm256x(p, out_f32, st);
   if (kind == 1) return osk_gemm::launch_gemm256p(p, out_f32, st);
   const int nblk = ((M + BM - 1) / BM) * ((N + BN - 1) / BN);
   dim3 grid(nblk), block(256);
   if (out_f32) hipLaunchKernelGGL((gemm_bf16_kernel<true>), grid, block, SMEM_BYTES, st, p);
   else hipLaunchKernelGGL((gemm_bf16_kernel<false>), grid, block, SMEM_BYTES, st, p);
+  return (int)hipGetLastError();
+}
+
+namespace {
+__global__ void __launch_bounds__(256) store_order_kernel(const unsigned short* __restrict__ w, int64_t wrs, unsigned short* __restrict__ o,
+                                                          int64_t ors, const float* __restrict__ bias, float* __restrict__ bias_o, int N, int K) {
+  const int k8 = K / 8;
+  const int64_t total = (int64_t)N * k8;
+  for (int64_t i = (int64_t)blockIdx.x * 256 + threadIdx.x; i < total; i += (int64_t)gridDim.x * 256) {
+    const int n = (int)(i / k8), c = (int)(i - (int64_t)n * k8);
+    const int src = osk_gemm::store_order_src(n);
+    *reinterpret_cast<uint4*>(o + (int64_t)n * ors + c * 8) = *reinterpret_cast<const uint4*>(w + (int64_t)src * wrs + c * 8);
+    if (c == 0 && bias) bias_o[n] = bias[src];
+  }
+}
+}
+
+extern "C" int osk_gemm_store_order_bf16(const void* W, int64_t w_row_stride, void* W_out, int64_t out_row_stride, const float* bias,
+                                         float* bias_out, int N, int K, void* stream) {
+  if (!W || !W_out || W == W_out || N <= 0 || K <= 0 || (N % 128) || (K % 8)) return OSK_EINVAL;
+  if ((w_row_stride & 7) || (out_row_stride & 7) || w_row_stride < K || out_row_stride < K) return OSK_EINVAL;
+  if (((uintptr_t)W & 15) || ((uintptr_t)W_out & 15) || (bias && (!bias_out || bias == bias_out))) return OSK_EINVAL;
+  const int64_t total = (int64_t)N * (K / 8);
+  const int blocks = (int)((total + 255) / 256 < 8192 ? (total + 255) / 256 : 8192);
+  hipLaunchKernelGGL(store_order_kernel, dim3(blocks), dim3(256), 0, (hipStream_t)stream, (const unsigned short*)W, w_row_stride,
+                     (unsigned short*)W_out, out_row_stride, bias, bias_out, N, K);
   return (int)hipGetLastError();
 }
 
@@ -262,7 +307,7 @@
   for (int i = 0; i < n_tasks; ++i) {
     const OskGemmTask& t = tasks[i];
     const OskGemmOperands& o = t.op;
-    if (t.vt_head_dim == 0) {
+    if (t.vt_head_dim == 0 || t.vt_head_dim == -1) {
       GemmParams& p = plain[n_plain++];
       const int rc = fill_params(p, o.A, o.a_batch_stride, o.a_row_stride, o.a_rows_per_batch, o.W, o.w_row_stride, o.bias, o.C,
                                  o.c_batch_stride, o.c_row_stride, o.c_rows_per_batch, o.res, o.gate, o.gate_batch_stride, o.M, t.N, K,
@@ -275,6 +320,10 @@
         p.skip_len = t.skip_len;
       }
       if (!large_tiles_ok(p) || t.N - t.skip_len < 128) return OSK_EUNSUPPORTED;
+      if (t.vt_head_dim == -1) {
+        if ((t.N % 128) || (t.skip_len % 128) || (o.gate && ((uintptr_t)o.res & 15))) return OSK_EUNSUPPORTED;
+        p.wperm = 1;
+      }
       continue;
     }
     GemmParams& p = vts[n_vt++];
@@ -299,7 +348,8 @@
   }
   if (n_vt > 2 || n_plain > 2) return OSK_EUNSUPPORTED;
   hipStream_t st = (hipStream_t)stream;
-  if (n_plain == 2 && plain[0].N == plain[1].N && plain[0].gelu_from == plain[1].gelu_from && !plain[0].skip_len && !plain[1].skip_len) {
+  if (n_plain == 2 && plain[0].N == plain[1].N && plain[0].gelu_from == plain[1].gelu_from && !plain[0].skip_len && !plain[1].skip_len &&
+      plain[0].wperm == plain[1].wperm) {
     const int big = plain[0].M >= plain[1].M ? 0 : 1;
     plain[big ^ 1].group = plain[big].group;
     const int rc = osk_gemm::launch_gemm256x_pair(plain[big], plain[big ^ 1], st);
diff --git a/open_sora_amd/csrc/gemm_epilogue16.h b/open_sora_amd/csrc/gemm_epilogue16.h
--- a/open_sora_amd/csrc/gemm_epilogue16.h
+++ b/open_sora_amd/csrc/gemm_epilogue16.h
@@ -351,6 +351,93 @@
   vt_interior<Geo>(aq, p, storeoff, rb, lane, std::make_integer_sequence<int, NB / 2>{});
 }
 
+OSK_DEV int so_col(int J, int q4) { return 32 * (J >> 1) + 8 * q4 + 4 * (J & 1); }
+
+template <class Geo, bool OUT_F32, bool GATE, int GELU, int I, int... Gs>
+OSK_DEV void so_row(const osk_v4f* aq, const GemmParams& p, int64_t roff, int nq, const float4* gq, std::integer_sequence<int, Gs...>) {
+  constexpr int NB = Geo::NB;
+  uint4 rw[NB / 2];
+  if constexpr (GATE) ((rw[Gs] = *reinterpret_cast<const uint4*>(p.res + roff + nq + 32 * Gs)), ...);
+  else ((rw[Gs] = make_uint4(0, 0, 0, 0)), ...);
+  float a[NB / 2][8];
+  (tile_values_rv<Geo, (2 * Gs) * NB + I, GATE, GELU>(aq, p, nq + 32 * Gs, gq[2 * Gs], make_uint2(rw[Gs].x, rw[Gs].y), a[Gs]), ...);
+  (tile_values_rv<Geo, (2 * Gs + 1) * NB + I, GATE, GELU>(aq, p, nq + 32 * Gs + 4, gq[2 * Gs + 1], make_uint2(rw[Gs].z, rw[Gs].w), a[Gs] + 4), ...);
+  if constexpr (OUT_F32) {
+    float* c = reinterpret_cast<float*>(p.C) + roff + nq;
+    ((*reinterpret_cast<float4*>(c + 32 * Gs) = make_float4(a[Gs][0], a[Gs][1], a[Gs][2], a[Gs][3]),
+      *reinterpret_cast<float4*>(c + 32 * Gs + 4) = make_float4(a[Gs][4], a[Gs][5], a[Gs][6], a[Gs][7])), ...);
+  } else {
+    unsigned short* c = reinterpret_cast<unsigned short*>(p.C) + roff + nq;
+    ((*reinterpret_cast<uint4*>(c + 32 * Gs) = make_uint4(pack_bf16x2(a[Gs][0], a[Gs][1]), pack_bf16x2(a[Gs][2], a[Gs][3]),
+                                                          pack_bf16x2(a[Gs][4], a[Gs][5]), pack_bf16x2(a[Gs][6], a[Gs][7]))), ...);
+  }
+}
+
+template <class Geo, bool OUT_F32, bool GATE, int GELU, int... Is>
+OSK_DEV void so_tile(const osk_v4f* aq, const GemmParams& p, const int64_t* rowoff, int nq, const float4* gq, std::integer_sequence<int, Is...>) {
+  (so_row<Geo, OUT_F32, GATE, GELU, Is>(aq, p, rowoff[Is], nq, gq, std::make_integer_sequence<int, Geo::NB / 2>{}), ...);
+}
+
+template <class Geo, bool OUT_F32, bool GATE>
+OSK_DEV void so_cols(const osk_v4f* aq, const GemmParams& p, const int64_t* rowoff, int m0w, int n0w, int q4) {
+  constexpr int NB = Geo::NB;
+  constexpr auto seq = std::make_integer_sequence<int, NB>{};
+  float4 gq[NB];
+#pragma unroll
+  for (int j = 0; j < NB; ++j) {
+    gq[j] = make_float4(0.f, 0.f, 0.f, 0.f);
+    if constexpr (GATE) gq[j] = *reinterpret_cast<const float4*>(p.gate + (m0w / p.crpb) * p.gbs + n0w + so_col(j, q4));
+  }
+  const int nq = n0w + 8 * q4;
+  if (n0w + NB * 16 <= p.gelu_from) so_tile<Geo, OUT_F32, GATE, GELU_NONE>(aq, p, rowoff, nq, gq, seq);
+  else if (n0w >= p.gelu_from) so_tile<Geo, OUT_F32, GATE, GELU_ALL>(aq, p, rowoff, nq, gq, seq);
+  else so_tile<Geo, OUT_F32, GATE, GELU_MIXED>(aq, p, rowoff, nq, gq, seq);
+}
+
+template <class Geo, bool OUT_F32, int T>
+OSK_DEV void so_tile_edge(const osk_v4f* aq, const GemmParams& p, int m0w, int n0w, int l15, int q4, bool folded) {
+  constexpr int NB = Geo::NB;
+  constexpr int J = T / NB, I = T % NB;
+  float acc[4];
+  Geo::template read<T>(aq, acc);
+  const int m = m0w + I * 16 + l15;
+  if (m >= p.M) return;
+  const int b = m / p.crpb, l = m - b * p.crpb;
+  const int64_t roff = b * p.cbs + (int64_t)l * p.crs;
+  const float* grow = p.gate ? p.gate + b * p.gbs : nullptr;
+  const int n = n0w + so_col(J, q4), ng = n0w + J * 16 + q4 * 4;
+  for (int j = 0; j < 4 && n + j < p.N; ++j) {
+    float t = acc[j];
+    if (!folded && p.bias) t += p.bias[ng + j];
+    if (n + j >= p.gelu_from) t = gelu_tanh(t);
+    if (grow) t = bf16_bits_to_f32(p.res[roff + n + j]) + grow[n + j] * t;
+    if constexpr (OUT_F32) reinterpret_cast<float*>(p.C)[roff + n + j] = t;
+    else reinterpret_cast<unsigned short*>(p.C)[roff + n + j] = f32_to_bf16_bits(t);
+  }
+}
+
+template <class Geo, bool OUT_F32, int... Ts>
+OSK_DEV void so_tiles_edge(const osk_v4f* aq, const GemmParams& p, int m0w, int n0w, int l15, int q4, bool folded, std::integer_sequence<int, Ts...>) {
+  (so_tile_edge<Geo, OUT_F32, Ts>(aq, p, m0w, n0w, l15, q4, folded), ...);
+}
+
+template <class Geo, bool OUT_F32>
+OSK_DEV void epilogue_all_so(const osk_v4f* aq, const GemmParams& p, int m0w, int n0w, int l15, int q4, bool interior, bool folded) {
+  constexpr int NB = Geo::NB;
+  if (m0w >= p.M || n0w >= p.N) return;
+  const bool wide = (((((uintptr_t)p.C) | (p.gate ? (uintptr_t)p.res : 0)) & 15) == 0) && ((p.crs & 7) == 0) && ((p.cbs & 7) == 0);
+  if (!interior || !wide || (p.bias && !folded)) {
+    so_tiles_edge<Geo, OUT_F32>(aq, p, m0w, n0w, l15, q4, folded, std::make_integer_sequence<int, NB * NB>{});
+    return;
+  }
+  int64_t rowoff[NB];
+  const int b = m0w / p.crpb, l0 = m0w - b * p.crpb + l15;
+#pragma unroll
+  for (int i = 0; i < NB; ++i) rowoff[i] = b * p.cbs + (int64_t)(l0 + 16 * i) * p.crs;
+  if (p.gate) so_cols<Geo, OUT_F32, true>(aq, p, rowoff, m0w, n0w, q4);
+  else so_cols<Geo, OUT_F32, false>(aq, p, rowoff, m0w, n0w, q4);
+}
+
 template <class Geo, bool OUT_F32>
 OSK_DEV void epilogue_all(const osk_v4f* aq, const GemmParams& p, int m0w, int n0w, int l15, int q4, bool interior, bool folded) {
   constexpr int NB = Geo::NB;
diff --git a/open_sora_amd/csrc/gemm_params.h b/open_sora_amd/csrc/gemm_params.h
--- a/open_sora_amd/csrc/gemm_params.h
+++ b/open_sora_amd/csrc/gemm_params.h
@@ -27,7 +27,12 @@
   int wrpb = 0x7fffffff, wvalid = 0x7fffffff;
   int64_t wbs = 0, ccbs = 0;
   const float* rowbias = nullptr;
+  int wperm = 0;
 };
+
+static __host__ __device__ __forceinline__ int store_order_src(int n) {
+  return (n & ~31) + 8 * ((n >> 2) & 3) + 4 * ((n >> 4) & 1) + (n & 3);
+}
 
 static __host__ __device__ __forceinline__ int vt_perm64(int pos, int kind) {
   const int g = pos & ~63, p = pos & 63;
diff --git a/open_sora_amd/mmdit.py b/open_sora_amd/mmdit.py
--- a/open_sora_amd/mmdit.py
+++ b/open_sora_amd/mmdit.py
@@ -314,6 +314,42 @@
             return _OPS.gemm_fp8(a8, sa, w.w8, w.sw, b, out, **epi)
         w = w.w
     return _OPS.gemm(a, w, b, out, **epi)
+
+
+def _store_order(plan, name: str, w, b, a):
+    if not hasattr(_OPS, "gemm_store_order") or not _bf16_operands(a, w) or w.shape[0] % 128:
+        return None
+    if a.shape[0] * a.shape[1] == 0 or _OPS.gemm_tile_kind(a, w) != 2:
+        return None
+    cache = plan.__dict__.setdefault("_so", {})
+    if name not in cache:
+        cache[name] = _OPS.gemm_store_order(w, b)
+    return cache[name]
+
+
+def _linear_so(plan, name: str, a, w, b, out: Tensor, **epi) -> Tensor:
+    so = _store_order(plan, name, w, b, a)
+    if so is None:
+        return _linear(a, w, b, out, **epi)
+    return _OPS.gemm(a, so[0], so[1], out, store_order=True, **epi)
+
+
+def _linear_pair_so(plan, names: tuple, first: dict, second: dict, gelu_from: int | None = None) -> None:
+    N = first["w"].shape[0]
+    if hasattr(_OPS, "gemm_store_order") and _bf16_operands(first["a"], first["w"], second["a"], second["w"]) and N % 128 == 0:
+        cache = plan.__dict__.setdefault("_so", {})
+        key = (names, tuple(first["a"].shape), tuple(second["a"].shape))
+        if cache.get(key, True):
+            if names not in cache:
+                cache[names] = [_OPS.gemm_store_order(d["w"], d["bias"]) for d in (first, second)]
+            ok = _OPS.gemm_pair(*(dict(d, w=so[0], bias=so[1]) for d, so in zip((first, second), cache[names])),
+                                gelu_from=gelu_from, store_order=True)
+            cache[key] = ok
+            if ok:
+                return
+            if not any(v is True for k, v in cache.items() if k[0] == names and k != key):
+                del cache[names]
+    _linear_pair(first, second, gelu_from=gelu_from)
 
 
 def _linear_pair(first: dict, second: dict, gelu_from: int | None = None) -> None:
@@ -913,14 +949,17 @@
 def _double_block_rest(plan, ws, v, paired, Li, Lt, x_img, x_txt, r_img, r_txt, xm_img, xm_txt, mbs, mod_img, mod_txt):
     (i_g1, i_sh2, i_sc2, i_g2), (t_g1, t_sh2, t_sc2, t_g2) = mod_img, mod_txt
     if paired:
-        _linear_pair(dict(a=v[:, Lt:], w=plan.img.proj_w, bias=plan.img.proj_b, out=x_img, res=r_img, gate=i_g1, gate_batch_stride=mbs),
-                     dict(a=v[:, :Lt], w=plan.txt.proj_w, bias=plan.txt.proj_b, out=x_txt, res=r_txt, gate=t_g1, gate_batch_stride=mbs))
+        _linear_pair_so(plan, ("img_proj", "txt_proj"),
+                        dict(a=v[:, Lt:], w=plan.img.proj_w, bias=plan.img.proj_b, out=x_img, res=r_img, gate=i_g1, gate_batch_stride=mbs),
+                        dict(a=v[:, :Lt], w=plan.txt.proj_w, bias=plan.txt.proj_b, out=x_txt, res=r_txt, gate=t_g1, gate_batch_stride=mbs))
         (iw0, ib0, iw2, ib2), (tw0, tb0, tw2, tb2) = plan.img_mlp, plan.txt_mlp
         a_img = _ln_modulate_for(iw0, x_img, i_sh2, i_sc2, xm_img, mbs)
         a_txt = _ln_modulate_for(tw0, x_txt, t_sh2, t_sc2, xm_txt, mbs)
-        _linear_pair(dict(a=a_img, w=iw0, bias=ib0, out=ws.h[:, Lt:]), dict(a=a_txt, w=tw0, bias=tb0, out=ws.h[:, :Lt]), gelu_from=0)
-        _linear_pair(dict(a=ws.h[:, Lt:], w=iw2, bias=ib2, out=x_img, res=x_img, gate=i_g2, gate_batch_stride=mbs),
-                     dict(a=ws.h[:, :Lt], w=tw2, bias=tb2, out=x_txt, res=x_txt, gate=t_g2, gate_batch_stride=mbs))
+        _linear_pair_so(plan, ("img_mlp0", "txt_mlp0"), dict(a=a_img, w=iw0, bias=ib0, out=ws.h[:, Lt:]),
+                        dict(a=a_txt, w=tw0, bias=tb0, out=ws.h[:, :Lt]), gelu_from=0)
+        _linear_pair_so(plan, ("img_mlp2", "txt_mlp2"),
+                        dict(a=ws.h[:, Lt:], w=iw2, bias=ib2, out=x_img, res=x_img, gate=i_g2, gate_batch_stride=mbs),
+                        dict(a=ws.h[:, :Lt], w=tw2, bias=tb2, out=x_txt, res=x_txt, gate=t_g2, gate_batch_stride=mbs))
         return
     if Li:
         _linear(v[:, Lt:], plan.img.proj_w, plan.img.proj_b, x_img, res=x_img, gate=i_g1, gate_batch_stride=mbs)
@@ -953,8 +992,10 @@
         vt_ready = False
         if ws.vt_group and not plan.pv8 and (2 * D) % 256 == 0 and _bf16_operands(act, plan.w1):
             b1 = plan.b1
+            so = _store_order(plan, "w1", plan.w1, b1, act) if D % 128 == 0 else None
+            w1s, b1s = (plan.w1, b1) if so is None else so
             vt_ready = _OPS.gemm_group([
-                dict(a=act, w=plan.w1, bias=b1, out=y, gelu_from=3 * D, skip=(2 * D, D)),
+                dict(a=act, w=w1s, bias=b1s, out=y, gelu_from=3 * D, skip=(2 * D, D), **({} if so is None else {"store_order": True})),
                 dict(x=act, w=plan.w1[2 * D: 3 * D], bias=None if b1 is None else b1[2 * D: 3 * D], vt=ws.vt, vt_pos=0, hd=hd)])
             if not vt_ready:
                 ws.vt_group = False
@@ -990,7 +1031,7 @@
         sp.attention(ws, pending, q, v, H, hd, plan.score_bound)
     if attn is not None and attn.mode == "store":
         _attn_store(attn, v)
-    _linear(y[:, :, 2 * D:], plan.w2, plan.b2, x_dst, res=x_src, gate=gate, gate_batch_stride=mbs)
+    _linear_so(plan, "w2", y[:, :, 2 * D:], plan.w2, plan.b2, x_dst, res=x_src, gate=gate, gate_batch_stride=mbs)
 
 
 def _run_modulation(vec32: Tensor, plan, D: int) -> Tensor:
```

Measured after the change: 4.161 latent frames/s. Within noise of the previous version (-0.0%).
